# AgentMaker/PAPC

Measured on AMD Instinct MI355X. Metric: point-clouds/sec (fwd+bwd) PointNet++SSG B=32 N=4096, higher is better.
Workload: dtype f32

## Files before the change

include/papc_hip.h:

```cpp
#ifndef PAPC_HIP_H
#define PAPC_HIP_H

#include <stddef.h>
#include <stdint.h>

#ifdef __cplusplus
extern "C" {
#endif

#define PAPC_OK 0
#define PAPC_E_INVALID (-1)
#define PAPC_E_UNSUPPORTED (-2)
#define PAPC_E_LAUNCH (-3)

typedef void *papc_stream_t;

int papc_version(void);
#define PAPC_ABI_VERSION 8
int papc_abi_version(void);
int64_t papc_abi_sizeof(const char *struct_name);
const char *papc_last_error_string(void);


int papc_fps_f32(const float *xyz, int64_t sb, int64_t sn, int64_t sc, int B, int N, int npoint,
// ... 142 lines not shown
                        const papc_scatter_dst *scatter, const papc_bwd_red *next_red, papc_stream_t stream);

int papc_mlp_bwd_dw_f32(const papc_bwd_dy *dy, int a_mode, const float *x, int64_t ldx,
                        const papc_group_src *grp, const float *bn_scale, const float *bn_shift, int64_t M,
                        int Cin, int Cout, int rows_per_chunk, float *dw_partial, float *db_partial,
                        int64_t part_ld, papc_stream_t stream);

int papc_mlp_bwd_dw_chunk_hint(int64_t M, int Cin, int Cout, int a_mode, int dz_mode, int K);

int papc_reduce_partials_f32(const float *partial, int n_chunks, int64_t n, float *out, int accumulate,
                             papc_stream_t stream);
typedef struct papc_reduce_job {
    const float *partial;
    int32_t n_chunks;
    int32_t accumulate;
    int64_t ld, n1, n2;
    float *out1, *out2;
} papc_reduce_job;
int papc_reduce_partials_batch_f32(const papc_reduce_job *jobs, int count, papc_stream_t stream);
int papc_reduce_partials2_f32(const float *partial, int n_chunks, int64_t ld, int64_t n1, float *out1, int64_t n2,
                              float *out2, int accumulate, papc_stream_t stream);

#define PAPC_FOLD_MAX 24
typedef struct papc_fold_job {
    const float *partial;
    int32_t n_chunks;
    int32_t accumulate;
    int64_t ld;
    int32_t rows, cols;
    float *out; int64_t out_ld;
} papc_fold_job;
typedef struct papc_fold_list { papc_fold_job *jobs; int32_t capacity, count; } papc_fold_list;
int papc_fold_jobs_f32(const papc_fold_job *jobs, int count, papc_stream_t stream);

#define PAPC_SA_MAX_LAYERS 8
#define PAPC_SA_IN_GROUP 0
#define PAPC_SA_IN_ROWS 1
#define PAPC_SA_NO_LINGATHER 1u
#define PAPC_SA_NO_XYZ1 2u
#define PAPC_SA_NO_NOSTORE 4u
#define PAPC_SA_NO_GMAX 8u
#define PAPC_SA_NO_FUSED_RED 16u
#define PAPC_SA_NO_COMPACT 32u
#define PAPC_SA_NO_PLANES 64u
#define PAPC_SA_NO_PLANES_POINTWISE 128u
#define PAPC_SA_NO_XYZ_FUSE 256u
#define PAPC_SA_NO_PSEL 1024u
#define PAPC_SA_NO_GSIGN 2048u
#define PAPC_SA_NO_WSTATS 512u
typedef struct papc_sa_desc {
    int32_t B, N, S, K, D;
    int32_t n_layers;
    int32_t cin;
    int32_t cout[PAPC_SA_MAX_LAYERS];
    int32_t input;
    int32_t identity_rows;
    int32_t xyz_first, pool, eval_bn, cut_gather_grad;
    float eps, momentum;
    uint32_t disable;
    int32_t inference;
    int32_t want_input_grad;
} papc_sa_desc;
typedef struct papc_sa_layer {
    const float *w, *b, *gamma, *beta;
    float *running_mean, *running_var;
} papc_sa_layer;
typedef struct papc_compact_src {
    const int32_t *start, *rows, *cidx, *seg_grp;
    const float *wrow, *coef;
    int32_t G;
} papc_compact_src;
typedef struct papc_sa_io {
    const float *xyz; int64_t sb, sn, sc;
    const float *new_xyz;
    const float *feats;
    const int32_t *idx;
    const float *x_rows;
    const float *xc; const double *xc_gram;
    const papc_compact_src *compact;
    const float *consts3; int32_t consts3_ld;
    papc_sa_layer layer[PAPC_SA_MAX_LAYERS];
    float *out;
    void *saved, *scratch;
    const papc_point_lists *plists;
    const float *wfeat;
} papc_sa_io;
typedef struct papc_sa_plan {
    papc_sa_desc d;
    int32_t cin0;
    int32_t lin0, xyz1, gmax, nostore, compact, sparse_max, planes;
    int64_t saved_bytes, fwd_scratch_bytes, bwd_scratch_bytes;
    int64_t off_y[PAPC_SA_MAX_LAYERS], off_cst[PAPC_SA_MAX_LAYERS], off_argmax;
} papc_sa_plan;
typedef struct papc_sa_grads {
    const float *gout;
    float *dw[PAPC_SA_MAX_LAYERS], *db[PAPC_SA_MAX_LAYERS], *dgamma[PAPC_SA_MAX_LAYERS], *dbeta[PAPC_SA_MAX_LAYERS];
    int32_t acc_w[PAPC_SA_MAX_LAYERS], acc_gb[PAPC_SA_MAX_LAYERS];
    const float *wt[PAPC_SA_MAX_LAYERS];
    float *grad_feats, *grad_x;
    struct papc_fold_list *defer;
} papc_sa_grads;
int papc_sa_mlp_plan(const papc_sa_desc *desc, const papc_sa_io *io, papc_sa_plan *plan);
int papc_sa_mlp_fwd(const papc_sa_plan *plan, const papc_sa_io *io, papc_stream_t stream);
int papc_sa_mlp_bwd(const papc_sa_plan *plan, const papc_sa_io *io, const papc_sa_grads *grads, papc_stream_t stream);

typedef struct papc_pfn_desc {
    int32_t P, T, C;
    float vx, vy, x_offset, y_offset;
    float eps, momentum;
    int32_t training;
    int32_t zero_padded;
} papc_pfn_desc;
typedef struct papc_pfn_io {
    const float *features; const int32_t *num_voxels, *coors;
    const float *w, *gamma, *beta;
    float *running_mean, *running_var;
    float *out;
    void *saved, *scratch;
    uint32_t *tickets;
} papc_pfn_io;
int papc_pfn_workspace(const papc_pfn_desc *desc, int64_t *saved_bytes, int64_t *scratch_bytes);
int papc_pfn_fwd(const papc_pfn_desc *desc, const papc_pfn_io *io, papc_stream_t stream);
int papc_pfn_bwd(const papc_pfn_desc *desc, const papc_pfn_io *io, const float *gout, float *dw, float *dgamma, float *dbeta, int accumulate,
                 papc_stream_t stream);


int papc_pfn_decorate_f32(const float *features, const int32_t *num_voxels, const int32_t *coors, int P, int T,
                          float vx, float vy, float x_offset, float y_offset, int with_distance, float *out,
                          papc_stream_t stream);
int papc_pfn_decorate_nf_f32(const float *features, int F, const int32_t *num_voxels, const int32_t *coors, int P, int T,
                             float vx, float vy, float x_offset, float y_offset, int with_distance, float *out, papc_stream_t stream);
int papc_pfn_stats_f32(const float *features, const int32_t *num_voxels, const int32_t *coors, int P, int T,
                       float vx, float vy, float x_offset, float y_offset, const float *w, int C,
                       float *stats_partial, int *n_blocks_out, papc_stream_t stream);
int papc_pfn_apply_f32(const float *features, const int32_t *num_voxels, const int32_t *coors, int P, int T,
                       float vx, float vy, float x_offset, float y_offset, const float *w, int C,
// ... 195 lines not shown
int papc_mlp_gemm_rows_keys_f32(const float *x, int64_t ldx, const float *bn_scale, const float *bn_shift, const float *w, const float *bias,
                                int64_t M, int Cin, int Cout, float *y, float *stats_partial, const int32_t *rows_dev, const float *wrow,
                                const int32_t *seg_grp, const float *sign_src, unsigned long long *keys, papc_stream_t stream);
int papc_bn_relu_select_seg_f32(const unsigned long long *keys, const float *y, int C, const int32_t *start, const float *sign_src,
                                const float *scale, const float *shift, int G, float *out, int32_t *argmax, float *ysel, papc_stream_t stream);
int papc_lingather_fwd_f32(const float *P, const papc_group_src *grp, int B, const float *w, int ldw, int xcol0, const float *bias, int C,
                           float *y, float *stats_partial, papc_stream_t stream);
int papc_lingather_bwd_f32(const papc_bwd_dy *dy, const papc_group_src *grp, int B, int C, float *G, float *dwx_partial, papc_stream_t stream);
int papc_lingather_bwd_pp_ok(const papc_group_src *grp, int B, int C);
int papc_lingather_bwd_pp_f32(const papc_bwd_dy *dy, const papc_group_src *grp, int B, int C, const float *P, const float *w, int ldw, int xcol0,
                              const float *bias, float *G, float *dwx_partial, papc_stream_t stream);
int papc_lingather_list_parts(int64_t BN);
int papc_lingather_bwd_parts(const papc_group_src *grp, int B, int C);
int papc_lingather_bwd_lists_ok(const papc_group_src *grp, int C);
int papc_point_lists_f32(const papc_group_src *grp, int B, const int32_t *start, int32_t *prange, int32_t *prow, float *pmeta, float *pmom,
                         papc_stream_t stream);

int papc_mlp_bwd_dx_xyz_ok(int64_t M, int Cin, int Cout);
int papc_mlp_bwd_dx_xyz_f32(const papc_bwd_dy *dy, const float *wt, int64_t M, int Cin, int Cout, const float *xc, const float *wf,
                            float *partial, papc_stream_t stream);

int papc_bn_max_prep_f32(const float *gout, const float *ysel, const float *scale, const float *shift, const float *mean,
                         const float *invstd, const float *c1, const float *c2, const float *w, const float *bias, int64_t G, int Co,
                         int Ci, float *psel, float *wcat, float *hbias, float *e_out, float *q_out, papc_stream_t stream);
int papc_mlp_bwd_dx_max_f32(const float *psel, const int32_t *argmax, int K, const float *x, int64_t ldx, const float *bn_scale,
                            const float *bn_shift, const float *wcat, const float *hbias, int64_t M, int Cin, int Cout, float *dx,
                            const papc_bwd_red *next_red, papc_stream_t stream);

int papc_mlp_max_nostore_ok(int64_t M, int Cin, int Cout, int K);
int64_t papc_mlp_bwd_dw_max_ws_floats(int64_t M, int Cin, int Cout);
int papc_mlp_bwd_dw_max_f32(const float *psel, const int32_t *argmax, int K, const float *x, const float *bn_scale, const float *bn_shift,
                            const float *w, const float *e, const float *scale, const float *c1, int64_t M, int Cin, int Cout,
                            float *workspace, float *dw, int accumulate, papc_stream_t stream);

int papc_mlp_xyz_ok(int64_t M, int C1, int C2);
int papc_xyz_parts(int64_t M);
int papc_xyz_bwd_parts(int64_t M);
int papc_xyz_group_f32(const papc_group_src *grp, int B, float *xc, double *gram_partial, papc_stream_t stream);
int papc_xyz_gram_fold_f32(const double *gram_partial, int parts, double *gram, papc_stream_t stream);
int papc_xyz_l1_finalize_f32(const double *gram_partial, int parts, int64_t M, const float *w, int ldw, int xcol0, const float *bias,
                             const float *gamma, const float *beta, float eps, float momentum, int C, float *mean, float *invstd, float *scale,
                             float *shift, float *running_mean, float *running_var, float *wf, double *gram, papc_stream_t stream);
int papc_xyz_l1_bwd_f32(const float *dz, const float *xc, const float *wf, int64_t M, int C, float *partial, papc_stream_t stream);
int papc_xyz_l1_bwd_finalize_f32(const float *partial, int parts, int64_t M, int C, const double *gram, const float *w, int ldw, int xcol0,
                                 const float *bias, const float *mean, const float *invstd, const float *scale, float *dgamma, float *dbeta,
                                 float *dw, int accumulate, papc_stream_t stream);

size_t papc_pg_planes_bytes(int64_t R, int64_t K);

typedef struct papc_pg_wjob {
    const float *src;
    int64_t row_stride, col_stride;
    int R, K;
    void *planes;
} papc_pg_wjob;
int papc_pg_prep_weights_f32(const papc_pg_wjob *jobs, int count, papc_stream_t stream);

#define PAPC_PG_PLAIN 0
#define PAPC_PG_CONCAT 1
#define PAPC_PG_BNRELU 2
#define PAPC_PG_DY_DENSE 3
#define PAPC_PG_DY_MAX 4
typedef struct papc_pg_prep {
    int mode;
    int64_t M; int C;
    const float *x; int64_t ldx;
    const float *xyz; int64_t sb, sn, sc; const float *feats; int N, D, xyz_first;
    const float *dz;
    const float *gout, *ysel; const int32_t *argmax; int K;
    const float *stats; int parts;
    const float *gamma, *beta; float eps, momentum; float *running_mean, *running_var;
    float *mean, *invstd, *scale, *shift;
    const float *red; int red_parts;
    float *dgamma, *dbeta; int accumulate;
    void *planes, *planes_t;
} papc_pg_prep;
int papc_pg_prep_rows_f32(const papc_pg_prep *args, papc_stream_t stream);

#define PAPC_PG_STORE 0
// ... 86 lines not shown
```

papc_amd/_lib.py:

```python
import ctypes
import os

_HERE = os.path.dirname(os.path.abspath(__file__))
LIB_PATH = os.environ.get("PAPC_LIB") or os.path.join(_HERE, "libpapc_hip.so")

ABI_VERSION = 8

c_p = ctypes.c_void_p
c_i = ctypes.c_int
c_l = ctypes.c_int64
c_f = ctypes.c_float


class PapcError(RuntimeError):
    pass


class GroupSrc(ctypes.Structure):
    _fields_ = [("xyz", c_p), ("sb", c_l), ("sn", c_l), ("sc", c_l), ("new_xyz", c_p), ("feats", c_p),
                ("idx", c_p), ("N", c_i), ("S", c_i), ("K", c_i), ("D", c_i), ("xyz_first", c_i),
                ("cidx", c_p), ("seg_grp", c_p), ("rows_dev", c_p), ("wstat", c_p), ("plists", c_p)]


class PointLists(ctypes.Structure):
# ... 27 lines not shown

class ReduceJob(ctypes.Structure):
    _fields_ = [("partial", c_p), ("n_chunks", ctypes.c_int32), ("accumulate", ctypes.c_int32), ("ld", c_l), ("n1", c_l), ("n2", c_l),
                ("out1", c_p), ("out2", c_p)]


class ScatterDst(ctypes.Structure):
    _fields_ = [("grad_feats", c_p), ("idx", c_p), ("N", c_i), ("S", c_i), ("K", c_i), ("D", c_i), ("col0", c_i)]


SIGNATURES = {
    "papc_version": (c_i, []),
    "papc_abi_version": (c_i, []),
    "papc_abi_sizeof": (c_l, [ctypes.c_char_p]),
    "papc_last_error_string": (ctypes.c_char_p, []),
    "papc_fps_f32": (c_i, [c_p, c_l, c_l, c_l, c_i, c_i, c_i, c_p, c_f, c_p, c_p, c_p]),
    "papc_ball_query_f32": (c_i, [c_p, c_l, c_l, c_l, c_p, c_i, c_i, c_i, c_i, c_p, c_p, c_p, c_i, c_p]),
    "papc_square_distance_f32": (c_i, [c_p, c_p, c_i, c_i, c_i, c_p, c_p]),
    "papc_index_points_f32": (c_i, [c_p, c_p, c_i, c_i, c_i, c_i, c_i, c_p, c_p]),
    "papc_index_points_bwd_f32": (c_i, [c_p, c_p, c_i, c_i, c_i, c_i, c_i, c_p, c_p]),
    "papc_group_points_f32": (c_i, [c_p, c_l, c_l, c_l, c_p, c_p, c_p, c_i, c_i, c_i, c_i, c_i, c_i, c_p, c_p]),
    "papc_group_points_bwd_f32": (c_i, [c_p, c_p, c_i, c_i, c_i, c_i, c_i, c_i, c_p, c_p, c_p, c_p]),
    "papc_three_nn_f32": (c_i, [c_p, c_l, c_l, c_l, c_p, c_l, c_l, c_l, c_i, c_i, c_i, c_p, c_p, c_p, c_p]),
    "papc_three_interpolate_f32": (c_i, [c_p, c_p, c_p, c_i, c_i, c_i, c_i, c_p, c_p]),
    "papc_three_interpolate_bwd_f32": (c_i, [c_p, c_p, c_p, c_i, c_i, c_i, c_i, c_p, c_p]),
    "papc_three_interpolate_bwd_first3_f32": (c_i, [c_p, c_p, c_i, c_i, c_i, c_i, c_p, c_p]),
    "papc_mlp_gemm_parts": (c_i, [c_l]),
    "papc_mlp_gemm_gmax_ok": (c_i, [c_l, c_i, c_i]),
    "papc_mlp_gemm_f32": (c_i, [c_i, c_p, c_l, c_p, c_p, c_p, c_p, c_p, c_l, c_i, c_i, c_p, c_p, c_p, c_p]),
    "papc_mlp_gemm_rows_f32": (c_i, [c_i, c_p, c_l, c_p, c_p, c_p, c_p, c_p, c_l, c_i, c_i, c_p, c_p, c_p, c_p, c_p]),
    "papc_mlp_gemm_rows_w_f32": (c_i, [c_i, c_p, c_l, c_p, c_p, c_p, c_p, c_p, c_l, c_i, c_i, c_p, c_p, c_p, c_p, c_p, c_p]),
    "papc_sa_mlp_plan": (c_i, [c_p, c_p, c_p]),
    "papc_sa_mlp_fwd": (c_i, [c_p, c_p, c_p]),
    "papc_sa_mlp_bwd": (c_i, [c_p, c_p, c_p, c_p]),
    "papc_pfn_workspace": (c_i, [c_p, c_p, c_p]),
    "papc_pfn_fwd": (c_i, [c_p, c_p, c_p]),
    "papc_pfn_bwd": (c_i, [c_p, c_p, c_p, c_p, c_p, c_p, c_i, c_p]),
    "papc_compact_plan_f32": (c_i, [c_p, c_i, c_i, c_p, c_p, c_p, c_p, c_p, c_p, c_p, c_p]),
    "papc_compact_corr_parts": (c_i, []),
    "papc_mlp_compact_ok": (c_i, [c_l, c_i, c_i, c_p]),
    "papc_bn_stats_corr_f32": (c_i, [c_p, c_i, c_p, c_p, c_i, c_p, c_p]),
    "papc_bn_relu_max_seg_f32": (c_i, [c_p, c_i, c_p, c_p, c_p, c_i, c_p, c_p, c_p, c_p]),
    "papc_mlp_seg_epi_ok": (c_i, [c_l, c_i, c_i]),
    "papc_mlp_gemm_rows_keys_f32": (c_i, [c_p, c_l, c_p, c_p, c_p, c_p, c_l, c_i, c_i, c_p, c_p, c_p, c_p, c_p, c_p, c_p, c_p]),
    "papc_bn_relu_select_seg_f32": (c_i, [c_p, c_p, c_i, c_p, c_p, c_p, c_p, c_i, c_p, c_p, c_p, c_p]),
    "papc_bn_select_max_f32": (c_i, [c_p, c_p, c_p, c_p, c_p, c_p, c_l, c_i, c_p, c_p, c_p]),
    "papc_bn_finalize_f32": (c_i, [c_p, c_i, c_l, c_i, c_p, c_p, c_f, c_f, c_p, c_p, c_p, c_p, c_p, c_p, c_p]),
    "papc_bn_relu_max_f32": (c_i, [c_p, c_p, c_p, c_l, c_i, c_i, c_p, c_p, c_p]),
    "papc_bn_relu_f32": (c_i, [c_p, c_p, c_p, c_l, c_i, c_p, c_p]),
    "papc_bn_bwd_reduce_max_f32": (c_i, [c_p, c_p, c_i, c_p, c_p, c_p, c_p, c_l, c_i, c_i, c_p, c_p, c_p]),
    "papc_bn_bwd_reduce_f32": (c_i, [c_i, c_p, c_p, c_p, c_i, c_p, c_p, c_p, c_p, c_p, c_l, c_i, c_i, c_p, c_p]),
    "papc_bn_bwd_finalize_f32": (c_i, [c_p, c_i, c_l, c_i, c_p, c_p, c_p, c_p, c_i, c_p]),
    "papc_bn_eval_consts_f32": (c_i, [c_p, c_p, c_p, c_p, c_f, c_i, c_p, c_p, c_p, c_p, c_p]),
    "papc_group_max_bwd_f32": (c_i, [c_p, c_p, c_l, c_i, c_i, c_p, c_p]),
    "papc_mlp_bwd_dx_f32": (c_i, [c_p, c_p, c_l, c_i, c_i, c_p, c_p, c_p, c_p]),
    "papc_mlp_bwd_dw_f32": (c_i, [c_p, c_i, c_p, c_l, c_p, c_p, c_p, c_l, c_i, c_i, c_i, c_p, c_p, c_l, c_p]),
    "papc_reduce_partials2_f32": (c_i, [c_p, c_i, c_l, c_l, c_p, c_l, c_p, c_i, c_p]),
    "papc_reduce_partials_batch_f32": (c_i, [c_p, c_i, c_p]),
    "papc_fold_jobs_f32": (c_i, [c_p, c_i, c_p]),
    "papc_mlp_bwd_dw_chunk_hint": (c_i, [c_l, c_i, c_i, c_i, c_i, c_i]),
    "papc_reduce_partials_f32": (c_i, [c_p, c_i, c_l, c_p, c_i, c_p]),
    "papc_pfn_decorate_f32": (c_i, [c_p, c_p, c_p, c_i, c_i, c_f, c_f, c_f, c_f, c_i, c_p, c_p]),
    "papc_pfn_decorate_nf_f32": (c_i, [c_p, c_i, c_p, c_p, c_i, c_i, c_f, c_f, c_f, c_f, c_i, c_p, c_p]),
    "papc_pfn_stats_f32": (c_i, [c_p, c_p, c_p, c_i, c_i, c_f, c_f, c_f, c_f, c_p, c_i, c_p, c_p, c_p]),
    "papc_pfn_apply_f32": (c_i, [c_p, c_p, c_p, c_i, c_i, c_f, c_f, c_f, c_f, c_p, c_i, c_p, c_p, c_p, c_p, c_p]),
    "papc_pfn_num_blocks": (c_i, [c_i]),
# ... 42 lines not shown
    "papc_kdbn_fwd_f32": (c_i, [c_p, c_l, c_p, c_l, c_p, c_p, c_p, c_p, c_p, c_p, c_i, c_i, c_i, c_i, c_f, c_f, c_i, c_p, c_p, c_p, c_p, c_p, c_p, c_p,
                                ctypes.c_size_t, c_p]),
    "papc_kdbn_bwd_workspace": (ctypes.c_size_t, [c_i, c_i, c_i, c_i]),
    "papc_kdbn_bwd_f32": (c_i, [c_p, c_p, c_p, c_p, c_p, c_l, c_p, c_l, c_p, c_p, c_p, c_p, c_p, c_i, c_i, c_i, c_i, c_i, c_p, c_l, c_p, c_p, c_p, c_p, c_i,
                                c_p, ctypes.c_size_t, c_p]),
    "papc_voxconv_ok": (c_i, [c_i]),
    "papc_voxconv_parts": (c_i, [c_i, c_i]),
    "papc_voxconv1_fwd_f32": (c_i, [c_p, c_p, c_p, c_i, c_i, c_p, c_p, c_p]),
    "papc_voxconv2_prep_f32": (c_i, [c_p, c_p, c_p, c_p]),
    "papc_voxconv2_pool_fwd_f32": (c_i, [c_p, c_p, c_p, c_p, c_p, c_i, c_i, c_p, c_p, c_p]),
    "papc_voxconv2_bwd_dx_f32": (c_i, [c_p] * 8 + [c_i, c_i, c_p, c_p, c_p, c_p]),
    "papc_voxconv2_bwd_dw_workspace": (ctypes.c_size_t, [c_i, c_i]),
    "papc_voxconv2_bwd_dw_f32": (c_i, [c_p, c_p, c_p, c_p, c_p, c_i, c_i, c_p, c_p, c_i, c_p, ctypes.c_size_t, c_p]),
    "papc_voxconv1_bwd_dw_workspace": (ctypes.c_size_t, [c_i, c_i]),
    "papc_voxconv1_bwd_dw_f32": (c_i, [c_p] * 8 + [c_i, c_i, c_p, c_p, c_i, c_p, ctypes.c_size_t, c_p]),
    "papc_leaky_dropout_fwd_f32": (c_i, [c_p, c_l, c_f, c_f, c_p, c_i, c_i, c_p, c_p, c_p]),
    "papc_leaky_dropout_bwd_f32": (c_i, [c_p, c_p, c_p, c_l, c_f, c_f, c_p, c_p]),
    "papc_occupancy_grid_f32": (c_i, [c_p, c_i, c_i, c_i, c_p, c_p, c_p]),
    "papc_nms_workspace": (ctypes.c_size_t, [c_i]),
    "papc_nms_f32": (c_i, [c_p, c_i, c_f, c_p, c_p, c_p, ctypes.c_size_t, c_p]),
    "papc_lingather_parts": (c_i, [c_l]),
    "papc_lingather_fwd_f32": (c_i, [c_p, c_p, c_i, c_p, c_i, c_i, c_p, c_i, c_p, c_p, c_p]),
    "papc_lingather_bwd_f32": (c_i, [c_p, c_p, c_i, c_i, c_p, c_p, c_p]),
    "papc_lingather_bwd_pp_f32": (c_i, [c_p, c_p, c_i, c_i, c_p, c_p, c_i, c_i, c_p, c_p, c_p, c_p]),
    "papc_lingather_list_parts": (c_i, [c_l]),
    "papc_lingather_bwd_parts": (c_i, [c_p, c_i, c_i]),
    "papc_lingather_bwd_lists_ok": (c_i, [c_p, c_i]),
    "papc_point_lists_f32": (c_i, [c_p, c_i, c_p, c_p, c_p, c_p, c_p, c_p]),
    "papc_lingather_bwd_pp_ok": (c_i, [c_p, c_i, c_i]),
    "papc_bn_max_prep_f32": (c_i, [c_p] * 10 + [c_l, c_i, c_i] + [c_p] * 6),
    "papc_mlp_max_nostore_ok": (c_i, [c_l, c_i, c_i, c_i]),
    "papc_mlp_bwd_dw_max_ws_floats": (c_l, [c_l, c_i, c_i]),
    "papc_mlp_bwd_dw_max_f32": (c_i, [c_p, c_p, c_i, c_p, c_p, c_p, c_p, c_p, c_p, c_p, c_l, c_i, c_i, c_p, c_p, c_i, c_p]),
    "papc_mlp_bwd_dx_xyz_ok": (c_i, [c_l, c_i, c_i]),
    "papc_mlp_bwd_dx_xyz_f32": (c_i, [c_p, c_p, c_l, c_i, c_i, c_p, c_p, c_p, c_p]),
    "papc_mlp_bwd_dx_max_f32": (c_i, [c_p, c_p, c_i, c_p, c_l, c_p, c_p, c_p, c_p, c_l, c_i, c_i, c_p, c_p, c_p]),
    "papc_mlp_xyz_ok": (c_i, [c_l, c_i, c_i]),
    "papc_xyz_parts": (c_i, [c_l]),
    "papc_xyz_bwd_parts": (c_i, [c_l]),
    "papc_xyz_group_f32": (c_i, [c_p, c_i, c_p, c_p, c_p]),
    "papc_xyz_gram_fold_f32": (c_i, [c_p, c_i, c_p, c_p]),
    "papc_xyz_l1_finalize_f32": (c_i, [c_p, c_i, c_l, c_p, c_i, c_i, c_p, c_p, c_p, c_f, c_f, c_i] + [c_p] * 9),
    "papc_xyz_l1_bwd_f32": (c_i, [c_p, c_p, c_p, c_l, c_i, c_p, c_p]),
    "papc_xyz_l1_bwd_finalize_f32": (c_i, [c_p, c_i, c_l, c_i, c_p, c_p, c_i, c_i] + [c_p] * 7 + [c_i, c_p]),
    "papc_pg_planes_bytes": (ctypes.c_size_t, [c_l, c_l]),
    "papc_pg_prep_weights_f32": (c_i, [c_p, c_i, c_p]),
    "papc_pg_prep_rows_f32": (c_i, [c_p, c_p]),
    "papc_pg_gemm_f32": (c_i, [c_p, c_p]),
    "papc_pg_gemm_group_f32": (c_i, [c_p, c_i, c_p]),
    "papc_pg_final_f32": (c_i, [c_p, c_i, c_l, c_i, c_p, c_p, c_f, c_f] + [c_p] * 10 + [c_l, c_p, c_p, c_p]),
    "papc_pg_final_groups_f32": (c_i, [c_p, c_i, c_l, c_i, c_p, c_p, c_f, c_f] + [c_p] * 10 + [c_l, c_i, c_p, c_p, c_p, c_p]),
    "papc_pg_fold_f32": (c_i, [c_p, c_i, c_p]),
    "papc_transpose_batch_f32": (c_i, [c_p, c_p, c_p, c_p, c_i, c_p]),
    "papc_transpose_batch_ld_f32": (c_i, [c_p, c_p, c_p, c_p, c_p, c_p, c_i, c_p]),
    "papc_rotate_nms_f32": (c_i, [c_p, c_i, c_f, c_p, c_p, c_p, ctypes.c_size_t, c_p]),
    "papc_rotate_iou_f32": (c_i, [c_p, c_p, c_i, c_i, c_i, c_p, c_p]),
    "papc_rbbox_iou_f32": (c_i, [c_p, c_p, c_p, c_f, c_i, c_i, c_p, c_p]),
    "papc_riou_f32": (c_i, [c_p, c_p, c_f, c_i, c_i, c_p, c_p]),
    "papc_fill_f32": (c_i, [c_p, c_l, c_f, c_p]),
    "papc_copy_strided_batch_f32": (c_i, [c_p, c_i, c_p]),
    "papc_copy2d_f32": (c_i, [c_p, c_l, c_p, c_l, c_i, c_i, c_i, c_p]),
    "papc_reduce_partials_strided_f32": (c_i, [c_p, c_i, c_l, c_i, c_i, c_p, c_l, c_i, c_p]),
    "papc_scale_by_f32": (c_i, [c_p, c_p, c_l, c_p, c_p]),
    "papc_adam_step_f32": (c_i, [c_p, c_p, c_p, c_p, c_l, c_f, ctypes.c_double, ctypes.c_double, c_f, c_f, c_i, c_f, c_p]),
    "papc_adam_step_zero_f32": (c_i, [c_p, c_p, c_p, c_p, c_l, c_f, ctypes.c_double, ctypes.c_double, c_f, c_f, c_i, c_f, c_p]),
    "papc_adam_tick": (c_i, [c_p, c_p]),
    "papc_flag_set": (c_i, [c_p, ctypes.c_uint32, c_p, c_p]),
    "papc_flag_wait": (c_i, [c_p, c_l, c_p]),
    "papc_flag_wait_slot": (c_i, [c_p, c_i, c_l, c_p]),
    "papc_adam_step_dev_f32": (c_i, [c_p, c_p, c_p, c_p, c_l, c_f, ctypes.c_double, ctypes.c_double, c_f, c_f, c_p, c_f, c_i, c_p]),
    "papc_knob_set": (c_i, [ctypes.c_char_p, c_i]),
    "papc_knob_get": (c_i, [ctypes.c_char_p, ctypes.POINTER(c_i)]),
    "papc_prof_enable": (c_i, [ctypes.c_uint]),
    "papc_prof_reset": (c_i, []),
    "papc_prof_read": (c_i, [c_i, ctypes.POINTER(ctypes.c_double), ctypes.POINTER(c_l)]),
}

# ... 100 lines not shown
```

papc_amd/csrc/bn_ops.hip:

```cpp
#include "common.h"

namespace papc {

template <int V> struct Vec;
template <> struct Vec<4> {
    float4 v;
    __device__ static Vec load(const float *p) { Vec r; r.v = *reinterpret_cast<const float4 *>(p); return r; }
    __device__ void store(float *p) const { *reinterpret_cast<float4 *>(p) = v; }
    __device__ float &operator[](int i) { return (&v.x)[i]; }
    __device__ float operator[](int i) const { return (&v.x)[i]; }
};
template <> struct Vec<1> {
    float v;
    __device__ static Vec load(const float *p) { Vec r; r.v = *p; return r; }
    __device__ void store(float *p) const { *p = v; }
    __device__ float &operator[](int) { return v; }
    __device__ float operator[](int) const { return v; }
};

template <int D>
__device__ __forceinline__ void sum_partial_rows_d(const float *__restrict__ part, int n_tiles, int C, int c, int tl, double &s1, double &s2)
{
    for (int t0 = tl; t0 < n_tiles; t0 += 64 * D) {
        float a[D], b[D];
#pragma unroll
        for (int j = 0; j < D; ++j) {
            const int t = t0 + 64 * j;
            const int64_t o = (int64_t)(t < n_tiles ? t : t0) * 2 * C + c;
            a[j] = part[o];
            b[j] = part[o + C];
        }
#pragma unroll
        for (int j = 0; j < D; ++j) {
// ... 473 lines not shown
    const int n = blockIdx.x, tid = threadIdx.x;
    double hacc = 0.0;
    for (int c = tid; c < Co; c += 256) {
        const float s = scale[c];
        const float e = s * c2[c] * invstd[c];
        const float q = e * (mean[c] - (bias ? bias[c] : 0.f)) - s * c1[c];
        const float wv = w[(int64_t)c * Ci + n];
        ewn[c] = e * wv;
        hacc += (double)q * (double)wv;
        wcat[(int64_t)n * (Co + Ci) + c] = wv;
        if (n == 0) { e_out[c] = e; q_out[c] = q; }
    }
    red[tid] = hacc;
    __syncthreads();
    for (int st = 128; st > 0; st >>= 1) {
        if (tid < st) red[tid] += red[tid + st];
        __syncthreads();
    }
    if (tid == 0) hbias[n] = (float)red[0];
    for (int j = tid; j < Ci; j += 256) {
        double g = 0.0;
        for (int c = 0; c < Co; ++c) g += (double)ewn[c] * (double)w[(int64_t)c * Ci + j];
        wcat[(int64_t)n * (Co + Ci) + Co + j] = (float)(-g);
    }
}

struct TransposeBatch {
    const float *src[8];
    float *dst[8];
    int rows[8], cols[8];
    int ld[8], copy[8];
};

__global__ __launch_bounds__(256) void transpose_batch_kernel(TransposeBatch t)
{
    __shared__ float tile[32][33];
    const int m = blockIdx.y;
    const int rows = t.rows[m], cols = t.cols[m];
    const int tiles_c = (cols + 31) >> 5, tiles = ((rows + 31) >> 5) * tiles_c;
    const float *__restrict__ src = t.src[m];
    float *__restrict__ dst = t.dst[m];
    const int tx = threadIdx.x & 31, ty = threadIdx.x >> 5;
    for (int tl = blockIdx.x; tl < tiles; tl += gridDim.x) {
        const int r0 = (tl / tiles_c) * 32, c0 = (tl % tiles_c) * 32;
#pragma unroll
        for (int i = 0; i < 4; ++i) {
            const int r = r0 + ty + 8 * i, c = c0 + tx;
            const float v = (r < rows && c < cols) ? src[(int64_t)r * t.ld[m] + c] : 0.f;
            tile[ty + 8 * i][tx] = v;
            if (t.copy[m] && r < rows && c < cols) dst[(int64_t)r * cols + c] = v;
        }
        if (t.copy[m]) continue;
        __syncthreads();
#pragma unroll
        for (int i = 0; i < 4; ++i) {
            const int c = c0 + ty + 8 * i, r = r0 + tx;
            if (r < rows && c < cols) dst[(int64_t)c * rows + r] = tile[tx][ty + 8 * i];
        }
        __syncthreads();
    }
}

int bn_finalize_clear(const float *stats_partial, int n_tiles, int64_t M, int C, const float *gamma, const float *beta, float eps, float momentum,
                      float *mean, float *invstd, float *scale, float *shift, float *running_mean, float *running_var, void *clr, int64_t bytes,
                      hipStream_t st)
{
    PAPC_REQUIRE(stats_partial && mean && invstd && scale && shift && clr, PAPC_E_INVALID, "bn_finalize_clear: null pointer");
    PAPC_REQUIRE(n_tiles >= 1 && M >= 1 && C >= 1 && bytes >= 16 && bytes % 16 == 0 && aligned16(clr), PAPC_E_INVALID, "bn_finalize_clear: bad sizes");
    const int64_t n16 = bytes / 16, nclr = cdiv(n16, BN_CLEAR_PER_WG);
    PAPC_REQUIRE(nclr + C < (1ll << 31), PAPC_E_UNSUPPORTED, "bn_finalize_clear: %lld bytes", (long long)bytes);
    ProfScope prof(PAPC_K_MISC, st);
    hipLaunchKernelGGL(bn_finalize_clear_kernel, dim3((unsigned)(C + nclr)), dim3(64), 0, st, stats_partial, n_tiles, M, C, gamma, beta, eps, momentum,
                       mean, invstd, scale, shift, running_mean, running_var, reinterpret_cast<uint4 *>(clr), n16);
    return check_launch("bn_finalize_clear");
}

}


using namespace papc;

extern "C" {

int papc_bn_finalize_f32(const float *stats_partial, int n_tiles, int64_t M, int C, const float *gamma,
                         const float *beta, float eps, float momentum, float *mean, float *invstd,
                         float *scale, float *shift, float *running_mean, float *running_var,
                         papc_stream_t stream)
{
    PAPC_REQUIRE(stats_partial && mean && invstd && scale && shift, PAPC_E_INVALID, "papc_bn_finalize_f32: null pointer");
    PAPC_REQUIRE(n_tiles >= 1 && M >= 1 && C >= 1, PAPC_E_INVALID, "papc_bn_finalize_f32: bad sizes");
    hipStream_t st = as_stream(stream);
    ProfScope prof(PAPC_K_MISC, st);
    hipLaunchKernelGGL(bn_finalize_kernel, dim3((unsigned)C), dim3(64), 0, st, stats_partial, n_tiles, M, C, gamma,
// ... 151 lines not shown
    hipLaunchKernelGGL(copy_strided_batch_kernel, dim3((unsigned)std::min<int64_t>(tmax, 4096), (unsigned)count), dim3(256), 0, st, j);
    return check_launch("papc_copy_strided_batch_f32");
}

int papc_scale_by_f32(const float *x, const float *scalar, int64_t n, float *out, papc_stream_t stream)
{
    PAPC_REQUIRE(x && scalar && out && n >= 1, PAPC_E_INVALID, "papc_scale_by_f32: null pointer or n < 1");
    hipStream_t st = as_stream(stream);
    ProfScope prof(PAPC_K_MISC, st);
    hipLaunchKernelGGL(scale_by_kernel, dim3(ew_grid(n)), dim3(256), 0, st, x, scalar, n, out);
    return check_launch("papc_scale_by_f32");
}

int papc_bn_max_prep_f32(const float *gout, const float *ysel, const float *scale, const float *shift, const float *mean,
                         const float *invstd, const float *c1, const float *c2, const float *w, const float *bias, int64_t G, int Co,
                         int Ci, float *psel, float *wcat, float *hbias, float *e_out, float *q_out, papc_stream_t stream)
{
    PAPC_REQUIRE(scale && shift && mean && invstd && c1 && c2 && w && wcat && hbias && e_out && q_out && (!psel || (gout && ysel)), PAPC_E_INVALID,
                 "papc_bn_max_prep_f32: null pointer");
    PAPC_REQUIRE(G >= 1 && Co >= 1 && Ci >= 1 && Co <= 8192, PAPC_E_INVALID, "papc_bn_max_prep_f32: bad sizes");
    hipStream_t st = as_stream(stream);
    ProfScope prof(PAPC_K_BWD_REDUCE, st);
    if (psel) hipLaunchKernelGGL(bn_max_psel_kernel, dim3(ew_grid(G * Co)), dim3(256), 0, st, gout, ysel, scale, shift, G * Co, Co, psel);
    const size_t lds = (size_t)((Co + 1) & ~1) * sizeof(float) + 256 * sizeof(double);
    hipLaunchKernelGGL(bn_max_wcat_kernel, dim3((unsigned)Ci), dim3(256), lds, st, w, bias, scale, mean, invstd, c1, c2, Co, Ci, wcat, hbias, e_out, q_out);
    return check_launch("papc_bn_max_prep_f32");
}

int papc_transpose_batch_f32(const float *const *src, float *const *dst, const int *rows, const int *cols, int count, papc_stream_t stream)
{
    return papc_transpose_batch_ld_f32(src, nullptr, dst, rows, cols, nullptr, count, stream);
}

int papc_transpose_batch_ld_f32(const float *const *src, const int *src_ld, float *const *dst, const int *rows, const int *cols, const int *copy, int count,
                                papc_stream_t stream)
{
    PAPC_REQUIRE(src && dst && rows && cols, PAPC_E_INVALID, "papc_transpose_batch_f32: null pointer");
    PAPC_REQUIRE(count >= 1 && count <= 8, PAPC_E_INVALID, "papc_transpose_batch_f32: count=%d not in [1, 8]", count);
    TransposeBatch t{};
    int max_tiles = 1;
    for (int i = 0; i < count; ++i) {
        PAPC_REQUIRE(src[i] && dst[i] && rows[i] >= 1 && cols[i] >= 1, PAPC_E_INVALID, "papc_transpose_batch_f32: bad entry %d", i);
        t.src[i] = src[i]; t.dst[i] = dst[i]; t.rows[i] = rows[i]; t.cols[i] = cols[i];
        t.ld[i] = src_ld ? src_ld[i] : cols[i]; t.copy[i] = copy ? copy[i] : 0;
        PAPC_REQUIRE(t.ld[i] >= cols[i], PAPC_E_INVALID, "papc_transpose_batch_f32: entry %d: row stride shorter than a row", i);
        max_tiles = std::max(max_tiles, (int)(cdiv(rows[i], 32) * cdiv(cols[i], 32)));
    }
    hipStream_t st = as_stream(stream);
    ProfScope prof(PAPC_K_MISC, st);
    hipLaunchKernelGGL(transpose_batch_kernel, dim3((unsigned)std::min(max_tiles, 512), (unsigned)count), dim3(256), 0, st, t);
    return check_launch("papc_transpose_batch_f32");
}

static int adam_step(float *param, float *grad, float *exp_avg, float *exp_avg_sq, int64_t n, float lr, double beta1, double beta2, float eps,
                     float weight_decay, int step, float grad_scale, bool zero, papc_stream_t stream, const char *who)
{
    PAPC_REQUIRE(param && grad && exp_avg && exp_avg_sq, PAPC_E_INVALID, "%s: null pointer", who);
    PAPC_REQUIRE(n >= 1 && step >= 1, PAPC_E_INVALID, "%s: bad n/step", who);
    hipStream_t st = as_stream(stream);
    ProfScope prof(PAPC_K_MISC, st);
    const float bc1 = (float)(1.0 - pow(beta1, (double)step)), bc2 = (float)(1.0 - pow(beta2, (double)step));
    if (zero)
        hipLaunchKernelGGL(adam_kernel<true>, dim3(ew_grid(n)), dim3(256), 0, st, param, grad, exp_avg, exp_avg_sq, n, lr, (float)beta1, (float)beta2,
                           (float)(1.0 - beta1), (float)(1.0 - beta2), eps, weight_decay, bc1, bc2, grad_scale);
    else
        hipLaunchKernelGGL(adam_kernel<false>, dim3(ew_grid(n)), dim3(256), 0, st, param, grad, exp_avg, exp_avg_sq, n, lr, (float)beta1, (float)beta2,
                           (float)(1.0 - beta1), (float)(1.0 - beta2), eps, weight_decay, bc1, bc2, grad_scale);
    return check_launch(who);
}

int papc_adam_step_f32(float *param, const float *grad, float *exp_avg, float *exp_avg_sq, int64_t n,
                       float lr, double beta1, double beta2, float eps, float weight_decay, int step,
                       float grad_scale, papc_stream_t stream)
{
    return adam_step(param, const_cast<float *>(grad), exp_avg, exp_avg_sq, n, lr, beta1, beta2, eps, weight_decay, step, grad_scale, false, stream, "papc_adam_step_f32");
}

int papc_adam_tick(int64_t *step_dev, papc_stream_t stream)
{
    PAPC_REQUIRE(step_dev, PAPC_E_INVALID, "papc_adam_tick: null pointer");
    hipStream_t st = as_stream(stream);
    ProfScope prof(PAPC_K_MISC, st);
    hipLaunchKernelGGL(adam_tick_kernel, dim3(1), dim3(1), 0, st, step_dev);
    return check_launch("papc_adam_tick");
}
// ... 54 lines not shown
```

papc_amd/csrc/capi.hip:

```cpp
#include <stdarg.h>
#include <string.h>

#include <mutex>
#include <vector>

#include "common.h"

#define GEMM_PARTS_DEFAULT 768

namespace papc {

static thread_local char g_err[512] = "";

void set_error(const char *fmt, ...)
{
    va_list ap;
    va_start(ap, fmt);
    vsnprintf(g_err, sizeof(g_err), fmt, ap);
    va_end(ap);
}

int check_launch(const char *what)
{
    hipError_t e = hipGetLastError();
// ... 15 lines not shown
    {"PAPC_GEMM_WAVES", 0, 0, 8},
    {"PAPC_MAXCAT_WAVES", 8, 4, 8},
    {"PAPC_GEMM_WS", 0, 0, 3},
    {"PAPC_GEMM_OCC", 0, 0, 1},
    {"PAPC_GEMM_DBG", 0, 0, 1},
    {"PAPC_GEMM_KB", 0, 0, 2},
    {"PAPC_GEMM_MINWG", 192, 1, 4096},
    {"PAPC_GEMM_TL", 0, 0, 1},
    {"PAPC_FPS_THREADS", 0, 0, 1024},
    {"PAPC_FPS_THREADS_SMALL", 0, 0, 1024},
    {"PAPC_STREAM", 1, 0, 1},
    {"PAPC_STREAM_MINTILES", 2048, 1, 1 << 30},
    {"PAPC_STREAM_CK", 0, 0, 8},
    {"PAPC_STREAM_ASM", 1, 0, 1},
    {"PAPC_PFN_MFMA", 1, 0, 1},
    {"PAPC_DW_RS64", 1, 0, 1},
    {"PAPC_DW_ROWS", 1, 0, 1},
    {"PAPC_DW_ROWS_BLOCKS", 4, 1, 16},
    {"PAPC_DW_ROWSX", 1, 0, 1},
    {"PAPC_PG_DBG", 0, 0, 15},
    {"PAPC_PG_NB", 0, 0, 2},
    {"PAPC_PG_NS", 0, 0, 3},
    {"PAPC_STREAM_MAXCAT", 1, 0, 1},
    {"PAPC_MAX_NOSTORE", 1, 0, 1},
    {"PAPC_PFN_FUSED_TAILS", 1, 0, 1},
    {"PAPC_STREAM_NW12", 1, 0, 1},
    {"PAPC_LG_LISTS", 1, 0, 1},
    {"PAPC_FOLD_WAVES", 16, 8, 16},
    {"PAPC_LGL_VARIANT", 0, 0, 3},
    {"PAPC_LG_PP", 1, 0, 1},
    {"PAPC_PG_GROUP", 1, 0, 1},
    {"PAPC_PG_PIPE", 1, 0, 1},
    {"PAPC_SEG_EPI", 1, 0, 1},
};
static int g_knobs[KNOB_COUNT];
static int knob_parse(int id, const char *e)
{
    const KnobDef &d = g_knob_defs[id];
    if (!e || !*e) return d.def;
    const int v = atoi(e);
    return (v < d.lo || v > d.hi) ? d.def : v;
}
static const bool g_knobs_loaded = [] {
    for (int i = 0; i < KNOB_COUNT; ++i) g_knobs[i] = knob_parse(i, getenv(g_knob_defs[i].name));
    return true;
}();
int knob(int id) { return g_knobs[id]; }

struct ProfState {
    std::mutex mu;
    unsigned mask = 0;
    std::vector<std::pair<hipEvent_t, hipEvent_t>> pending[PAPC_K_COUNT];
    std::vector<hipEvent_t> pool;
    double total_ms[PAPC_K_COUNT] = {0};
    int64_t launches[PAPC_K_COUNT] = {0};
};
static ProfState g_prof;

static hipEvent_t prof_get_event()
{
    if (!g_prof.pool.empty()) {
        hipEvent_t e = g_prof.pool.back();
        g_prof.pool.pop_back();
        return e;
    }
    hipEvent_t e;
// ... 24 lines not shown
    for (auto &pr : g_prof.pending[k]) {
        float ms = 0.f;
        if (hipEventSynchronize(pr.second) == hipSuccess && hipEventElapsedTime(&ms, pr.first, pr.second) == hipSuccess) {
            g_prof.total_ms[k] += ms;
            g_prof.launches[k] += 1;
        }
        g_prof.pool.push_back(pr.first);
        g_prof.pool.push_back(pr.second);
    }
    g_prof.pending[k].clear();
}

}

extern "C" {

int papc_version(void) { return 600;  }

int papc_abi_version(void) { return PAPC_ABI_VERSION; }

int64_t papc_abi_sizeof(const char *struct_name)
{
    if (!struct_name) return -1;
#define PAPC_SIZEOF(T) if (strcmp(struct_name, #T) == 0) return (int64_t)sizeof(T);
    PAPC_SIZEOF(papc_group_src)
    PAPC_SIZEOF(papc_point_lists)
    PAPC_SIZEOF(papc_group_max)
    PAPC_SIZEOF(papc_bwd_dy)
    PAPC_SIZEOF(papc_scatter_dst)
    PAPC_SIZEOF(papc_bwd_red)
    PAPC_SIZEOF(papc_reduce_job)
    PAPC_SIZEOF(papc_fold_job)
    PAPC_SIZEOF(papc_fold_list)
    PAPC_SIZEOF(papc_sa_desc)
    PAPC_SIZEOF(papc_sa_layer)
    PAPC_SIZEOF(papc_compact_src)
    PAPC_SIZEOF(papc_sa_io)
    PAPC_SIZEOF(papc_sa_plan)
    PAPC_SIZEOF(papc_sa_grads)
    PAPC_SIZEOF(papc_pfn_desc)
    PAPC_SIZEOF(papc_pfn_io)
    PAPC_SIZEOF(papc_det_loss_desc)
    PAPC_SIZEOF(papc_det_loss_io)
    PAPC_SIZEOF(papc_det_post_desc)
    PAPC_SIZEOF(papc_det_post_io)
    PAPC_SIZEOF(papc_head_fc_layer)
    PAPC_SIZEOF(papc_head_bwd_job)
    PAPC_SIZEOF(papc_pg_wjob)
    PAPC_SIZEOF(papc_pg_prep)
    PAPC_SIZEOF(papc_pg_gemm)
    PAPC_SIZEOF(papc_pg_fold_job)
    PAPC_SIZEOF(papc_copy_job)
#undef PAPC_SIZEOF
    return -1;
}

const char *papc_last_error_string(void) { return papc::g_err; }

int papc_knob_set(const char *name, int value)
{
    PAPC_REQUIRE(name, PAPC_E_INVALID, "papc_knob_set: null name");
    for (int i = 0; i < papc::KNOB_COUNT; ++i)
        if (!strcmp(name, papc::g_knob_defs[i].name)) {
            PAPC_REQUIRE(value >= papc::g_knob_defs[i].lo && value <= papc::g_knob_defs[i].hi, PAPC_E_INVALID,
                         "papc_knob_set: %s = %d outside [%d, %d]", name, value, papc::g_knob_defs[i].lo, papc::g_knob_defs[i].hi);
            papc::g_knobs[i] = value;
// ... 45 lines not shown
```

papc_amd/csrc/common.h:

```cpp
#pragma once
#include <hip/hip_runtime.h>
#include <stdint.h>
#include <stdio.h>
#include <stdlib.h>
#include <string.h>
#include <algorithm>

#include "papc_hip.h"

namespace papc {

void set_error(const char *fmt, ...);
int check_launch(const char *what);

#define PAPC_REQUIRE(cond, code, ...)      \
    do {                                   \
        if (!(cond)) {                     \
            papc::set_error(__VA_ARGS__);  \
            return (code);                 \
        }                                  \
    } while (0)

enum Knob {
    KNOB_LG_PARTS, KNOB_DW_F32, KNOB_DW_DBG, KNOB_DW_XYZ, KNOB_PARTS, KNOB_GEMM_F32, KNOB_GEMM_WAVES, KNOB_MAXCAT_WAVES,
    KNOB_GEMM_WS, KNOB_GEMM_OCC, KNOB_GEMM_DBG, KNOB_GEMM_KB, KNOB_GEMM_MINWG, KNOB_GEMM_TL, KNOB_FPS_THREADS,
    KNOB_FPS_THREADS_SMALL, KNOB_STREAM, KNOB_STREAM_MINTILES, KNOB_STREAM_CK, KNOB_STREAM_ASM, KNOB_PFN_MFMA, KNOB_DW_RS64, KNOB_DW_ROWS, KNOB_DW_ROWS_BLOCKS, KNOB_DW_ROWSX, KNOB_PG_DBG, KNOB_PG_NB, KNOB_PG_NS, KNOB_STREAM_MAXCAT, KNOB_MAX_NOSTORE, KNOB_PFN_FUSED_TAILS, KNOB_STREAM_NW12, KNOB_LG_LISTS, KNOB_FOLD_WAVES, KNOB_LGL_VARIANT, KNOB_LG_PP, KNOB_PG_GROUP, KNOB_PG_PIPE, KNOB_SEG_EPI, KNOB_COUNT
};
int knob(int id);

struct ProfScope {
    int kernel;
    hipStream_t stream;
    bool on;
    hipEvent_t e0;
    ProfScope(int kernel, hipStream_t stream);
    ~ProfScope();
};

static inline hipStream_t as_stream(papc_stream_t s) { return reinterpret_cast<hipStream_t>(s); }

static inline int64_t cdiv(int64_t a, int64_t b) { return (a + b - 1) / b; }
static inline bool aligned16(const void *p) { return (reinterpret_cast<uintptr_t>(p) & 15) == 0; }

#define PAPC_DPP(v, ctrl, rmask) __builtin_amdgcn_update_dpp((int)(v), (int)(v), (ctrl), (rmask), 0xF, false)

__device__ __forceinline__ float wave_sum_f32_to_lane63(float v)
{
    float t;
    t = __int_as_float(PAPC_DPP(__float_as_int(v), 0xB1, 0xF));  v += t;
    t = __int_as_float(PAPC_DPP(__float_as_int(v), 0x4E, 0xF));  v += t;
    t = __int_as_float(PAPC_DPP(__float_as_int(v), 0x124, 0xF)); v += t;
    t = __int_as_float(PAPC_DPP(__float_as_int(v), 0x128, 0xF)); v += t;
    t = __int_as_float(__builtin_amdgcn_update_dpp(0, __float_as_int(v), 0x142, 0xA, 0xF, false)); v += t;
    t = __int_as_float(__builtin_amdgcn_update_dpp(0, __float_as_int(v), 0x143, 0xC, 0xF, false)); v += t;
    return v;
}

__device__ __forceinline__ float half_sum_f32(float v)
{
// ... 97 lines not shown
```

papc_amd/csrc/fold.h:

```cpp
#pragma once
#include "common.h"

namespace papc {

template <typename V> __device__ __forceinline__ V fold_zero();
template <> __device__ __forceinline__ float fold_zero<float>() { return 0.f; }
template <> __device__ __forceinline__ float4 fold_zero<float4>() { return make_float4(0.f, 0.f, 0.f, 0.f); }
__device__ __forceinline__ float fold_add(float s, float v) { return s + v; }
__device__ __forceinline__ float4 fold_add(float4 s, const float4 &v) { s.x += v.x; s.y += v.y; s.z += v.z; s.w += v.w; return s; }
__device__ __forceinline__ float fold_add_if(float s, float v, bool take) { return s + (take ? v : 0.f); }
__device__ __forceinline__ float4 fold_add_if(float4 s, const float4 &v, bool take) { return take ? fold_add(s, v) : s; }

template <int FW, int NLOAD, typename V>
__device__ __forceinline__ bool fold_lanes(const float *__restrict__ part, int64_t ld, int n_chunks, int64_t i, bool live, V (&red)[FW][64], V &total)
{
    const int el = threadIdx.x & 63, cl = threadIdx.x >> 6;
    V s = fold_zero<V>();
    if (live) {
        for (int t0 = cl; t0 < n_chunks; t0 += FW * NLOAD) {
            V v[NLOAD];
#pragma unroll
            for (int j = 0; j < NLOAD; ++j) {
                const int t = t0 + FW * j;
                v[j] = *reinterpret_cast<const V *>(part + (int64_t)(t < n_chunks ? t : t0) * ld + i);
            }
#pragma unroll
            for (int j = 0; j < NLOAD; ++j) s = fold_add_if(s, v[j], t0 + FW * j < n_chunks);
        }
    }
    red[cl][el] = s;
    __syncthreads();
    const bool top = cl == 0 && live;
    if (top) {
#pragma unroll
        for (int g = 1; g < FW; ++g) s = fold_add(s, red[g][el]);
    }
    total = s;
    return top;
}

enum FoldStart { FOLD_FROM_FIRST, FOLD_FROM_ZERO };

template <int NLOAD, FoldStart START, typename V>
__device__ __forceinline__ V fold_in_order(const float *__restrict__ part, int64_t ld, int n_chunks, int64_t i)
{
    V s = fold_zero<V>();
    for (int t0 = 0; t0 < n_chunks; t0 += NLOAD) {
        V v[NLOAD];
#pragma unroll
        for (int j = 0; j < NLOAD; ++j) v[j] = *reinterpret_cast<const V *>(part + (int64_t)(t0 + j < n_chunks ? t0 + j : t0) * ld + i);
#pragma unroll
        for (int j = 0; j < NLOAD; ++j)
            if (t0 + j < n_chunks) { if (START == FOLD_FROM_FIRST && t0 + j == 0) s = v[j]; else s = fold_add(s, v[j]); }
    }
    return s;
}

}
```

papc_amd/csrc/folds.hip:

```cpp
#include "fold.h"

namespace papc {

__device__ __forceinline__ void reduce_partials_body(float (&red)[16][64], const float *__restrict__ part, int n_chunks, int64_t n, int64_t ld,
                                                     float *__restrict__ out, int64_t n1, float *__restrict__ out2, int accumulate)
{
    const int64_t i = (int64_t)blockIdx.x * 64 + (threadIdx.x & 63);
    float s;
    if (fold_lanes<16, 8>(part, ld, n_chunks, i, i < n, red, s)) {
        float *o = i < n1 ? out + i : out2 + (i - n1);
        *o = accumulate ? *o + s : s;
    }
}

__global__ __launch_bounds__(1024) void reduce_partials_kernel(const float *__restrict__ part, int n_chunks, int64_t n,
                                                               int64_t ld, float *__restrict__ out, int64_t n1,
                                                               float *__restrict__ out2, int accumulate)
{
    __shared__ float red[16][64];
    reduce_partials_body(red, part, n_chunks, n, ld, out, n1, out2, accumulate);
}

struct ReduceBatch {
    const float *part[8]; float *out1[8], *out2[8];
    int64_t ld[8], n1[8], n[8];
    int n_chunks[8], accumulate[8];
};
__global__ __launch_bounds__(1024) void reduce_partials_batch_kernel(ReduceBatch b)
{
    __shared__ float red[16][64];
    const int job = blockIdx.y;
    if ((int64_t)blockIdx.x * 64 >= b.n[job]) return;
// ... 18 lines not shown
                                                                       float *__restrict__ out, int64_t out_ld, int accumulate)
{
    __shared__ float red[64][17];
    const int el = threadIdx.x & 15, sl = threadIdx.x >> 4;
    const int64_t n = (int64_t)rows * cols;
    const int64_t e = (int64_t)blockIdx.x * 16 + el;
    float s = 0.f;
    if (e < n) {
        for (int t0 = sl; t0 < n_chunks; t0 += 64 * 4) {
            float v[4];
#pragma unroll
            for (int j = 0; j < 4; ++j) v[j] = (t0 + 64 * j < n_chunks) ? part[(int64_t)(t0 + 64 * j) * ld + e] : 0.f;
#pragma unroll
            for (int j = 0; j < 4; ++j) s += v[j];
        }
    }
    red[sl][el] = s;
    __syncthreads();
    for (int h = 32; h >= 1; h >>= 1) {
        if (sl < h) red[sl][el] += red[sl + h][el];
        __syncthreads();
    }
    if (sl == 0 && e < n) {
        const int r = (int)(e / cols), c = (int)(e - (int64_t)r * cols);
        float *o = out + (int64_t)r * out_ld + c;
        *o = accumulate ? *o + red[0][el] : red[0][el];
    }
}

struct FoldBatch {
    const float *part[PAPC_FOLD_MAX]; float *out[PAPC_FOLD_MAX];
    int64_t ld[PAPC_FOLD_MAX], out_ld[PAPC_FOLD_MAX];
    int n_chunks[PAPC_FOLD_MAX], rows[PAPC_FOLD_MAX], cols[PAPC_FOLD_MAX], wg0[PAPC_FOLD_MAX + 1];
    unsigned acc_mask, wide_mask, vec_mask;
    int count;
};
template <int FW>
__global__ __launch_bounds__(64 * FW) void fold_jobs_kernel(FoldBatch b)
{
    __shared__ float red[FW][64];
    int job = 0;
    while (job + 1 < b.count && (int)blockIdx.x >= b.wg0[job + 1]) ++job;
    const int wg = (int)blockIdx.x - b.wg0[job];
    const float *__restrict__ part = b.part[job];
    float *__restrict__ out = b.out[job];
    const int64_t ld = b.ld[job], out_ld = b.out_ld[job];
    const int n_chunks = b.n_chunks[job], cols = b.cols[job];
    const int64_t n = (int64_t)b.rows[job] * cols;
    const bool acc = (b.acc_mask >> job) & 1u;
    if ((b.wide_mask >> job) & 1u) {
        const int64_t e = ((int64_t)wg * (64 * FW) + threadIdx.x) * 4;
        if (e >= n) return;
        float4 s = fold_in_order<8, FOLD_FROM_FIRST, float4>(part, ld, n_chunks, e);
        float4 *o = reinterpret_cast<float4 *>(out + e);
        if (acc) s = fold_add(s, *o);
        *o = s;
        return;
    }
    const int el = threadIdx.x & 63;
    if ((b.vec_mask >> job) & 1u) {
        __shared__ float4 red4[FW][64];
        const int64_t i4 = ((int64_t)wg * 64 + el) * 4;
        float4 s4;
        if (fold_lanes<FW, 8>(part, ld, n_chunks, i4, i4 < n, red4, s4)) {
            float4 *o = reinterpret_cast<float4 *>(out + i4);
            if (acc) s4 = fold_add(s4, *o);
            *o = s4;
        }
        return;
    }
    const int64_t i = (int64_t)wg * 64 + el;
    float s;
    if (fold_lanes<FW, 8>(part, ld, n_chunks, i, i < n, red, s)) {
        const int r = (int)(i / cols), c = (int)(i - (int64_t)r * cols);
        float *o = out + (int64_t)r * out_ld + c;
        *o = acc ? *o + s : s;
    }
}

}


using namespace papc;

static bool disjoint_column_blocks(const papc_fold_job &a, const papc_fold_job &b)
{
    if (a.rows < 2 || b.rows < 2 || a.out_ld != b.out_ld) return false;
    const bool a_first = (uintptr_t)a.out <= (uintptr_t)b.out;
    const papc_fold_job &p = a_first ? a : b, &q = a_first ? b : a;
    const uintptr_t bytes = (uintptr_t)q.out - (uintptr_t)p.out;
    if (bytes % sizeof(float)) return false;
    const int64_t c0 = (int64_t)(bytes / sizeof(float)) % p.out_ld;
    return c0 >= p.cols && c0 + q.cols <= p.out_ld;
}

extern "C" {

int papc_reduce_partials2_f32(const float *partial, int n_chunks, int64_t ld, int64_t n1, float *out1, int64_t n2,
                              float *out2, int accumulate, papc_stream_t stream)
{
    PAPC_REQUIRE(partial && out1 && (n2 == 0 || out2), PAPC_E_INVALID, "papc_reduce_partials2_f32: null pointer");
    PAPC_REQUIRE(n_chunks >= 1 && n1 >= 1 && n2 >= 0 && ld >= n1 + n2, PAPC_E_INVALID, "papc_reduce_partials2_f32: bad sizes");
    hipStream_t st = as_stream(stream);
    ProfScope prof(PAPC_K_MISC, st);
    const int64_t n = n1 + n2;
    const bool wide = n_chunks <= 64 && n >= 16384 && n1 % 4 == 0 && n2 % 4 == 0 && ld % 4 == 0 && aligned16(partial) && aligned16(out1) &&
                      (n2 == 0 || aligned16(out2));
    if (wide)
        hipLaunchKernelGGL(reduce_partials_wide_kernel, dim3((unsigned)cdiv(n, 256)), dim3(256), 0, st, partial, n_chunks, n, ld, out1, n1, out2, accumulate);
    else
        hipLaunchKernelGGL(reduce_partials_kernel, dim3((unsigned)cdiv(n, 64)), dim3(1024), 0, st, partial, n_chunks, n, ld, out1, n1, out2, accumulate);
    return check_launch("papc_reduce_partials2_f32");
}

int papc_reduce_partials_batch_f32(const papc_reduce_job *jobs, int count, papc_stream_t stream)
{
    PAPC_REQUIRE(jobs, PAPC_E_INVALID, "papc_reduce_partials_batch_f32: null jobs");
    PAPC_REQUIRE(count >= 1 && count <= 8, PAPC_E_INVALID, "papc_reduce_partials_batch_f32: count=%d not in [1, 8]", count);
    ReduceBatch b;
    memset(&b, 0, sizeof(b));
    int64_t nmax = 0;
    for (int i = 0; i < count; ++i) {
        const papc_reduce_job &j = jobs[i];
        PAPC_REQUIRE(j.partial && j.out1 && (j.n2 == 0 || j.out2), PAPC_E_INVALID, "papc_reduce_partials_batch_f32: null pointer in job %d", i);
        PAPC_REQUIRE(j.n_chunks >= 1 && j.n1 >= 1 && j.n2 >= 0 && j.ld >= j.n1 + j.n2, PAPC_E_INVALID, "papc_reduce_partials_batch_f32: bad sizes in job %d", i);
        b.part[i] = j.partial; b.out1[i] = j.out1; b.out2[i] = j.out2; b.ld[i] = j.ld; b.n1[i] = j.n1; b.n[i] = j.n1 + j.n2;
        b.n_chunks[i] = j.n_chunks; b.accumulate[i] = j.accumulate;
        nmax = std::max(nmax, j.n1 + j.n2);
    }
    hipStream_t st = as_stream(stream);
    ProfScope prof(PAPC_K_MISC, st);
    hipLaunchKernelGGL(reduce_partials_batch_kernel, dim3((unsigned)cdiv(nmax, 64), (unsigned)count), dim3(1024), 0, st, b);
    return check_launch("papc_reduce_partials_batch_f32");
}

int papc_fold_jobs_f32(const papc_fold_job *jobs, int count, papc_stream_t stream)
{
    PAPC_REQUIRE(jobs, PAPC_E_INVALID, "papc_fold_jobs_f32: null jobs");
    PAPC_REQUIRE(count >= 1, PAPC_E_INVALID, "papc_fold_jobs_f32: count=%d", count);
    hipStream_t st = as_stream(stream);
    const int FW = knob(KNOB_FOLD_WAVES) == 16 ? 16 : 8;
    for (int j0 = 0; j0 < count;) {
        FoldBatch b;
        memset(&b, 0, sizeof(b));
        int64_t wgs = 0;
        uintptr_t lo[PAPC_FOLD_MAX], hi[PAPC_FOLD_MAX];
        int nj = 0;
        for (; nj < PAPC_FOLD_MAX && j0 + nj < count; ++nj) {
            const int i = nj;
            const papc_fold_job &j = jobs[j0 + i];
            PAPC_REQUIRE(j.partial && j.out, PAPC_E_INVALID, "papc_fold_jobs_f32: null pointer in job %d", j0 + i);
            PAPC_REQUIRE(j.n_chunks >= 1 && j.rows >= 1 && j.cols >= 1 && j.ld >= (int64_t)j.rows * j.cols && j.out_ld >= j.cols, PAPC_E_INVALID,
                         "papc_fold_jobs_f32: bad sizes in job %d", j0 + i);
            lo[i] = (uintptr_t)j.out;
            hi[i] = lo[i] + sizeof(float) * (uintptr_t)((int64_t)(j.rows - 1) * j.out_ld + j.cols);
            bool overlaps = false;
            for (int k = 0; k < i && !overlaps; ++k)
                overlaps = lo[i] < hi[k] && lo[k] < hi[i] && !disjoint_column_blocks(jobs[j0 + k], j);
            if (overlaps) break;
            const int64_t n = (int64_t)j.rows * j.cols;
            const bool wide = j.n_chunks <= 16 && n >= 16384 && n % 4 == 0 && j.ld % 4 == 0 && (j.rows == 1 || j.out_ld == j.cols) && aligned16(j.partial) && aligned16(j.out);
            b.part[i] = j.partial; b.out[i] = j.out; b.ld[i] = j.ld; b.out_ld[i] = j.out_ld; b.n_chunks[i] = j.n_chunks; b.rows[i] = j.rows; b.cols[i] = j.cols;
            if (j.accumulate) b.acc_mask |= 1u << i;
            const bool vec = !wide && n >= 1024 && n % 4 == 0 && j.ld % 4 == 0 && (j.rows == 1 || j.out_ld == j.cols) && aligned16(j.partial) && aligned16(j.out);
            if (wide) b.wide_mask |= 1u << i;
            if (vec) b.vec_mask |= 1u << i;
            b.wg0[i] = (int)wgs;
            wgs += wide ? cdiv(n, 4 * 64 * FW) : (vec ? cdiv(n, 256) : cdiv(n, 64));
            PAPC_REQUIRE(wgs < (1ll << 30), PAPC_E_UNSUPPORTED, "papc_fold_jobs_f32: too many elements");
        }
        b.wg0[nj] = (int)wgs;
        b.count = nj;
        ProfScope prof(PAPC_K_BWD_DW, st);
        if (FW == 8) hipLaunchKernelGGL(fold_jobs_kernel<8>, dim3((unsigned)wgs), dim3(512), 0, st, b);
        else hipLaunchKernelGGL(fold_jobs_kernel<16>, dim3((unsigned)wgs), dim3(1024), 0, st, b);
        const int rc = check_launch("papc_fold_jobs_f32");
        if (rc != PAPC_OK) return rc;
        j0 += nj;
    }
    return PAPC_OK;
}

int papc_reduce_partials_f32(const float *partial, int n_chunks, int64_t n, float *out, int accumulate, papc_stream_t stream)
{
    PAPC_REQUIRE(partial && out, PAPC_E_INVALID, "papc_reduce_partials_f32: null pointer");
    PAPC_REQUIRE(n_chunks >= 1 && n >= 1, PAPC_E_INVALID, "papc_reduce_partials_f32: bad sizes");
    hipStream_t st = as_stream(stream);
    ProfScope prof(PAPC_K_MISC, st);
    hipLaunchKernelGGL(reduce_partials_kernel, dim3((unsigned)cdiv(n, 64)), dim3(1024), 0, st, partial, n_chunks, n, n, out, n, (float *)nullptr, accumulate);
    return check_launch("papc_reduce_partials_f32");
}

int papc_reduce_partials_strided_f32(const float *partial, int n_chunks, int64_t ld, int rows, int cols, float *out, int64_t out_ld,
                                     int accumulate, papc_stream_t stream)
{
    PAPC_REQUIRE(partial && out, PAPC_E_INVALID, "papc_reduce_partials_strided_f32: null pointer");
    PAPC_REQUIRE(n_chunks >= 1 && rows >= 1 && cols >= 1 && ld >= (int64_t)rows * cols && out_ld >= cols, PAPC_E_INVALID,
                 "papc_reduce_partials_strided_f32: bad sizes");
    hipStream_t st = as_stream(stream);
    ProfScope prof(PAPC_K_MISC, st);
    hipLaunchKernelGGL(reduce_partials_strided_kernel, dim3((unsigned)cdiv((int64_t)rows * cols, 16)), dim3(1024), 0, st, partial, n_chunks, ld,
                       rows, cols, out, out_ld, accumulate);
    return check_launch("papc_reduce_partials_strided_f32");
}

}
```

papc_amd/csrc/mlp_dw.hip:

```cpp
#include <type_traits>
#include "mlp_loaders.h"

namespace papc {

template <int I, int N, class F>
__device__ __forceinline__ void dw_sfor(F &&f)
{
    if constexpr (I < N) {
        f(std::integral_constant<int, I>{});
        dw_sfor<I + 1, N>(f);
    }
}

void fill_dy(DySrc &d, const papc_bwd_dy *s);
int check_dy(const papc_bwd_dy *dy, int64_t M, int C, bool *vec, const char *who);
int fill_asrc(ASrc &a, int a_mode, const float *x, int64_t ldx, const papc_group_src *grp, const float *sc,
              const float *sh, int Cin, const char *who);

struct DwArgs {
    ASrc x;
    ASrc dy;
    int64_t M; int Cin; int Cout; int rows_per_chunk;
    float *dw_partial;
    float *db_partial;
    int64_t part_ld;
    int xmap;
    int TOp, TIp;
    int RS;
    unsigned long long *dbg;
};

constexpr int DW_T = 128;
constexpr int DW_TI_WIDE = 160;
constexpr int DW_STAGE_FLOATS = 9216;
// ... 1047 lines not shown
            for (int a = 0; a < NT; ++a)
#pragma unroll
                for (int b = 0; b < NTI; ++b)
#pragma unroll
                    for (int r = 0; r < 16; ++r) slab[wave - half][(a * NTI + b) * 16 + r][lane] = acc[a][b][r];
        }
        __syncthreads();
        if (wave < half) {
#pragma unroll
            for (int a = 0; a < NT; ++a)
#pragma unroll
                for (int b = 0; b < NTI; ++b)
#pragma unroll
                    for (int r = 0; r < 16; ++r) acc[a][b][r] += slab[wave][(a * NTI + b) * 16 + r][lane];
        }
        __syncthreads();
    }
    if (wave == 0) {
#pragma unroll
        for (int a = 0; a < NT; ++a)
#pragma unroll
            for (int b = 0; b < NTI; ++b)
#pragma unroll
                for (int r = 0; r < 16; ++r) {
                    const int rr = (r & 3) + 8 * (r >> 2) + 4 * hi;
                    const int row = a < 2 ? o0 + 32 * a + rr : Cout + 32 * yb + rr;
                    out[(int64_t)row * CI + 32 * b + l31] = acc[a][b][r];
                }
    }
}

__global__ __launch_bounds__(64) void dw_max_fold_kernel(const float *__restrict__ partial, int n_chunks, int64_t part_ld, int n, double *__restrict__ out)
{
    const int l = threadIdx.x & 15, q = threadIdx.x >> 4;
    const int e = blockIdx.x * 16 + l;
    const int per = (n_chunks + 3) / 4, c0 = q * per, c1 = min(n_chunks, c0 + per);
    double s = 0.0;
    if (e < n) {
        int c = c0;
        for (; c + 8 <= c1; c += 8) {
            float v[8];
#pragma unroll
            for (int j = 0; j < 8; ++j) v[j] = partial[(int64_t)(c + j) * part_ld + e];
#pragma unroll
            for (int j = 0; j < 8; ++j) s += (double)v[j];
        }
        for (; c < c1; ++c) s += (double)partial[(int64_t)c * part_ld + e];
    }
    const double s1 = __shfl(s, l + 16), s2 = __shfl(s, l + 32), s3 = __shfl(s, l + 48);
    if (q == 0 && e < n) out[e] = ((s + s1) + s2) + s3;
}

__global__ __launch_bounds__(256) void dw_max_finalize_kernel(const double *__restrict__ fold, const float *__restrict__ w, const float *__restrict__ e,
                                                              const float *__restrict__ scale, const float *__restrict__ c1, double inv_m, int Cout,
                                                              float *__restrict__ dw, int accumulate)
{
    constexpr int CI = 64;
    __shared__ double gc[CI][CI];
    const int tid = threadIdx.x;
    const double *G = fold + (int64_t)Cout * CI, *S = G + CI * CI;
    for (int q = tid; q < CI * CI; q += 256) {
        const int j = q >> 6, i = q & 63;
        gc[j][i] = G[q] - S[j] * S[i] * inv_m;
    }
    __syncthreads();
    const int i = tid & 63, c = 4 * blockIdx.x + (tid >> 6);
    if (c >= Cout) return;
    double dot = 0.0;
    for (int j = 0; j < CI; ++j) dot += (double)w[(int64_t)c * CI + j] * gc[j][i];
    const double v = fold[(int64_t)c * CI + i] - (double)scale[c] * (double)c1[c] * S[i] - (double)e[c] * dot;
    float *o = dw + (int64_t)c * CI + i;
    *o = accumulate ? *o + (float)v : (float)v;
}

static void dw_dbg_report(const DwArgs &p, int xm, int dm)
{
    hipDeviceSynchronize();
    unsigned long long h[32];
    hipMemcpy(h, g_dw_dbg, sizeof(h), hipMemcpyDeviceToHost);
    const double n = (double)h[4];
    fprintf(stderr, "[dw dbg] x %d dy %d M %lld Cout %d Cin %d: slots %.0f | consumer cyc/slot: reads+mfma-issue %.0f barrier %.0f | producer grp0 per ACTIVE slot: wait %.0f finish %.0f issue %.0f ; barrier/slot %.0f\n",
            xm, dm, (long long)p.M, p.Cout, p.Cin, n, h[0] / n, h[1] / n, h[8] / n, h[9] / n, h[10] / n, h[11] / n);
}

static bool dw_rowsx_ragged(int Cin, int Cout)
{
    return (Cin == 128 && Cout == 196) || (Cin == 196 && Cout == 256) || (Cin == 96 && Cout == 128) || (Cin == 64 && Cout == 96);
}
static bool dw_rowsx_eligible(int Cin, int Cout, bool dense, int K)
{
    return knob(KNOB_DW_ROWSX) != 0 && ((Cin == 128 && Cout % 128 == 0) || dw_rowsx_ragged(Cin, Cout)) && !dw_f32_exact() && (dense || (K >= 16 && K % 16 == 0));
}
static bool dw_rows_eligible(int Cin, int Cout, bool dense, int K)
{
    return knob(KNOB_DW_ROWS) != 0 && Cin % 64 == 0 && Cout % 64 == 0 && (Cin / 64) * (Cout / 64) <= knob(KNOB_DW_ROWS_BLOCKS) && !dw_f32_exact() && (dense || (K >= 16 && K % 16 == 0));
}

template <int XMODE, int DYMODE, bool VEC>
static int launch_dw_v(const DwArgs &p_in, hipStream_t st)
{
    DwArgs p = p_in;
    const int dbg_on = knob(KNOB_DW_DBG);
    if (dbg_on) {
        if (!g_dw_dbg) hipMalloc(&g_dw_dbg, 32 * sizeof(unsigned long long));
        hipMemsetAsync(g_dw_dbg, 0, 32 * sizeof(unsigned long long), st);
// ... 147 lines not shown
        else hipLaunchKernelGGL(dw_xyz_kernel<1>, dim3((unsigned)cdiv(M, rows_per_chunk)), dim3(256), 0, st, p);
        return check_launch("papc_mlp_bwd_dw_f32");
    }
    switch (a_mode) {
    case A_PLAIN: return dense ? launch_dw<A_PLAIN, A_DY_DENSE>(p, vec, st) : launch_dw<A_PLAIN, A_DY_MAX>(p, vec, st);
    case A_BNRELU: return dense ? launch_dw<A_BNRELU, A_DY_DENSE>(p, vec, st) : launch_dw<A_BNRELU, A_DY_MAX>(p, vec, st);
    default: return dense ? launch_dw<A_GROUP, A_DY_DENSE>(p, vec, st) : launch_dw<A_GROUP, A_DY_MAX>(p, vec, st);
    }
}

static int dw_max_chunks()
{
    static int n = 0;
    if (!n) {
        hipDeviceProp_t prop;
        int dev = 0, ncu = 256;
        if (hipGetDevice(&dev) == hipSuccess && hipGetDeviceProperties(&prop, dev) == hipSuccess && prop.multiProcessorCount > 0) ncu = prop.multiProcessorCount;
        n = std::max(8, (ncu / 2) & ~7);
    }
    return n;
}

extern "C" int64_t papc_mlp_bwd_dw_max_ws_floats(int64_t M, int Cin, int Cout)
{
    (void)M;
    const int64_t n = (int64_t)(Cout + Cin) * Cin + Cin;
    return (int64_t)dw_max_chunks() * n + 2 * n + 2;
}

extern "C" int papc_mlp_bwd_dw_max_f32(const float *psel, const int32_t *argmax, int K, const float *x, const float *bn_scale, const float *bn_shift,
                                       const float *w, const float *e, const float *scale, const float *c1, int64_t M, int Cin, int Cout,
                                       float *workspace, float *dw, int accumulate, papc_stream_t stream)
{
    PAPC_REQUIRE(psel && argmax && x && bn_scale && bn_shift && w && e && scale && c1 && workspace && dw, PAPC_E_INVALID, "papc_mlp_bwd_dw_max_f32: null pointer");
    PAPC_REQUIRE(papc_mlp_max_nostore_ok(M, Cin, Cout, K), PAPC_E_UNSUPPORTED,
                 "papc_mlp_bwd_dw_max_f32: not built for M=%lld Cin=%d Cout=%d K=%d (see papc_mlp_max_nostore_ok)", (long long)M, Cin, Cout, K);
    PAPC_REQUIRE(aligned16(x) && aligned16(workspace), PAPC_E_INVALID, "papc_mlp_bwd_dw_max_f32: x / workspace must be 16-byte aligned");
    DwMaxArgs p;
    memset(&p, 0, sizeof(p));
    const int n = (Cout + Cin) * Cin + Cin;
    p.x = x; p.xsc = bn_scale; p.xsh = bn_shift; p.psel = psel; p.argmax = argmax; p.partial = workspace;
    p.M = M; p.part_ld = n; p.K = K; p.Cout = Cout; p.n_chunks = dw_max_chunks();
    p.rows_per_chunk = (int)(cdiv(cdiv(M, p.n_chunks), 64) * 64);
    double *fold = reinterpret_cast<double *>(workspace + (((int64_t)p.n_chunks * n + 1) & ~(int64_t)1));
    hipStream_t st = as_stream(stream);
    ProfScope prof(PAPC_K_BWD_DW, st);
    hipLaunchKernelGGL(dw_rows_max_kernel, dim3((unsigned)(2 * p.n_chunks)), dim3(512), 0, st, p);
    hipLaunchKernelGGL(dw_max_fold_kernel, dim3((unsigned)cdiv(n, 16)), dim3(64), 0, st, workspace, p.n_chunks, (int64_t)n, n, fold);
    hipLaunchKernelGGL(dw_max_finalize_kernel, dim3((unsigned)cdiv(Cout, 4)), dim3(256), 0, st, fold, w, e, scale, c1, 1.0 / (double)M, Cout, dw, accumulate);
    return check_launch("papc_mlp_bwd_dw_max_f32");
}
```

papc_amd/csrc/sa_mlp.hip:

```cpp
#include "common.h"

#define SA_CALL(expr)                 \
    do {                              \
        const int rc__ = (expr);      \
        if (rc__ != PAPC_OK) return rc__; \
    } while (0)

namespace papc {
int pfn_gram_stats(const float *features, const int32_t *num_voxels, const int32_t *coors, int P, int T, float vx, float vy, float x_offset, float y_offset, int zero_padded,
                   double *gram_partial, const float *w, int C, const float *gamma, const float *beta, float eps, float momentum, float *mean, float *invstd,
                   float *scale, float *shift, float *running_mean, float *running_var, double *gram, unsigned *ticket, hipStream_t st);
int pfn_gram_impl(const float *features, const int32_t *num_voxels, const int32_t *coors, int P, int T, float vx, float vy, float x_offset, float y_offset,
                  double *gram_partial, int zero_padded, papc_stream_t stream);
int pfn_apply_impl(const float *features, const int32_t *num_voxels, const int32_t *coors, int P, int T, float vx, float vy, float x_offset, float y_offset,
                   const float *w, int C, const float *scale, const float *shift, float *out, int32_t *argmax, int zero_padded, papc_stream_t stream);
int pfn_bwd_sparse_impl(const float *features, const int32_t *num_voxels, const int32_t *coors, int P, int T, float vx, float vy, float x_offset, float y_offset,
                        const float *w, int C, const float *gout, const int32_t *argmax, const float *mean, const float *invstd, const float *scale,
                        const float *shift, float *partial, int zero_padded, papc_stream_t stream);
int bn_finalize_clear(const float *stats_partial, int n_tiles, int64_t M, int C, const float *gamma, const float *beta, float eps, float momentum,
                      float *mean, float *invstd, float *scale, float *shift, float *running_mean, float *running_var, void *clr, int64_t bytes,
                      hipStream_t st);
int pfn_bwd_fold_finalize(const float *partial, int n_chunks, float *sums, int64_t M, const float *w, int C, const double *gram, const float *mean,
                          const float *invstd, const float *scale, float *dgamma, float *dbeta, float *dw, int flags, unsigned *ticket, hipStream_t st);

constexpr int A_PLAIN_ = PAPC_A_PLAIN, A_BNRELU_ = PAPC_A_BNRELU, A_GROUP_ = PAPC_A_GROUP, A_XYZ_ = PAPC_A_XYZ;

struct Carver {
    char *base;
    size_t off;
    template <class T>
    T *take(size_t n)
    {
        off = (off + 255) & ~(size_t)255;
// ... 441 lines not shown
            plan->off_cst[l] = l < L ? (int64_t)(reinterpret_cast<char *>(ps.cst[l]) - fake) : -1;
        }
        plan->off_argmax = ps.argmax ? (int64_t)(reinterpret_cast<char *>(ps.argmax) - fake) : -1;
        plan->saved_bytes = (int64_t)layout_planes_saved(*plan, nullptr, ps) + 256;
        plan->fwd_scratch_bytes = (int64_t)layout_planes_fwd(*plan, nullptr, pf) + 256;
        plan->bwd_scratch_bytes = (int64_t)layout_planes_bwd(*plan, nullptr, pb) + 256;
        return PAPC_OK;
    }
    plan->lin0 = !(d.disable & PAPC_SA_NO_LINGATHER) && !ev && !plain && has_idx && has_feats && L >= 2 && d.D % 4 == 0 && d.D >= 16 &&
                 d.cout[0] % 4 == 0 && d.cout[0] <= 256;
    plan->xyz1 = !(d.disable & PAPC_SA_NO_XYZ1) && !ev && !plain && has_idx && !has_feats && d.D == 0 && L >= 3 &&
                 papc_mlp_xyz_ok(M, d.cout[0], d.cout[1]);
    plan->compact = plan->lin0 && d.pool && !(d.disable & PAPC_SA_NO_COMPACT) && io && io->compact && papc_mlp_compact_ok(M, d.K, L, d.cout);
    const int cL = d.cout[L - 1], cLi = L > 1 ? d.cout[L - 2] : plan->cin0;
    plan->gmax = !plan->compact && d.pool && !(d.disable & PAPC_SA_NO_GMAX) && !ev && papc_mlp_gemm_gmax_ok(M, cL, d.K);
    plan->nostore = plan->gmax && !(d.disable & PAPC_SA_NO_NOSTORE) && L >= 2 && !(L == 2 && plan->xyz1) && papc_mlp_max_nostore_ok(M, cLi, cL, d.K);
    plan->sparse_max = plan->nostore;
    SavedPtrs s; FwdPtrs f; BwdPtrs b;
    {
        char *fake = reinterpret_cast<char *>((uintptr_t)1 << 40);
        layout_saved(*plan, fake, s);
        for (int l = 0; l < PAPC_SA_MAX_LAYERS; ++l) {
            plan->off_y[l] = (l < L && s.y[l]) ? (int64_t)(reinterpret_cast<char *>(s.y[l]) - fake) : -1;
            plan->off_cst[l] = (l < L && s.cst[l]) ? (int64_t)(reinterpret_cast<char *>(s.cst[l]) - fake) : -1;
        }
        plan->off_argmax = s.argmax ? (int64_t)(reinterpret_cast<char *>(s.argmax) - fake) : -1;
    }
    plan->saved_bytes = (int64_t)layout_saved(*plan, nullptr, s) + 256;
    plan->fwd_scratch_bytes = (int64_t)layout_fwd(*plan, nullptr, f) + 256;
    plan->bwd_scratch_bytes = (int64_t)layout_bwd(*plan, nullptr, b) + 256;
    return PAPC_OK;
}

int papc_sa_mlp_fwd(const papc_sa_plan *plan, const papc_sa_io *io, papc_stream_t st)
{
    PAPC_REQUIRE(plan && io && io->out && io->saved && io->scratch, PAPC_E_INVALID, "papc_sa_mlp_fwd: null pointer");
    const papc_sa_plan &p = *plan;
    const papc_sa_desc &d = p.d;
    const int L = d.n_layers;
    const int64_t M = rows_of(d), G = (int64_t)d.B * d.S;
    const bool plain = d.input == PAPC_SA_IN_ROWS, ev = d.eval_bn != 0;
    PAPC_REQUIRE(plain ? io->x_rows != nullptr : (io->xyz && io->new_xyz), PAPC_E_INVALID, "papc_sa_mlp_fwd: missing input");
    PAPC_REQUIRE(plain || d.identity_rows || io->idx, PAPC_E_INVALID, "papc_sa_mlp_fwd: grouped input without idx (set identity_rows for sample_and_group_all)");
    PAPC_REQUIRE(plain || d.D == 0 || io->feats, PAPC_E_INVALID, "papc_sa_mlp_fwd: D = %d but feats is NULL", d.D);
    PAPC_REQUIRE(!p.compact || io->compact, PAPC_E_INVALID, "papc_sa_mlp_fwd: the plan is compacted but io->compact is NULL");
    if (p.planes) {
        for (int l = 0; l < L; ++l) PAPC_REQUIRE(io->layer[l].w && io->layer[l].gamma && io->layer[l].beta, PAPC_E_INVALID, "papc_sa_mlp_fwd: layer %d lacks w / gamma / beta", l);
        return planes_fwd(p, *io, st);
    }
    SavedPtrs s; FwdPtrs f;
    layout_saved(p, io->saved, s);
    layout_fwd(p, io->scratch, f);
    const int parts = papc_mlp_gemm_parts(M);
    const bool wstats = p.compact && !(d.disable & PAPC_SA_NO_WSTATS);
    const int R_c = (p.compact && !wstats) ? papc_compact_corr_parts() : 0;
    papc_group_src grp;
    if (!plain) fill_grp(grp, d, *io, p.compact);
    if (!plain && wstats) grp.wstat = io->compact->wrow;
    int cmax = 0;
    for (int l = 0; l < L; ++l) cmax = std::max(cmax, d.cout[l]);
    const size_t stats_stride = (size_t)(std::max(parts, p.lin0 ? papc_lingather_parts(M) : 0) + R_c) * 2 * cmax;
    const bool seg_epi = seg_epi_widths(p) && !ev && knob(KNOB_SEG_EPI) && papc_mlp_seg_epi_ok(M, cin_of(p, L - 1), d.cout[L - 1]);

    const float *prev_y = nullptr, *prev_sc = nullptr, *prev_sh = nullptr;
    int cin = p.cin0;
    const float *xc = nullptr;
    papc_group_max gm;
    memset(&gm, 0, sizeof(gm));
    for (int l = 0; l < L; ++l) {
        const papc_sa_layer &ly = io->layer[l];
        PAPC_REQUIRE(ly.w && ly.gamma && ly.beta, PAPC_E_INVALID, "papc_sa_mlp_fwd: layer %d lacks w / gamma / beta", l);
        PAPC_REQUIRE(!ev || (ly.running_mean && ly.running_var), PAPC_E_INVALID, "papc_sa_mlp_fwd: eval_bn needs the running statistics");
        const int cout = d.cout[l];
        float *stats = ev ? nullptr : f.stats + (size_t)l * stats_stride;
        int parts_l = parts;
        const papc_group_max *gm_ref = nullptr;
        if (l == L - 1 && p.gmax) {
            gm.gmax = s.gbuf_f; gm.gmin = s.gbuf_f + G * cout; gm.amax = f.gbuf_i; gm.amin = f.gbuf_i + G * cout; gm.K = d.K;
            gm.sign_src = (d.disable & PAPC_SA_NO_GSIGN) ? nullptr : ly.gamma;
            gm_ref = &gm;
        }
        float *y = s.y[l];
        float *cst = s.cst[l];
        if (l == 0 && p.xyz1) {
            const double *gpart1;
            if (io->xc && io->xc_gram) { xc = io->xc; gpart1 = io->xc_gram; }
            else {
                SA_CALL(papc_xyz_group_f32(&grp, d.B, s.xc, f.gpart + 16, st));
                SA_CALL(papc_xyz_gram_fold_f32(f.gpart + 16, papc_xyz_parts(M), f.gpart, st));
                xc = s.xc; gpart1 = f.gpart;
            }
            SA_CALL(papc_xyz_l1_finalize_f32(gpart1, 1, M, ly.w, cin, 0, ly.b, ly.gamma, ly.beta, d.eps, d.momentum, cout, cst, cst + cout, cst + 2 * cout,
                                             cst + 3 * cout, ly.running_mean, ly.running_var, s.wf, s.gram, st));
            prev_y = nullptr; prev_sc = cst + 2 * cout; prev_sh = cst + 3 * cout;
            cin = cout;
            continue;
        }
        if (l == 1 && p.xyz1) {
            SA_CALL(papc_mlp_gemm_f32(A_XYZ_, xc, 4, nullptr, s.wf, nullptr, ly.w, ly.b, M, cin, cout, y, stats, gm_ref, st));
        } else if (l == 0 && plain) {
            SA_CALL(papc_mlp_gemm_f32(A_PLAIN_, io->x_rows, cin, nullptr, nullptr, nullptr, ly.w, ly.b, M, cin, cout, y, stats, gm_ref, st));
        } else if (l == 0 && p.lin0) {
            const int fcol0 = d.xyz_first ? 3 : 0;
            const float *wfeat = io->wfeat;
            if (!wfeat) {
                SA_CALL(papc_copy2d_f32(ly.w + fcol0, cin, f.wfeat, d.D, cout, d.D, 0, st));
                wfeat = f.wfeat;
            }
            const int64_t BN = (int64_t)d.B * d.N;
            SA_CALL(papc_mlp_gemm_f32(A_PLAIN_, io->feats, d.D, nullptr, nullptr, nullptr, wfeat, nullptr, BN, d.D, cout, s.P, nullptr, nullptr, st));
            parts_l = papc_lingather_parts(M);
            SA_CALL(papc_lingather_fwd_f32(s.P, &grp, d.B, ly.w, cin, d.xyz_first ? 0 : d.D, ly.b, cout, y, stats, st));
        } else if (l == 0) {
            SA_CALL(papc_mlp_gemm_f32(A_GROUP_, nullptr, 0, &grp, nullptr, nullptr, ly.w, ly.b, M, cin, cout, y, stats, gm_ref, st));
        } else if (p.compact && seg_epi && l == L - 1) {
            SA_CALL(papc_mlp_gemm_rows_keys_f32(prev_y, cin, prev_sc, prev_sh, ly.w, ly.b, M, cin, cout, y, stats, io->compact->rows,
                                                wstats ? io->compact->wrow : nullptr, io->compact->seg_grp, ly.gamma, f.keys, st));
        } else if (p.compact) {
            SA_CALL(papc_mlp_gemm_rows_w_f32(A_BNRELU_, prev_y, cin, nullptr, prev_sc, prev_sh, ly.w, ly.b, M, cin, cout, y, stats, nullptr, io->compact->rows,
                                             wstats ? io->compact->wrow : nullptr, st));
        } else {
            SA_CALL(papc_mlp_gemm_f32(A_BNRELU_, prev_y, cin, nullptr, prev_sc, prev_sh, ly.w, ly.b, M, cin, cout, y, stats, gm_ref, st));
        }
        if (p.compact && !wstats) {
            SA_CALL(papc_bn_stats_corr_f32(y, cout, io->compact->start, io->compact->coef, io->compact->G, stats + (size_t)parts_l * 2 * cout, st));
            parts_l += R_c;
// ... 65 lines not shown
        }
        if (n) SA_CALL(papc_transpose_batch_f32(srcs, dsts, rws, cls, n, st));
    }

    papc_reduce_job jobs[PAPC_SA_MAX_LAYERS];
    int n_jobs = 0;
    bool xyz_fused = false;
    bool dz0_masked = false;
    const float *dz = nullptr;
    const float *fused_red = nullptr;
    int flip = 0;
    for (int l = L - 1; l >= 0; --l) {
        const papc_sa_layer &ly = io->layer[l];
        const int cout = d.cout[l], cin = cin_of(p, l);
        const float *cst = s.cst[l];
        float *c12 = b.c12[l];
        const bool acc_w = gr->acc_w[l] != 0, acc_gb = gr->acc_gb[l] != 0;
        float *dgamma = gr->dgamma[l] ? gr->dgamma[l] : b.tmp_gb, *dbeta = gr->dbeta[l] ? gr->dbeta[l] : b.tmp_gb + cmaxc;
        const bool gb_tmp = ev && acc_gb && gr->db[l];
        float *fgamma = gb_tmp ? b.tmp_gb : dgamma, *fbeta = gb_tmp ? b.tmp_gb + cmaxc : dbeta;
        PAPC_REQUIRE(gr->dw[l], PAPC_E_INVALID, "papc_sa_mlp_bwd: dw[%d] is NULL", l);
        papc_bwd_dy dy;
        memset(&dy, 0, sizeof(dy));
        if (p.compact) { dy.wrow = io->compact->wrow; dy.seg_grp = io->compact->seg_grp; dy.rows_dev = io->compact->rows; }
        if (l == L - 1 && !d.pool) { dy.dz_mode = PAPC_DZ_DENSE; dy.dz = gr->gout; dy.K = 1; }
        else if (l == L - 1) { dy.dz_mode = PAPC_DZ_MAX; dy.gout = gr->gout; dy.argmax = s.argmax; dy.K = d.K; }
        else { dy.dz_mode = PAPC_DZ_DENSE; dy.dz = dz; dy.K = 1; }
        if (l == 0 && p.xyz1) {
            PAPC_REQUIRE(!gr->dgamma[l] || (gr->acc_gb[l] != 0) == (gr->acc_w[l] != 0), PAPC_E_UNSUPPORTED,
                         "papc_sa_mlp_bwd: the coordinates-only first layer takes ONE accumulate flag for dw / dgamma / dbeta");
            int nbp = papc_xyz_bwd_parts(M);
            if (xyz_fused) nbp = papc_mlp_gemm_parts(M);
            else SA_CALL(papc_xyz_l1_bwd_f32(dz, xc, s.wf, M, cout, b.bpart, st));
            SA_CALL(papc_xyz_l1_bwd_finalize_f32(b.bpart, nbp, M, cout, s.gram, ly.w, cin, 0, ly.b, cst, cst + cout, cst + 2 * cout, dgamma, dbeta, gr->dw[l],
                                                 acc_w ? 1 : 0, st));
            if (gr->db[l] && !acc_w) SA_CALL(papc_fill_f32(gr->db[l], cout, 0.f, st));
            break;
        }
        dy.y = s.y[l];
        dy.mean = cst; dy.invstd = cst + cout; dy.scale = cst + 2 * cout; dy.shift = cst + 3 * cout;
        dy.c1 = c12; dy.c2 = c12 + cout;
        const float *red;
        int red_parts;
        if (!fused_red) {
            red = b.red; red_parts = n_parts;
            if (p.sparse_max && l == L - 1)
                SA_CALL(papc_bn_bwd_reduce_max_f32(ysel, dy.gout, dy.K, dy.mean, dy.invstd, dy.scale, dy.shift, M, cout, n_parts, b.red, b.psel, st));
            else if (p.compact && l == L - 1 && dy.dz_mode == PAPC_DZ_MAX && ysel && b.psel && !(d.disable & PAPC_SA_NO_PSEL)) {
                SA_CALL(papc_bn_bwd_reduce_max_f32(ysel, dy.gout, dy.K, dy.mean, dy.invstd, dy.scale, dy.shift, M, cout, n_parts, b.red, b.psel, st));
                dy.psel = b.psel;
            } else
                SA_CALL(papc_bn_bwd_reduce_f32(dy.dz_mode, dy.dz_mode == PAPC_DZ_MAX ? ysel : dy.dz, dy.gout, dy.argmax, dy.K, dy.y, dy.mean, dy.invstd, dy.scale,
                                               dy.shift, M, cout, n_parts, b.red, st));
        } else { red = fused_red; red_parts = gemm_parts; }
        SA_CALL(papc_bn_bwd_finalize_f32(red, red_parts, M, cout, fgamma, fbeta, c12, c12 + cout, ((acc_gb && !gb_tmp) ? 1 : 0) | (ev ? 2 : 0), st));
        if (l == 0 && p.lin0) {
            const int64_t BN = (int64_t)d.B * d.N;
            const int parts_l = papc_lingather_bwd_parts(&grp, d.B, cout);
            if (!papc_lingather_bwd_lists_ok(&grp, cout)) SA_CALL(papc_fill_f32(b.Gs, BN * cout, 0.f, st));
            if (dz0_masked && papc_lingather_bwd_pp_ok(&grp, d.B, cout))
                SA_CALL(papc_lingather_bwd_pp_f32(&dy, &grp, d.B, cout, s.P, ly.w, cin, d.xyz_first ? 0 : d.D, ly.b, b.Gs, b.dwx_part, st));
            else
                SA_CALL(papc_lingather_bwd_f32(&dy, &grp, d.B, cout, b.Gs, b.dwx_part, st));
            const int fcol0 = d.xyz_first ? 3 : 0, xcol0 = d.xyz_first ? 0 : d.D;
            float *dw = gr->dw[l];
            const int acc = acc_w ? 1 : 0;
            if (!defer_fold(*gr, b.dwx_part, parts_l, (int64_t)cout * 3, cout, 3, dw + xcol0, cin, acc))
                SA_CALL(papc_reduce_partials_strided_f32(b.dwx_part, parts_l, (int64_t)cout * 3, cout, 3, dw + xcol0, cin, acc, st));
            papc_bwd_dy dyg;
            memset(&dyg, 0, sizeof(dyg));
            dyg.dz_mode = PAPC_DZ_DENSE; dyg.dz = b.Gs; dyg.K = 1; dyg.y = b.Gs;
            dyg.mean = zeros; dyg.invstd = ones; dyg.scale = ones; dyg.shift = big; dyg.c1 = zeros; dyg.c2 = zeros;
            const int rpc_g = dw_rows_per_chunk(BN, cout, d.D, 64);
            const int n_chunks_g = (int)((BN + rpc_g - 1) / rpc_g);
            const int64_t pld_g = (int64_t)cout * d.D + cout;
            SA_CALL(papc_mlp_bwd_dw_f32(&dyg, A_PLAIN_, io->feats, d.D, nullptr, nullptr, nullptr, BN, d.D, cout, rpc_g, b.part_g, b.part_g + (int64_t)cout * d.D, pld_g, st));
            if (!defer_fold(*gr, b.part_g, n_chunks_g, pld_g, cout, d.D, dw + fcol0, cin, acc))
                SA_CALL(papc_reduce_partials_strided_f32(b.part_g, n_chunks_g, pld_g, cout, d.D, dw + fcol0, cin, acc, st));
            if (gr->db[l] && !acc_w) SA_CALL(papc_fill_f32(gr->db[l], cout, 0.f, st));
            if (f_needs) {
                const float *wft;
                if (gr->wt[l]) wft = gr->wt[l] + (int64_t)fcol0 * cout;
                else {
                    SA_CALL(papc_copy2d_f32(ly.w + fcol0, cin, b.wft, cout, cout, d.D, 1, st));
                    wft = b.wft;
                }
                SA_CALL(papc_mlp_gemm_f32(A_PLAIN_, b.Gs, cout, nullptr, nullptr, nullptr, wft, nullptr, BN, cout, d.D, gr->grad_feats, nullptr, nullptr, st));
            }
            break;
        }
        if (p.sparse_max && l == L - 1) {
            SA_CALL(papc_bn_max_prep_f32(nullptr, nullptr, cst + 2 * cout, cst + 3 * cout, cst, cst + cout, c12, c12 + cout, ly.w, ly.b, G, cout, cin, nullptr,
                                         b.wcat, b.hb, b.eq, b.eq + cout, st));
        }
        const bool x1 = p.xyz1 && l == 1;
        if (p.nostore && l == L - 1) {
            const float *pc = s.cst[l - 1];
            SA_CALL(papc_mlp_bwd_dw_max_f32(b.psel, s.argmax, d.K, s.y[l - 1], pc + 2 * cin, pc + 3 * cin, ly.w, b.eq, cst + 2 * cout, c12, M, cin, cout, b.dwmax_ws,
                                            gr->dw[l], acc_w ? 1 : 0, st));
            if (gr->db[l] && !acc_w) SA_CALL(papc_fill_f32(gr->db[l], cout, 0.f, st));
        } else {
            const int am = l == 0 ? (plain ? A_PLAIN_ : A_GROUP_) : (x1 ? A_XYZ_ : A_BNRELU_);
            const int rpc = dw_chunk(p, l, am, dy.dz_mode);
            const int n_chunks = (int)((M + rpc - 1) / rpc);
            const int64_t pld = (int64_t)cout * cin + cout;
            float *dwp = b.part[l], *dbp = b.part[l] + (int64_t)cout * cin;
            if (l == 0 && plain) SA_CALL(papc_mlp_bwd_dw_f32(&dy, A_PLAIN_, io->x_rows, cin, nullptr, nullptr, nullptr, M, cin, cout, rpc, dwp, dbp, pld, st));
            else if (l == 0) SA_CALL(papc_mlp_bwd_dw_f32(&dy, A_GROUP_, nullptr, 0, &grp, nullptr, nullptr, M, cin, cout, rpc, dwp, dbp, pld, st));
            else if (x1) SA_CALL(papc_mlp_bwd_dw_f32(&dy, A_XYZ_, xc, 4, nullptr, s.wf, nullptr, M, cin, cout, rpc, dwp, dbp, pld, st));
            else {
                const float *pc = s.cst[l - 1];
                SA_CALL(papc_mlp_bwd_dw_f32(&dy, A_BNRELU_, s.y[l - 1], cin, nullptr, pc + 2 * cin, pc + 3 * cin, M, cin, cout, rpc, dwp, dbp, pld, st));
            }
            const bool want_db = gr->db[l] && !ev;
            if (defer_room(*gr, 2)) {
                defer_fold(*gr, b.part[l], n_chunks, pld, 1, cout * cin, gr->dw[l], (int64_t)cout * cin, acc_w ? 1 : 0);
                if (want_db) defer_fold(*gr, b.part[l] + (int64_t)cout * cin, n_chunks, pld, 1, cout, gr->db[l], cout, acc_w ? 1 : 0);
            } else {
                papc_reduce_job &j = jobs[n_jobs++];
                j.partial = b.part[l]; j.n_chunks = n_chunks; j.accumulate = acc_w ? 1 : 0; j.ld = pld; j.n1 = (int64_t)cout * cin; j.out1 = gr->dw[l];
                j.n2 = want_db ? cout : 0; j.out2 = want_db ? gr->db[l] : nullptr;
            }
            if (ev && gr->db[l]) {
                hipLaunchKernelGGL(mul_vec_kernel, dim3((unsigned)cdiv(cout, 256)), dim3(256), 0, as_stream(st), cst + 2 * cout, fbeta, cout, gr->db[l], acc_w ? 1 : 0);
                SA_CALL(check_launch("papc_sa_mlp_bwd (eval-mode bias gradient)"));
                if (gb_tmp) {
                    hipLaunchKernelGGL(add_vec2_kernel, dim3((unsigned)cdiv(cout, 256)), dim3(256), 0, as_stream(st), fgamma, fbeta, cout, gr->dgamma[l], gr->dbeta[l]);
                    SA_CALL(check_launch("papc_sa_mlp_bwd (eval-mode dgamma / dbeta accumulate)"));
                }
            }
        }
        fused_red = nullptr;
// ... 112 lines not shown
```

papc_amd/csrc/xyz1.hip:

```cpp
#include "mlp_loaders.h"

namespace papc {

constexpr int XYZ_T = 256;
constexpr int XYZ_MAX_PARTS = 512;

__global__ __launch_bounds__(XYZ_T) void xyz_group_kernel(GroupSrc g, int64_t M, float4 *__restrict__ xc, double *__restrict__ partial)
{
    __shared__ double red[XYZ_T / 64][10];
    double s[10];
#pragma unroll
    for (int i = 0; i < 10; ++i) s[i] = 0.0;
    const int64_t per = (M + gridDim.x - 1) / gridDim.x;
    const int64_t m0 = (int64_t)blockIdx.x * per, m1 = min(M, m0 + per);
    for (int64_t m = m0 + threadIdx.x; m < m1; m += XYZ_T) {
        const uint32_t grp = fdiv((uint32_t)m, g.divK);
        const uint32_t b = fdiv(grp, g.divS);
        int j = g.idx ? g.idx[m] : (int)(m - (int64_t)b * g.S * g.K);
        const bool ok = j >= 0 && j < g.N;
        j = ok ? j : 0;
        const float *pp = g.xyz + (int64_t)b * g.sb + (int64_t)j * g.sn;
        const float *qq = g.new_xyz + (int64_t)grp * 3;
        float x = pp[0] - qq[0], y = pp[g.sc] - qq[1], z = pp[2 * g.sc] - qq[2];
        if (!ok) { x = 0.f; y = 0.f; z = 0.f; }
        xc[m] = make_float4(x, y, z, 0.f);
        const double dx = x, dy = y, dz = z;
        s[0] += dx; s[1] += dy; s[2] += dz;
        s[3] += dx * dx; s[4] += dx * dy; s[5] += dx * dz; s[6] += dy * dy; s[7] += dy * dz; s[8] += dz * dz;
        s[9] += 1.0;
    }
    const int lane = threadIdx.x & 63, wave = threadIdx.x >> 6;
#pragma unroll
    for (int i = 0; i < 10; ++i) {
        double v = s[i];
#pragma unroll
        for (int o = 32; o >= 1; o >>= 1) v += __shfl_xor(v, o);
        if (lane == 0) red[wave][i] = v;
    }
    __syncthreads();
    if (threadIdx.x < 10) {
        double v = 0.0;
#pragma unroll
        for (int w = 0; w < XYZ_T / 64; ++w) v += red[w][threadIdx.x];
        partial[(int64_t)blockIdx.x * 16 + threadIdx.x] = v;
    }
}

__global__ __launch_bounds__(256) void xyz_gram_fold_kernel(const double *__restrict__ partial, int parts, double *__restrict__ gram)
{
    __shared__ double red[16][16];
    const int e = threadIdx.x & 15, sl = threadIdx.x >> 4;
    double s = 0.0;
    if (e < 10) for (int t = sl; t < parts; t += 16) s += partial[(int64_t)t * 16 + e];
    red[sl][e] = s;
    __syncthreads();
    if (threadIdx.x < 16) {
        double v = 0.0;
#pragma unroll
        for (int q = 0; q < 16; ++q) v += red[q][threadIdx.x];
        gram[threadIdx.x] = threadIdx.x < 10 ? v : 0.0;
    }
}

__global__ __launch_bounds__(256) void xyz_l1_finalize_kernel(const double *__restrict__ partial, int parts, double M, const float *__restrict__ w, int ldw,
                                                              int xcol0, const float *__restrict__ bias, const float *__restrict__ gamma,
                                                              const float *__restrict__ beta, float eps, float momentum, int C, float *mean,
                                                              float *invstd, float *scale, float *shift, float *rmean, float *rvar, float *wf,
                                                              double *gram)
{
    __shared__ double red[16][16];
    __shared__ double G[10];
    const int e = threadIdx.x & 15, sl = threadIdx.x >> 4;
    double s = 0.0;
    if (e < 10) for (int t = sl; t < parts; t += 16) s += partial[(int64_t)t * 16 + e];
    red[sl][e] = s;
    __syncthreads();
    if (threadIdx.x < 10) {
        double v = 0.0;
#pragma unroll
        for (int q = 0; q < 16; ++q) v += red[q][threadIdx.x];
        G[threadIdx.x] = v;
        gram[threadIdx.x] = v;
    }
    __syncthreads();
    for (int c = threadIdx.x; c < C; c += 256) {
        const double w0 = w[(int64_t)c * ldw + xcol0], w1 = w[(int64_t)c * ldw + xcol0 + 1], w2 = w[(int64_t)c * ldw + xcol0 + 2];
        const double b = bias ? (double)bias[c] : 0.0;
        const double mx = G[0] / M, my = G[1] / M, mz = G[2] / M;
        const double cxx = G[3] / M - mx * mx, cxy = G[4] / M - mx * my, cxz = G[5] / M - mx * mz;
        const double cyy = G[6] / M - my * my, cyz = G[7] / M - my * mz, czz = G[8] / M - mz * mz;
        const double mu = w0 * mx + w1 * my + w2 * mz + b;
        double var = w0 * (w0 * cxx + w1 * cxy + w2 * cxz) + w1 * (w0 * cxy + w1 * cyy + w2 * cyz) + w2 * (w0 * cxz + w1 * cyz + w2 * czz);
        if (var < 0.0) var = 0.0;
        const double is = 1.0 / sqrt(var + (double)eps);
        const double sc = (gamma ? (double)gamma[c] : 1.0) * is;
        const double sh = (beta ? (double)beta[c] : 0.0) - mu * sc;
        mean[c] = (float)mu; invstd[c] = (float)is; scale[c] = (float)sc; shift[c] = (float)sh;
        if (rmean) rmean[c] = momentum * rmean[c] + (1.f - momentum) * (float)mu;
        if (rvar) rvar[c] = momentum * rvar[c] + (1.f - momentum) * (float)var;
        wf[c * 4 + 0] = (float)(sc * w0); wf[c * 4 + 1] = (float)(sc * w1); wf[c * 4 + 2] = (float)(sc * w2);
        wf[c * 4 + 3] = (float)(sc * b + sh);
    }
}

__global__ __launch_bounds__(XYZ_T) void xyz_l1_bwd_kernel(const float *__restrict__ dz, const float4 *__restrict__ xc, const float *__restrict__ wf,
                                                           int64_t M, int C, int64_t rows_per_chunk, float *__restrict__ partial)
{
    __shared__ float red[XYZ_T * 16];
    const int tid = threadIdx.x;
    const int CQ = C >> 2;
    const int RSL = XYZ_T / CQ;
    const int cq = tid % CQ, slot = tid / CQ;
    const bool act = slot < RSL;
    const int c = cq * 4;
    float4 k[4];
#pragma unroll
    for (int i = 0; i < 4; ++i) k[i] = ld4(wf + (c + i) * 4);
    float a[4][4];
#pragma unroll
    for (int i = 0; i < 4; ++i) a[i][0] = a[i][1] = a[i][2] = a[i][3] = 0.f;
    const int64_t mbeg = (int64_t)blockIdx.x * rows_per_chunk, mend = min(M, mbeg + rows_per_chunk);
    constexpr int U = 4;
    if (act) {
        for (int64_t m0 = mbeg + slot; m0 < mend; m0 += (int64_t)U * RSL) {
            float4 vz[U], vx[U];
            bool ok[U];
#pragma unroll
            for (int u = 0; u < U; ++u) {
                const int64_t m = m0 + (int64_t)u * RSL;
                ok[u] = m < mend;
                const int64_t mc = ok[u] ? m : mbeg;
                vz[u] = ld4(dz + mc * C + c);
                vx[u] = xc[mc];
            }
#pragma unroll
            for (int u = 0; u < U; ++u) {
                if (!ok[u]) continue;
                const float g[4] = {vz[u].x, vz[u].y, vz[u].z, vz[u].w};
#pragma unroll
                for (int i = 0; i < 4; ++i) {
                    const float z = fmaf(k[i].z, vx[u].z, fmaf(k[i].y, vx[u].y, fmaf(k[i].x, vx[u].x, k[i].w)));
                    const float p = z > 0.f ? g[i] : 0.f;
                    a[i][0] = fmaf(p, vx[u].x, a[i][0]); a[i][1] = fmaf(p, vx[u].y, a[i][1]); a[i][2] = fmaf(p, vx[u].z, a[i][2]);
                    a[i][3] += p;
                }
            }
        }
    }
#pragma unroll
    for (int i = 0; i < 4; ++i)
#pragma unroll
        for (int j = 0; j < 4; ++j) red[tid * 16 + i * 4 + j] = act ? a[i][j] : 0.f;
    __syncthreads();
    float *out = partial + (int64_t)blockIdx.x * C * 4;
    for (int t = tid; t < C * 4; t += XYZ_T) {
        const int ch = t >> 2, j = t & 3;
        const int q = ch >> 2, i = ch & 3;
        float sacc = 0.f;
        for (int sl = 0; sl < RSL; ++sl) sacc += red[(sl * CQ + q) * 16 + i * 4 + j];
        out[t] = sacc;
    }
}

__global__ __launch_bounds__(1024) void xyz_l1_bwd_finalize_kernel(const float *__restrict__ partial, int parts, double M, int C, const double *__restrict__ gram,
                                                                   const float *__restrict__ w, int ldw, int xcol0, const float *__restrict__ bias,
                                                                   const float *__restrict__ mean, const float *__restrict__ invstd,
                                                                   const float *__restrict__ scale, float *dgamma, float *dbeta, float *dw, int accumulate)
{
    __shared__ double red[64][17], red2[8][17];
    const int e = threadIdx.x & 15, sl = threadIdx.x >> 4;
    const int e0 = blockIdx.x * 16;
    const int c = blockIdx.x * 4 + threadIdx.x;
    const bool fin = threadIdx.x < 4 && c < C;
    const int cc = fin ? c : 0;
    const double w0 = w[(int64_t)cc * ldw + xcol0], w1 = w[(int64_t)cc * ldw + xcol0 + 1], w2 = w[(int64_t)cc * ldw + xcol0 + 2];
    const double b = bias ? (double)bias[cc] : 0.0;
    const double mu = mean[cc], is = invstd[cc], sc = scale[cc];
    double gq[9];
#pragma unroll
    for (int i = 0; i < 9; ++i) gq[i] = gram[i];
    double s = 0.0;
    if (e0 + e < C * 4) {
        for (int t0 = sl; t0 < parts; t0 += 64 * 12) {
            float v[12];
#pragma unroll
            for (int q = 0; q < 12; ++q) v[q] = (t0 + 64 * q < parts) ? partial[(int64_t)(t0 + 64 * q) * C * 4 + e0 + e] : 0.f;
#pragma unroll
            for (int q = 0; q < 12; ++q) s += (double)v[q];
        }
    }
    red[sl][e] = s;
    __syncthreads();
    if (sl < 8) {
        double t = 0.0;
#pragma unroll
        for (int q = 0; q < 8; ++q) t += red[sl * 8 + q][e];
        red2[sl][e] = t;
    }
    __syncthreads();
    if (sl == 0) {
        double t = 0.0;
#pragma unroll
        for (int q = 0; q < 8; ++q) t += red2[q][e];
        red[0][e] = t;
    }
    __syncthreads();
    if (fin) {
        const double T0 = red[0][threadIdx.x * 4 + 0], T1 = red[0][threadIdx.x * 4 + 1], T2 = red[0][threadIdx.x * 4 + 2], S = red[0][threadIdx.x * 4 + 3];
        const double dg = is * (w0 * T0 + w1 * T1 + w2 * T2 + (b - mu) * S);
        dbeta[c] = accumulate ? dbeta[c] + (float)S : (float)S;
        dgamma[c] = accumulate ? dgamma[c] + (float)dg : (float)dg;
        const double c1 = S / M, c2 = dg / M;
        const double Sx[3] = {gq[0], gq[1], gq[2]};
        const double Sxx[3][3] = {{gq[3], gq[4], gq[5]}, {gq[4], gq[6], gq[7]}, {gq[5], gq[7], gq[8]}};
        const double T[3] = {T0, T1, T2};
#pragma unroll
        for (int k = 0; k < 3; ++k) {
            const double yx = w0 * Sxx[0][k] + w1 * Sxx[1][k] + w2 * Sxx[2][k] + (b - mu) * Sx[k];
            const float gk_ = (float)(sc * (T[k] - c1 * Sx[k] - c2 * is * yx));
            float *o = dw + (int64_t)c * ldw + xcol0 + k;
            *o = accumulate ? *o + gk_ : gk_;
        }
    }
}

}

using namespace papc;

extern "C" {

int papc_xyz_parts(int64_t M) { return M >= 1 ? (int)std::min<int64_t>(cdiv(M, 1024), XYZ_MAX_PARTS) : 0; }
int papc_xyz_bwd_parts(int64_t M) { return M >= 1 ? (int)cdiv(M, 1024) : 0; }

int papc_xyz_group_f32(const papc_group_src *grp, int B, float *xc, double *gram_partial, papc_stream_t stream)
{
    PAPC_REQUIRE(grp && grp->xyz && grp->new_xyz && xc && gram_partial, PAPC_E_INVALID, "papc_xyz_group_f32: null pointer");
    PAPC_REQUIRE(B >= 1 && grp->N >= 1 && grp->S >= 1 && grp->K >= 1, PAPC_E_INVALID, "papc_xyz_group_f32: bad sizes");
    PAPC_REQUIRE(aligned16(xc), PAPC_E_INVALID, "papc_xyz_group_f32: xc must be 16-byte aligned");
    const int64_t M = (int64_t)B * grp->S * grp->K;
    PAPC_REQUIRE(M < (1ll << 31), PAPC_E_UNSUPPORTED, "papc_xyz_group_f32: M=%lld >= 2^31 rows", (long long)M);
    GroupSrc g;
    memset(&g, 0, sizeof(g));
    g.xyz = grp->xyz; g.sb = grp->sb; g.sn = grp->sn; g.sc = grp->sc; g.new_xyz = grp->new_xyz; g.idx = grp->idx;
    g.N = grp->N; g.S = grp->S; g.K = grp->K; g.D = 0; g.xyz_first = 1;
    g.divK = make_fastdiv((uint32_t)grp->K); g.divS = make_fastdiv((uint32_t)grp->S);
    hipStream_t st = as_stream(stream);
    ProfScope prof(PAPC_K_GROUP, st);
    hipLaunchKernelGGL(xyz_group_kernel, dim3((unsigned)papc_xyz_parts(M)), dim3(XYZ_T), 0, st, g, M, reinterpret_cast<float4 *>(xc), gram_partial);
    return check_launch("papc_xyz_group_f32");
}

int papc_xyz_gram_fold_f32(const double *gram_partial, int parts, double *gram, papc_stream_t stream)
{
    PAPC_REQUIRE(gram_partial && gram && parts >= 1, PAPC_E_INVALID, "papc_xyz_gram_fold_f32: bad arguments");
    hipStream_t st = as_stream(stream);
    ProfScope prof(PAPC_K_GROUP, st);
    hipLaunchKernelGGL(xyz_gram_fold_kernel, dim3(1), dim3(256), 0, st, gram_partial, parts, gram);
    return check_launch("papc_xyz_gram_fold_f32");
}

int papc_xyz_l1_finalize_f32(const double *gram_partial, int parts, int64_t M, const float *w, int ldw, int xcol0, const float *bias,
                             const float *gamma, const float *beta, float eps, float momentum, int C, float *mean, float *invstd, float *scale,
                             float *shift, float *running_mean, float *running_var, float *wf, double *gram, papc_stream_t stream)
{
    PAPC_REQUIRE(gram_partial && w && mean && invstd && scale && shift && wf && gram, PAPC_E_INVALID, "papc_xyz_l1_finalize_f32: null pointer");
    PAPC_REQUIRE(parts >= 1 && M >= 1 && C >= 1 && ldw >= xcol0 + 3 && xcol0 >= 0, PAPC_E_INVALID, "papc_xyz_l1_finalize_f32: bad sizes");
    hipStream_t st = as_stream(stream);
    ProfScope prof(PAPC_K_MISC, st);
    hipLaunchKernelGGL(xyz_l1_finalize_kernel, dim3(1), dim3(256), 0, st, gram_partial, parts, (double)M, w, ldw, xcol0, bias, gamma, beta, eps,
                       momentum, C, mean, invstd, scale, shift, running_mean, running_var, wf, gram);
    return check_launch("papc_xyz_l1_finalize_f32");
}

int papc_xyz_l1_bwd_f32(const float *dz, const float *xc, const float *wf, int64_t M, int C, float *partial, papc_stream_t stream)
{
    PAPC_REQUIRE(dz && xc && wf && partial, PAPC_E_INVALID, "papc_xyz_l1_bwd_f32: null pointer");
    PAPC_REQUIRE(M >= 1 && C >= 4 && C <= 256 && C % 4 == 0, PAPC_E_UNSUPPORTED, "papc_xyz_l1_bwd_f32: C=%d must be a multiple of 4 in [4, 256]", C);
    PAPC_REQUIRE(aligned16(dz) && aligned16(xc) && aligned16(wf), PAPC_E_INVALID, "papc_xyz_l1_bwd_f32: 16-byte alignment");
    hipStream_t st = as_stream(stream);
    ProfScope prof(PAPC_K_BWD_DW, st);
    hipLaunchKernelGGL(xyz_l1_bwd_kernel, dim3((unsigned)papc_xyz_bwd_parts(M)), dim3(XYZ_T), 0, st, dz, reinterpret_cast<const float4 *>(xc), wf, M, C,
                       (int64_t)1024, partial);
    return check_launch("papc_xyz_l1_bwd_f32");
}

int papc_xyz_l1_bwd_finalize_f32(const float *partial, int parts, int64_t M, int C, const double *gram, const float *w, int ldw, int xcol0,
                                 const float *bias, const float *mean, const float *invstd, const float *scale, float *dgamma, float *dbeta,
                                 float *dw, int accumulate, papc_stream_t stream)
{
    PAPC_REQUIRE(partial && gram && w && mean && invstd && scale && dgamma && dbeta && dw, PAPC_E_INVALID, "papc_xyz_l1_bwd_finalize_f32: null pointer");
    PAPC_REQUIRE(parts >= 1 && M >= 1 && C >= 1 && C <= 256 && ldw >= xcol0 + 3 && xcol0 >= 0, PAPC_E_INVALID, "papc_xyz_l1_bwd_finalize_f32: bad sizes");
    hipStream_t st = as_stream(stream);
    ProfScope prof(PAPC_K_BWD_DW, st);
    hipLaunchKernelGGL(xyz_l1_bwd_finalize_kernel, dim3((unsigned)cdiv(C, 4)), dim3(1024), 0, st, partial, parts, (double)M, C, gram, w, ldw, xcol0, bias, mean, invstd,
                       scale, dgamma, dbeta, dw, accumulate);
    return check_launch("papc_xyz_l1_bwd_finalize_f32");
}

}
```

papc_amd/folds.py:

```python
import ctypes
import os
import threading

import torch

from . import _lib

ENABLED = os.environ.get("PAPC_DEFER_FOLDS", "1") != "0"
CAPACITY = 96


class FoldJob(ctypes.Structure):
    _fields_ = [("partial", ctypes.c_void_p), ("n_chunks", ctypes.c_int32), ("accumulate", ctypes.c_int32), ("ld", ctypes.c_int64),
                ("rows", ctypes.c_int32), ("cols", ctypes.c_int32), ("out", ctypes.c_void_p), ("out_ld", ctypes.c_int64)]


class FoldList(ctypes.Structure):
    _fields_ = [("jobs", ctypes.POINTER(FoldJob)), ("capacity", ctypes.c_int32), ("count", ctypes.c_int32)]


class _Pending:

    def __init__(self, task_id):
        self.task_id = task_id
        self.jobs = (FoldJob * CAPACITY)()
        self.lst = FoldList(ctypes.cast(self.jobs, ctypes.POINTER(FoldJob)), CAPACITY, 0)
        self.keep = []
        self.stream = _cur_stream()
        self.owner = threading.get_ident()
        self.done = False

    def flush(self):
        with _lock:
            _live.pop(self.task_id, None)
            for k in [k for k, q in _live.items() if q.owner == self.owner and k > self.task_id]:
                _live.pop(k).drop()
        if self.done:
            return
        try:
            if self.lst.count:
                _launch(self)
        finally:
            self.drop()

    def drop(self):
        self.done = True
        self.lst.count = 0
# ... 51 lines not shown
```

papc_amd/mlp.py:

```python
import ctypes

import torch

from . import _lib
from ._lib import BwdDy, BwdRed, GroupMax, GroupSrc, ReduceJob, ScatterDst, check, cst_ptrs, ptr, stream_ptr
from .nodeparts import DwPartials, LayerSlots, bn_bwd_sums, identity_bn, launch_batched
from .nodeparts import grad_targets_of, _dw_rows_per_chunk

A_PLAIN, A_BNRELU, A_GROUP, A_XYZ = 0, 1, 2, 6
DZ_DENSE, DZ_MAX = 0, 1


class StackSpec:

    def __init__(self, B, N, S, K, D, xyz_first, eps=1e-5, momentum=0.9, cut_gather_grad=False, pool=True, eval_bn=False):
        self.B, self.N, self.S, self.K, self.D = B, N, S, K, D
        self.pool = bool(pool)
        self.eval_bn = bool(eval_bn)
        self.xyz_first = bool(xyz_first)
        self.eps, self.momentum = float(eps), float(momentum)
        self.cut_gather_grad = cut_gather_grad
        self.M = B * S * K
        self.grad_targets = None
        self.wt_table = None
        self.xyz_pre = None
        self.compact = None
        self.plists = None


def _group_src(spec, xyz, new_xyz, feats, idx):
    g = GroupSrc()
    g.xyz = xyz.data_ptr()
    g.sb, g.sn, g.sc = xyz.stride(0), xyz.stride(1), xyz.stride(2)
    g.new_xyz = new_xyz.data_ptr()
    g.feats = ptr(feats)
    g.idx = ptr(idx)
    g.N, g.S, g.K, g.D = spec.N, spec.S, spec.K, spec.D
    g.xyz_first = int(spec.xyz_first)
    return g


import os
_FUSE_RED = os.environ.get("PAPC_NO_RED") != "1"
_FUSE_GMAX = os.environ.get("PAPC_NO_GMAX") != "1"
_LIN_GATHER = os.environ.get("PAPC_LIN_GATHER", "1") == "1"
_NOSTORE = os.environ.get("PAPC_NOSTORE", "1") == "1"
_SPARSE_MAX = os.environ.get("PAPC_SPARSE_MAX", "0") == "1"
_PY_ORCH = os.environ.get("PAPC_PY_ORCH", "0") == "1"
_XYZ1 = os.environ.get("PAPC_XYZ1", "1") == "1"
_XYZ_FUSE = os.environ.get("PAPC_XYZ_FUSE", "1") == "1"




def precompute_wt(weights, feat_blocks=()):
    lib = _lib.load()
    st = stream_ptr()
    table = {}
    ok = lambda w: w.is_cuda and w.is_contiguous() and w.dtype == torch.float32
    jobs = []
    for w in weights:
        if ok(w):
            cout = w.shape[0]
            cin = w.numel() // cout
            t = torch.empty(cin, cout, device=w.device, dtype=torch.float32)
            table[w.data_ptr()] = t
            jobs.append((w.data_ptr(), cin, t, cout, cin, 0))
    for w, xyz_first in feat_blocks:
        cout = w.shape[0]
        cin = w.numel() // cout
        if ok(w) and cin > 3:
            t = torch.empty(cout, cin - 3, device=w.device, dtype=torch.float32)
            table[("f", w.data_ptr())] = (t, bool(xyz_first))
            jobs.append((w.data_ptr() + (12 if xyz_first else 0), cin, t, cout, cin - 3, 1))
    for g0 in range(0, len(jobs), 8):
        grp = jobs[g0:g0 + 8]
        n = len(grp)
        srcs, dsts = (ctypes.c_void_p * n)(), (ctypes.c_void_p * n)()
        lds, rws, cls, cps = (ctypes.c_int * n)(), (ctypes.c_int * n)(), (ctypes.c_int * n)(), (ctypes.c_int * n)()
        for i, (src, ld, t, rows, cols, cp) in enumerate(grp):
            srcs[i], lds[i], dsts[i], rws[i], cls[i], cps[i] = src, ld, t.data_ptr(), rows, cols, cp
        check(lib.papc_transpose_batch_ld_f32(srcs, lds, dsts, rws, cls, cps, n, st), "papc_transpose_batch_ld_f32")
    return table


def xyz_first_layer_ok(M, c1, c2, n_layers):
    return bool(_XYZ1 and n_layers >= 3 and _lib.load().papc_mlp_xyz_ok(M, c1, c2))


def xyz_pregroup(xyz, new_xyz, idx, out=None):
    lib = _lib.load()
    B, N = xyz.shape[0], xyz.shape[1]
    S, K = idx.shape[1], idx.shape[2]
    M = B * S * K
    dev = xyz.device
    if out is None:
        out = (torch.empty(M, 4, device=dev, dtype=torch.float32), torch.empty(1, 16, device=dev, dtype=torch.float64))
    gpart = torch.empty(lib.papc_xyz_parts(M), 16, device=dev, dtype=torch.float64)
    g = GroupSrc()
    g.xyz = xyz.data_ptr()
    g.sb, g.sn, g.sc = xyz.stride(0), xyz.stride(1), xyz.stride(2)
    g.new_xyz, g.feats, g.idx = new_xyz.data_ptr(), 0, idx.data_ptr()
    g.N, g.S, g.K, g.D, g.xyz_first = N, S, K, 0, 1
    check(lib.papc_xyz_group_f32(ctypes.byref(g), B, ptr(out[0]), ptr(gpart), stream_ptr()), "papc_xyz_group_f32")
    check(lib.papc_xyz_gram_fold_f32(ptr(gpart), gpart.shape[0], ptr(out[1]), stream_ptr()), "papc_xyz_gram_fold_f32")
    return out


class SharedMLPMax(torch.autograd.Function):

    @staticmethod
    def forward(ctx, spec, bn_buffers, xyz, new_xyz, feats, idx, x_rows, *params):
        lib = _lib.load()
        st = stream_ptr()
        dev = params[0].device
# ... 342 lines not shown
```

papc_amd/models.py:

```python
import torch
import torch.nn as nn
import torch.nn.functional as F

from .layers import (PointNetFeaturePropagation, PointNetSetAbstraction, PointNetSetAbstractionMsg, _bn_buffers,
                     _stack_params)
from . import _lib
from . import head as _head
from .copyops import cat_copy
from .mlp import StackSpec, shared_mlp_max
from .plan import new_xyz

import os
_FUSED_HEAD = os.environ.get("PAPC_NO_FUSED_HEAD") != "1"


def _starts(start_idx, n):
    if start_idx is None:
        return [None] * n
    assert len(start_idx) == n, "start_idx must hold one [B] tensor per FPS level"
    return list(start_idx)


def _bn1d(bn, y):
    if not (bn.training and bn.track_running_stats and y.shape[0] > 1):
# ... 49 lines not shown
        self.bn2 = nn.BatchNorm1d(256)
        self.drop2 = nn.Dropout(0.4)
        self.fc3 = nn.Linear(256, num_classes)

    def plan_sampling(self, inputs, start_idx=None, out=None, stage=None):
        xyz = torch.as_tensor(inputs)
        if self.normal_channel:
            xyz = xyz[:, :3, :]
        s = _starts(start_idx, 2)
        with torch.no_grad():
            o = out if out is not None else (None, None)
            if stage == "fps1":
                return self.sa1.sample_fps(xyz, s[0], out=new_xyz(o[0]))
            p1 = self.sa1.sample(xyz, s[0], out=o[0], new_xyz=new_xyz(o[0]) if stage == "rest" else None)
            p2 = self.sa2.sample(new_xyz(p1).transpose(1, 2), s[1], out=o[1])
        return p1, p2

    def forward(self, inputs, start_idx=None, plan=None, after_sa2=None, tap=None, after_sa3=None, labels=None, after_sa1=None):
        xyz = torch.as_tensor(inputs)
        B = xyz.shape[0]
        if self.normal_channel:
            norm, xyz = xyz[:, 3:, :], xyz[:, :3, :]
        else:
            norm = None
        s = _starts(start_idx, 2)
        pl = plan if plan is not None else (None, None)
        wt = None
        if torch.is_grad_enabled() and xyz.is_cuda:
            from . import smallm
            from .mlp import precompute_wt
            ws = [c.weight for c in list(self.sa1.mlp_convs)[1:]] + [c.weight for c in self.sa2.mlp_convs]
            if not (smallm.takes_group_all(B, self.sa2.npoint, [c.weight.shape[0] for c in self.sa3.mlp_convs])):
                ws += [c.weight for c in self.sa3.mlp_convs]
            wt = precompute_wt(ws, feat_blocks=[(self.sa2.mlp_convs[0].weight, True)])
        l1_xyz, l1_points = self.sa1(xyz, norm, s[0], sampled=pl[0], wt_table=wt)
        if after_sa1 is not None:
            after_sa1()
        l2_xyz, l2_points = self.sa2(l1_xyz, l1_points, s[1], sampled=pl[1], wt_table=wt)
        if after_sa2 is not None:
            after_sa2()
        if tap is not None:
            tap["l2_points"] = l2_points
        l3_xyz, l3_points = self.sa3(l2_xyz, l2_points, wt_table=wt)
        if after_sa3 is not None:
            after_sa3()
        x = l3_points.reshape(B, 1024)
        return self._head(x, labels)


class PointNet2_MSG_Clas(nn.Module, _ClasHead):
    def __init__(self, name_scope='PointNet2_MSG_Clas_', num_classes=16, normal_channel=False, reference_quirks=False):
        super().__init__()
        in_channel = 3 if normal_channel else 0
        self.normal_channel = normal_channel
        q = dict(reference_quirks=reference_quirks)
        self.sa1 = PointNetSetAbstractionMsg(512, [0.1, 0.2, 0.4], [16, 32, 128], in_channel,
                                             [[32, 32, 64], [64, 64, 128], [64, 96, 128]], **q)
        self.sa2 = PointNetSetAbstractionMsg(128, [0.2, 0.4, 0.8], [32, 64, 128], 320,
                                             [[64, 64, 128], [128, 128, 256], [128, 128, 256]], **q)
        self.sa3 = PointNetSetAbstraction(None, None, None, 640 + 3, [256, 512, 1024], True, **q)
        self.fc1 = nn.Linear(1024, 512)
        self.bn1 = nn.BatchNorm1d(512)
        self.drop1 = nn.Dropout(0.4)
        self.fc2 = nn.Linear(512, 256)
        self.bn2 = nn.BatchNorm1d(256)
        self.drop2 = nn.Dropout(0.5)
        self.fc3 = nn.Linear(256, num_classes)

# ... 592 lines not shown
```

papc_amd/stack.py:

```python
import ctypes
import os

import torch

from . import _lib
from ._lib import check, ptr, stream_ptr
from .nodeparts import LayerSlots

MAXL = 8
c_p, c_i, c_l, c_f = ctypes.c_void_p, ctypes.c_int32, ctypes.c_int64, ctypes.c_float
NO_LINGATHER, NO_XYZ1, NO_NOSTORE, NO_GMAX, NO_FUSED_RED, NO_COMPACT, NO_PLANES, NO_PLANES_POINTWISE, NO_XYZ_FUSE, NO_WSTATS, NO_PSEL, NO_GSIGN = 1, 2, 4, 8, 16, 32, 64, 128, 256, 512, 1024, 2048


class SaDesc(ctypes.Structure):
    _fields_ = [("B", c_i), ("N", c_i), ("S", c_i), ("K", c_i), ("D", c_i), ("n_layers", c_i), ("cin", c_i), ("cout", c_i * MAXL),
                ("input", c_i), ("identity_rows", c_i), ("xyz_first", c_i), ("pool", c_i), ("eval_bn", c_i), ("cut_gather_grad", c_i),
                ("eps", c_f), ("momentum", c_f), ("disable", ctypes.c_uint32), ("inference", c_i), ("want_input_grad", c_i)]


class SaLayer(ctypes.Structure):
    _fields_ = [("w", c_p), ("b", c_p), ("gamma", c_p), ("beta", c_p), ("running_mean", c_p), ("running_var", c_p)]


class CompactSrc(ctypes.Structure):
    _fields_ = [("start", c_p), ("rows", c_p), ("cidx", c_p), ("seg_grp", c_p), ("wrow", c_p), ("coef", c_p), ("G", c_i)]


class SaIo(ctypes.Structure):
    _fields_ = [("xyz", c_p), ("sb", c_l), ("sn", c_l), ("sc", c_l), ("new_xyz", c_p), ("feats", c_p), ("idx", c_p), ("x_rows", c_p),
                ("xc", c_p), ("xc_gram", c_p), ("compact", ctypes.POINTER(CompactSrc)), ("consts3", c_p), ("consts3_ld", c_i),
                ("layer", SaLayer * MAXL), ("out", c_p), ("saved", c_p), ("scratch", c_p), ("plists", c_p), ("wfeat", c_p)]


class SaPlan(ctypes.Structure):
    _fields_ = [("d", SaDesc), ("cin0", c_i), ("lin0", c_i), ("xyz1", c_i), ("gmax", c_i), ("nostore", c_i), ("compact", c_i), ("sparse_max", c_i),
                ("planes", c_i), ("saved_bytes", c_l), ("fwd_scratch_bytes", c_l), ("bwd_scratch_bytes", c_l), ("off_y", c_l * MAXL), ("off_cst", c_l * MAXL),
                ("off_argmax", c_l)]


class SaGrads(ctypes.Structure):
    _fields_ = [("gout", c_p), ("dw", c_p * MAXL), ("db", c_p * MAXL), ("dgamma", c_p * MAXL), ("dbeta", c_p * MAXL), ("acc_w", c_i * MAXL),
                ("acc_gb", c_i * MAXL), ("wt", c_p * MAXL), ("grad_feats", c_p), ("grad_x", c_p), ("defer", c_p)]

# ... 78 lines not shown
        lib = _lib.load()
        dev = params[0].device
        L = len(params) // 4
        assert 1 <= L <= MAXL
        plain = x_rows is not None
        d = SaDesc()
        d.B, d.N, d.S, d.K, d.D, d.n_layers = spec.B, spec.N, spec.S, spec.K, spec.D, L
        d.cin = x_rows.shape[1] if plain else spec.D + 3
        for l in range(L):
            d.cout[l] = params[4 * l].shape[0]
        d.input = 1 if plain else 0
        d.identity_rows = int((not plain) and idx is None)
        d.xyz_first, d.pool, d.eval_bn, d.cut_gather_grad = int(spec.xyz_first), int(spec.pool), int(spec.eval_bn), int(bool(spec.cut_gather_grad))
        d.eps, d.momentum = spec.eps, spec.momentum
        d.disable = _disable_bits()
        if feats is not None and not feats.is_contiguous():
            d.disable |= NO_LINGATHER | NO_PLANES
        if plain and not x_rows.is_contiguous():
            d.disable |= NO_PLANES
        d.inference = int(not any(ctx.needs_input_grad))
        d.want_input_grad = int((plain and x_rows.requires_grad) or ((not plain) and feats is not None and feats.requires_grad and not spec.cut_gather_grad))
        keep = []
        io = SaIo()
        _fill_io(io, spec, xyz, new_xyz, feats, idx, x_rows, params, bn_buffers, keep)
        plan = SaPlan()
        check(lib.papc_sa_mlp_plan(ctypes.byref(d), ctypes.byref(io), ctypes.byref(plan)), "papc_sa_mlp_plan")
        M = spec.M
        G = spec.B * spec.S
        cL = params[4 * (L - 1)].shape[0]
        out = torch.empty(G if spec.pool else M, cL, device=dev, dtype=torch.float32)
        saved = torch.empty(plan.saved_bytes, device=dev, dtype=torch.uint8)
        scratch = torch.empty(plan.fwd_scratch_bytes, device=dev, dtype=torch.uint8)
        io.out, io.saved, io.scratch = out.data_ptr(), saved.data_ptr(), scratch.data_ptr()
        check(lib.papc_sa_mlp_fwd(ctypes.byref(plan), ctypes.byref(io), stream_ptr()), "papc_sa_mlp_fwd")
        ctx.spec, ctx.L, ctx.plan, ctx.saved = spec, L, plan, saved
        LAST_PLANS[(int(M), tuple(int(d.cout[l]) for l in range(L)))] = dict(
            lin0=bool(plan.lin0), xyz1=bool(plan.xyz1), gmax=bool(plan.gmax), nostore=bool(plan.nostore), compact=bool(plan.compact), planes=bool(plan.planes),
            xyz_fuse=bool(plan.xyz1) and not (d.disable & NO_XYZ_FUSE))
        ctx.compact = spec.compact if plan.compact else None
        ctx.nostore, ctx.xyz1, ctx.lin0, ctx.planes = bool(plan.nostore), bool(plan.xyz1), bool(plan.lin0), bool(plan.planes)
        ctx.bn_buffers = bn_buffers
        ctx.wt_table = spec.wt_table
        ctx.feats_needs_grad = feats is not None and feats.requires_grad and not spec.cut_gather_grad
        ctx.x_needs_grad = plain and x_rows.requires_grad
        ctx.save_for_backward(xyz, new_xyz, feats, idx, x_rows, *params)
        return out

    @staticmethod
    def views(ctx):
        plan, saved, spec, L = ctx.plan, ctx.saved, ctx.spec, ctx.L
        M, G = spec.M, spec.B * spec.S
        def view(off, n, dt):
            return None if off < 0 else saved[off: off + 4 * n].view(dt)
        cs = [plan.d.cout[l] for l in range(L)]
        am = view(plan.off_argmax, G * cs[-1], torch.int32)
        ys = [None if plan.off_y[l] < 0 else view(plan.off_y[l], M * cs[l], torch.float32).view(M, cs[l]) for l in range(L)]
        cst = [view(plan.off_cst[l], 4 * cs[l], torch.float32).view(4, cs[l]) for l in range(L)]
        return (None if am is None else am.view(G, cs[-1])), ys, cst

    @staticmethod
    def backward(ctx, gout):
        lib = _lib.load()
        spec, L, plan = ctx.spec, ctx.L, ctx.plan
        tens = ctx.saved_tensors
        xyz, new_xyz, feats, idx, x_rows = tens[:5]
        params = tens[5:]
# ... 38 lines not shown
```

Before: 22300.

## Fold small finalize kernels into transpose and fold-job launches

Defers the weight-transpose prep so it runs in the same launch as the SA1 xyz layer-1 BN finalize, with an extra grid row executing the finalize body. It also adds deferred variants of the dw-max and xyz-l1 backward finalize that push a finalize record into the fold job list instead of launching separate single-block kernels. The aim is to cut kernel launch count and per-launch overhead of tiny serial kernels. It adds complexity through mixed job encodings in the fold list and new knobs.

New measurement: 22550, median of 6. 1.01x the previous value.

```diff
diff --git a/include/papc_hip.h b/include/papc_hip.h
--- a/include/papc_hip.h
+++ b/include/papc_hip.h
@@ -198,6 +198,20 @@
 } papc_fold_job;
 typedef struct papc_fold_list { papc_fold_job *jobs; int32_t capacity, count; } papc_fold_list;
 int papc_fold_jobs_f32(const papc_fold_job *jobs, int count, papc_stream_t stream);
+#define PAPC_FOLD_F64Q (-1)
+#define PAPC_FOLD_FIN (-2)
+#define PAPC_FIN_DW_MAX 1
+#define PAPC_FIN_XYZ_BWD 2
+typedef struct papc_fold_fin {
+    int32_t kind, accumulate;
+    int32_t C, parts, ldw, xcol0;
+    double M, inv_m;
+    const void *src;
+    const double *gram;
+    const float *w, *bias, *mean, *invstd, *scale, *e, *c1;
+    float *dgamma, *dbeta, *dw;
+} papc_fold_fin;
+#define PAPC_FOLD_FIN_SLOTS ((int)((sizeof(papc_fold_fin) + sizeof(papc_fold_job) - 1) / sizeof(papc_fold_job)))
 
 #define PAPC_SA_MAX_LAYERS 8
 #define PAPC_SA_IN_GROUP 0
@@ -213,6 +227,7 @@
 #define PAPC_SA_NO_XYZ_FUSE 256u
 #define PAPC_SA_NO_PSEL 1024u
 #define PAPC_SA_NO_GSIGN 2048u
+#define PAPC_SA_L1_DONE 4096u
 #define PAPC_SA_NO_WSTATS 512u
 typedef struct papc_sa_desc {
     int32_t B, N, S, K, D;
@@ -268,6 +283,8 @@
 } papc_sa_grads;
 int papc_sa_mlp_plan(const papc_sa_desc *desc, const papc_sa_io *io, papc_sa_plan *plan);
 int papc_sa_mlp_fwd(const papc_sa_plan *plan, const papc_sa_io *io, papc_stream_t stream);
+int papc_sa_mlp_xyz1_prep(const papc_sa_plan *plan, const papc_sa_io *io, const float *const *src, const int *src_ld, float *const *dst,
+                          const int *rows, const int *cols, const int *copy, int count, papc_stream_t stream);
 int papc_sa_mlp_bwd(const papc_sa_plan *plan, const papc_sa_io *io, const papc_sa_grads *grads, papc_stream_t stream);
 
 typedef struct papc_pfn_desc {
@@ -529,6 +546,9 @@
 int papc_mlp_bwd_dw_max_f32(const float *psel, const int32_t *argmax, int K, const float *x, const float *bn_scale, const float *bn_shift,
                             const float *w, const float *e, const float *scale, const float *c1, int64_t M, int Cin, int Cout,
                             float *workspace, float *dw, int accumulate, papc_stream_t stream);
+int papc_mlp_bwd_dw_max_defer_f32(const float *psel, const int32_t *argmax, int K, const float *x, const float *bn_scale, const float *bn_shift,
+                                  const float *w, const float *e, const float *scale, const float *c1, int64_t M, int Cin, int Cout,
+                                  float *workspace, float *dw, int accumulate, papc_fold_list *defer, papc_stream_t stream);
 
 int papc_mlp_xyz_ok(int64_t M, int C1, int C2);
 int papc_xyz_parts(int64_t M);
@@ -542,6 +562,9 @@
 int papc_xyz_l1_bwd_finalize_f32(const float *partial, int parts, int64_t M, int C, const double *gram, const float *w, int ldw, int xcol0,
                                  const float *bias, const float *mean, const float *invstd, const float *scale, float *dgamma, float *dbeta,
                                  float *dw, int accumulate, papc_stream_t stream);
+int papc_xyz_l1_bwd_finalize_defer_f32(const float *partial, int parts, int64_t M, int C, const double *gram, const float *w, int ldw, int xcol0,
+                                       const float *bias, const float *mean, const float *invstd, const float *scale, float *dgamma, float *dbeta,
+                                       float *dw, int accumulate, papc_fold_list *defer, papc_stream_t stream);
 
 size_t papc_pg_planes_bytes(int64_t R, int64_t K);
 
diff --git a/papc_amd/_lib.py b/papc_amd/_lib.py
--- a/papc_amd/_lib.py
+++ b/papc_amd/_lib.py
@@ -83,6 +83,7 @@
     "papc_mlp_gemm_rows_w_f32": (c_i, [c_i, c_p, c_l, c_p, c_p, c_p, c_p, c_p, c_l, c_i, c_i, c_p, c_p, c_p, c_p, c_p, c_p]),
     "papc_sa_mlp_plan": (c_i, [c_p, c_p, c_p]),
     "papc_sa_mlp_fwd": (c_i, [c_p, c_p, c_p]),
+    "papc_sa_mlp_xyz1_prep": (c_i, [c_p, c_p, c_p, c_p, c_p, c_p, c_p, c_p, c_i, c_p]),
     "papc_sa_mlp_bwd": (c_i, [c_p, c_p, c_p, c_p]),
     "papc_pfn_workspace": (c_i, [c_p, c_p, c_p]),
     "papc_pfn_fwd": (c_i, [c_p, c_p, c_p]),
@@ -191,6 +192,7 @@
     "papc_mlp_max_nostore_ok": (c_i, [c_l, c_i, c_i, c_i]),
     "papc_mlp_bwd_dw_max_ws_floats": (c_l, [c_l, c_i, c_i]),
     "papc_mlp_bwd_dw_max_f32": (c_i, [c_p, c_p, c_i, c_p, c_p, c_p, c_p, c_p, c_p, c_p, c_l, c_i, c_i, c_p, c_p, c_i, c_p]),
+    "papc_mlp_bwd_dw_max_defer_f32": (c_i, [c_p, c_p, c_i, c_p, c_p, c_p, c_p, c_p, c_p, c_p, c_l, c_i, c_i, c_p, c_p, c_i, c_p, c_p]),
     "papc_mlp_bwd_dx_xyz_ok": (c_i, [c_l, c_i, c_i]),
     "papc_mlp_bwd_dx_xyz_f32": (c_i, [c_p, c_p, c_l, c_i, c_i, c_p, c_p, c_p, c_p]),
     "papc_mlp_bwd_dx_max_f32": (c_i, [c_p, c_p, c_i, c_p, c_l, c_p, c_p, c_p, c_p, c_l, c_i, c_i, c_p, c_p, c_p]),
@@ -202,6 +204,7 @@
     "papc_xyz_l1_finalize_f32": (c_i, [c_p, c_i, c_l, c_p, c_i, c_i, c_p, c_p, c_p, c_f, c_f, c_i] + [c_p] * 9),
     "papc_xyz_l1_bwd_f32": (c_i, [c_p, c_p, c_p, c_l, c_i, c_p, c_p]),
     "papc_xyz_l1_bwd_finalize_f32": (c_i, [c_p, c_i, c_l, c_i, c_p, c_p, c_i, c_i] + [c_p] * 7 + [c_i, c_p]),
+    "papc_xyz_l1_bwd_finalize_defer_f32": (c_i, [c_p, c_i, c_l, c_i, c_p, c_p, c_i, c_i] + [c_p] * 7 + [c_i, c_p, c_p]),
     "papc_pg_planes_bytes": (ctypes.c_size_t, [c_l, c_l]),
     "papc_pg_prep_weights_f32": (c_i, [c_p, c_i, c_p]),
     "papc_pg_prep_rows_f32": (c_i, [c_p, c_p]),
diff --git a/papc_amd/csrc/bn_ops.hip b/papc_amd/csrc/bn_ops.hip
--- a/papc_amd/csrc/bn_ops.hip
+++ b/papc_amd/csrc/bn_ops.hip
@@ -1,4 +1,5 @@
 #include "common.h"
+#include "finalize.h"
 
 namespace papc {
 
@@ -538,9 +539,8 @@
     int ld[8], copy[8];
 };
 
-__global__ __launch_bounds__(256) void transpose_batch_kernel(TransposeBatch t)
-{
-    __shared__ float tile[32][33];
+__device__ __forceinline__ void transpose_batch_body(float (&tile)[32][33], const TransposeBatch &t)
+{
     const int m = blockIdx.y;
     const int rows = t.rows[m], cols = t.cols[m];
     const int tiles_c = (cols + 31) >> 5, tiles = ((rows + 31) >> 5) * tiles_c;
@@ -565,6 +565,20 @@
         }
         __syncthreads();
     }
+}
+
+__global__ __launch_bounds__(256) void transpose_batch_kernel(TransposeBatch t)
+{
+    __shared__ float tile[32][33];
+    transpose_batch_body(tile, t);
+}
+
+__global__ __launch_bounds__(256) void transpose_batch_l1_kernel(TransposeBatch t, int count, XyzL1Fin a)
+{
+    __shared__ float tile[32][33];
+    __shared__ double lds[XYZ_L1_FIN_LDS];
+    if ((int)blockIdx.y < count) transpose_batch_body(tile, t);
+    else if (blockIdx.x == 0) xyz_l1_finalize_body(lds, a);
 }
 
 int bn_finalize_clear(const float *stats_partial, int n_tiles, int64_t M, int C, const float *gamma, const float *beta, float eps, float momentum,
@@ -782,25 +796,51 @@
     return papc_transpose_batch_ld_f32(src, nullptr, dst, rows, cols, nullptr, count, stream);
 }
 
-int papc_transpose_batch_ld_f32(const float *const *src, const int *src_ld, float *const *dst, const int *rows, const int *cols, const int *copy, int count,
-                                papc_stream_t stream)
-{
-    PAPC_REQUIRE(src && dst && rows && cols, PAPC_E_INVALID, "papc_transpose_batch_f32: null pointer");
-    PAPC_REQUIRE(count >= 1 && count <= 8, PAPC_E_INVALID, "papc_transpose_batch_f32: count=%d not in [1, 8]", count);
-    TransposeBatch t{};
-    int max_tiles = 1;
+static int fill_transposes(TransposeBatch &t, int *max_tiles, const float *const *src, const int *src_ld, float *const *dst, const int *rows, const int *cols,
+                           const int *copy, int count)
+{
+    *max_tiles = 1;
     for (int i = 0; i < count; ++i) {
         PAPC_REQUIRE(src[i] && dst[i] && rows[i] >= 1 && cols[i] >= 1, PAPC_E_INVALID, "papc_transpose_batch_f32: bad entry %d", i);
         t.src[i] = src[i]; t.dst[i] = dst[i]; t.rows[i] = rows[i]; t.cols[i] = cols[i];
         t.ld[i] = src_ld ? src_ld[i] : cols[i]; t.copy[i] = copy ? copy[i] : 0;
         PAPC_REQUIRE(t.ld[i] >= cols[i], PAPC_E_INVALID, "papc_transpose_batch_f32: entry %d: row stride shorter than a row", i);
-        max_tiles = std::max(max_tiles, (int)(cdiv(rows[i], 32) * cdiv(cols[i], 32)));
-    }
+        *max_tiles = std::max(*max_tiles, (int)(cdiv(rows[i], 32) * cdiv(cols[i], 32)));
+    }
+    return PAPC_OK;
+}
+
+int papc_transpose_batch_ld_f32(const float *const *src, const int *src_ld, float *const *dst, const int *rows, const int *cols, const int *copy, int count,
+                                papc_stream_t stream)
+{
+    PAPC_REQUIRE(src && dst && rows && cols, PAPC_E_INVALID, "papc_transpose_batch_f32: null pointer");
+    PAPC_REQUIRE(count >= 1 && count <= 8, PAPC_E_INVALID, "papc_transpose_batch_f32: count=%d not in [1, 8]", count);
+    TransposeBatch t{};
+    int max_tiles = 1;
+    const int rc = fill_transposes(t, &max_tiles, src, src_ld, dst, rows, cols, copy, count);
+    if (rc != PAPC_OK) return rc;
     hipStream_t st = as_stream(stream);
     ProfScope prof(PAPC_K_MISC, st);
     hipLaunchKernelGGL(transpose_batch_kernel, dim3((unsigned)std::min(max_tiles, 512), (unsigned)count), dim3(256), 0, st, t);
     return check_launch("papc_transpose_batch_f32");
 }
+
+}
+
+int papc::transpose_batch_l1(const float *const *src, const int *src_ld, float *const *dst, const int *rows, const int *cols, const int *copy, int count,
+                             const XyzL1Fin &a, hipStream_t st)
+{
+    PAPC_REQUIRE(count >= 0 && count <= 8 && (count == 0 || (src && dst && rows && cols)), PAPC_E_INVALID, "transpose_batch_l1: bad arguments");
+    TransposeBatch t{};
+    int max_tiles = 1;
+    const int rc = fill_transposes(t, &max_tiles, src, src_ld, dst, rows, cols, copy, count);
+    if (rc != PAPC_OK) return rc;
+    ProfScope prof(PAPC_K_MISC, st);
+    hipLaunchKernelGGL(transpose_batch_l1_kernel, dim3((unsigned)std::min(max_tiles, 512), (unsigned)count + 1), dim3(256), 0, st, t, count, a);
+    return check_launch("papc_sa_mlp_xyz1_prep");
+}
+
+extern "C" {
 
 static int adam_step(float *param, float *grad, float *exp_avg, float *exp_avg_sq, int64_t n, float lr, double beta1, double beta2, float eps,
                      float weight_decay, int step, float grad_scale, bool zero, papc_stream_t stream, const char *who)
diff --git a/papc_amd/csrc/capi.hip b/papc_amd/csrc/capi.hip
--- a/papc_amd/csrc/capi.hip
+++ b/papc_amd/csrc/capi.hip
@@ -71,6 +71,8 @@
     {"PAPC_PG_GROUP", 1, 0, 1},
     {"PAPC_PG_PIPE", 1, 0, 1},
     {"PAPC_SEG_EPI", 1, 0, 1},
+    {"PAPC_FOLD_FIN", 1, 0, 1},
+    {"PAPC_XYZ1_RIDE", 1, 0, 1},
 };
 static int g_knobs[KNOB_COUNT];
 static int knob_parse(int id, const char *e)
@@ -161,6 +163,7 @@
     PAPC_SIZEOF(papc_reduce_job)
     PAPC_SIZEOF(papc_fold_job)
     PAPC_SIZEOF(papc_fold_list)
+    PAPC_SIZEOF(papc_fold_fin)
     PAPC_SIZEOF(papc_sa_desc)
     PAPC_SIZEOF(papc_sa_layer)
     PAPC_SIZEOF(papc_compact_src)
diff --git a/papc_amd/csrc/common.h b/papc_amd/csrc/common.h
--- a/papc_amd/csrc/common.h
+++ b/papc_amd/csrc/common.h
@@ -24,7 +24,7 @@
 enum Knob {
     KNOB_LG_PARTS, KNOB_DW_F32, KNOB_DW_DBG, KNOB_DW_XYZ, KNOB_PARTS, KNOB_GEMM_F32, KNOB_GEMM_WAVES, KNOB_MAXCAT_WAVES,
     KNOB_GEMM_WS, KNOB_GEMM_OCC, KNOB_GEMM_DBG, KNOB_GEMM_KB, KNOB_GEMM_MINWG, KNOB_GEMM_TL, KNOB_FPS_THREADS,
-    KNOB_FPS_THREADS_SMALL, KNOB_STREAM, KNOB_STREAM_MINTILES, KNOB_STREAM_CK, KNOB_STREAM_ASM, KNOB_PFN_MFMA, KNOB_DW_RS64, KNOB_DW_ROWS, KNOB_DW_ROWS_BLOCKS, KNOB_DW_ROWSX, KNOB_PG_DBG, KNOB_PG_NB, KNOB_PG_NS, KNOB_STREAM_MAXCAT, KNOB_MAX_NOSTORE, KNOB_PFN_FUSED_TAILS, KNOB_STREAM_NW12, KNOB_LG_LISTS, KNOB_FOLD_WAVES, KNOB_LGL_VARIANT, KNOB_LG_PP, KNOB_PG_GROUP, KNOB_PG_PIPE, KNOB_SEG_EPI, KNOB_COUNT
+    KNOB_FPS_THREADS_SMALL, KNOB_STREAM, KNOB_STREAM_MINTILES, KNOB_STREAM_CK, KNOB_STREAM_ASM, KNOB_PFN_MFMA, KNOB_DW_RS64, KNOB_DW_ROWS, KNOB_DW_ROWS_BLOCKS, KNOB_DW_ROWSX, KNOB_PG_DBG, KNOB_PG_NB, KNOB_PG_NS, KNOB_STREAM_MAXCAT, KNOB_MAX_NOSTORE, KNOB_PFN_FUSED_TAILS, KNOB_STREAM_NW12, KNOB_LG_LISTS, KNOB_FOLD_WAVES, KNOB_LGL_VARIANT, KNOB_LG_PP, KNOB_PG_GROUP, KNOB_PG_PIPE, KNOB_SEG_EPI, KNOB_FOLD_FIN, KNOB_XYZ1_RIDE, KNOB_COUNT
 };
 int knob(int id);
 
diff --git a/papc_amd/csrc/finalize.h b/papc_amd/csrc/finalize.h
--- /dev/null
+++ b/papc_amd/csrc/finalize.h
@@ -0,0 +1,143 @@
+#pragma once
+#include "common.h"
+
+namespace papc {
+
+constexpr int DWMAX_CI = 64;
+constexpr int DWMAX_FIN_LDS = DWMAX_CI * DWMAX_CI;
+constexpr int XYZ_BWD_FIN_LDS = 64 * 17 + 8 * 17;
+
+__device__ __forceinline__ void dw_max_finalize_body(double *__restrict__ gc, int wg, int nt, const double *__restrict__ fold, const float *__restrict__ w,
+                                                     const float *__restrict__ e, const float *__restrict__ scale, const float *__restrict__ c1, double inv_m,
+                                                     int Cout, float *__restrict__ dw, int accumulate)
+{
+    constexpr int CI = DWMAX_CI;
+    const int tid = threadIdx.x;
+    const double *G = fold + (int64_t)Cout * CI, *S = G + CI * CI;
+    for (int q = tid; q < CI * CI; q += nt) {
+        const int j = q >> 6, i = q & 63;
+        gc[j * CI + i] = G[q] - S[j] * S[i] * inv_m;
+    }
+    __syncthreads();
+    const int i = tid & 63, c = 4 * wg + (tid >> 6);
+    if (tid >= 256 || c >= Cout) return;
+    double dot = 0.0;
+    for (int j = 0; j < CI; ++j) dot += (double)w[(int64_t)c * CI + j] * gc[j * CI + i];
+    const double v = fold[(int64_t)c * CI + i] - (double)scale[c] * (double)c1[c] * S[i] - (double)e[c] * dot;
+    float *o = dw + (int64_t)c * CI + i;
+    *o = accumulate ? *o + (float)v : (float)v;
+}
+
+struct XyzL1Fin {
+    const double *partial; int parts; double M;
+    const float *w; int ldw, xcol0;
+    const float *bias, *gamma, *beta;
+    float eps, momentum; int C;
+    float *mean, *invstd, *scale, *shift, *rmean, *rvar, *wf;
+    double *gram;
+};
+constexpr int XYZ_L1_FIN_LDS = 16 * 16 + 10;
+int transpose_batch_l1(const float *const *src, const int *src_ld, float *const *dst, const int *rows, const int *cols, const int *copy, int count,
+                       const XyzL1Fin &a, hipStream_t st);
+__device__ __forceinline__ void xyz_l1_finalize_body(double *__restrict__ lds, const XyzL1Fin &a)
+{
+    double(*red)[16] = reinterpret_cast<double(*)[16]>(lds);
+    double *G = lds + 16 * 16;
+    const double M = a.M;
+    const int e = threadIdx.x & 15, sl = threadIdx.x >> 4;
+    double s = 0.0;
+    if (e < 10) for (int t = sl; t < a.parts; t += 16) s += a.partial[(int64_t)t * 16 + e];
+    red[sl][e] = s;
+    __syncthreads();
+    if (threadIdx.x < 10) {
+        double v = 0.0;
+#pragma unroll
+        for (int q = 0; q < 16; ++q) v += red[q][threadIdx.x];
+        G[threadIdx.x] = v;
+        a.gram[threadIdx.x] = v;
+    }
+    __syncthreads();
+    for (int c = threadIdx.x; c < a.C; c += 256) {
+        const double w0 = a.w[(int64_t)c * a.ldw + a.xcol0], w1 = a.w[(int64_t)c * a.ldw + a.xcol0 + 1], w2 = a.w[(int64_t)c * a.ldw + a.xcol0 + 2];
+        const double b = a.bias ? (double)a.bias[c] : 0.0;
+        const double mx = G[0] / M, my = G[1] / M, mz = G[2] / M;
+        const double cxx = G[3] / M - mx * mx, cxy = G[4] / M - mx * my, cxz = G[5] / M - mx * mz;
+        const double cyy = G[6] / M - my * my, cyz = G[7] / M - my * mz, czz = G[8] / M - mz * mz;
+        const double mu = w0 * mx + w1 * my + w2 * mz + b;
+        double var = w0 * (w0 * cxx + w1 * cxy + w2 * cxz) + w1 * (w0 * cxy + w1 * cyy + w2 * cyz) + w2 * (w0 * cxz + w1 * cyz + w2 * czz);
+        if (var < 0.0) var = 0.0;
+        const double is = 1.0 / sqrt(var + (double)a.eps);
+        const double sc = (a.gamma ? (double)a.gamma[c] : 1.0) * is;
+        const double sh = (a.beta ? (double)a.beta[c] : 0.0) - mu * sc;
+        a.mean[c] = (float)mu; a.invstd[c] = (float)is; a.scale[c] = (float)sc; a.shift[c] = (float)sh;
+        if (a.rmean) a.rmean[c] = a.momentum * a.rmean[c] + (1.f - a.momentum) * (float)mu;
+        if (a.rvar) a.rvar[c] = a.momentum * a.rvar[c] + (1.f - a.momentum) * (float)var;
+        a.wf[c * 4 + 0] = (float)(sc * w0); a.wf[c * 4 + 1] = (float)(sc * w1); a.wf[c * 4 + 2] = (float)(sc * w2);
+        a.wf[c * 4 + 3] = (float)(sc * b + sh);
+    }
+}
+
+__device__ __forceinline__ void xyz_l1_bwd_finalize_body(double *__restrict__ lds, int wg, const float *__restrict__ partial, int parts, double M, int C,
+                                                         const double *__restrict__ gram, const float *__restrict__ w, int ldw, int xcol0,
+                                                         const float *__restrict__ bias, const float *__restrict__ mean, const float *__restrict__ invstd,
+                                                         const float *__restrict__ scale, float *dgamma, float *dbeta, float *dw, int accumulate)
+{
+    double(*red)[17] = reinterpret_cast<double(*)[17]>(lds);
+    double(*red2)[17] = reinterpret_cast<double(*)[17]>(lds + 64 * 17);
+    const int e = threadIdx.x & 15, sl = threadIdx.x >> 4;
+    const int e0 = wg * 16;
+    const int c = wg * 4 + threadIdx.x;
+    const bool fin = threadIdx.x < 4 && c < C;
+    const int cc = fin ? c : 0;
+    const double w0 = w[(int64_t)cc * ldw + xcol0], w1 = w[(int64_t)cc * ldw + xcol0 + 1], w2 = w[(int64_t)cc * ldw + xcol0 + 2];
+    const double b = bias ? (double)bias[cc] : 0.0;
+    const double mu = mean[cc], is = invstd[cc], sc = scale[cc];
+    double gq[9];
+#pragma unroll
+    for (int i = 0; i < 9; ++i) gq[i] = gram[i];
+    double s = 0.0;
+    if (e0 + e < C * 4) {
+        for (int t0 = sl; t0 < parts; t0 += 64 * 12) {
+            float v[12];
+#pragma unroll
+            for (int q = 0; q < 12; ++q) v[q] = (t0 + 64 * q < parts) ? partial[(int64_t)(t0 + 64 * q) * C * 4 + e0 + e] : 0.f;
+#pragma unroll
+            for (int q = 0; q < 12; ++q) s += (double)v[q];
+        }
+    }
+    red[sl][e] = s;
+    __syncthreads();
+    if (sl < 8) {
+        double t = 0.0;
+#pragma unroll
+        for (int q = 0; q < 8; ++q) t += red[sl * 8 + q][e];
+        red2[sl][e] = t;
+    }
+    __syncthreads();
+    if (sl == 0) {
+        double t = 0.0;
+#pragma unroll
+        for (int q = 0; q < 8; ++q) t += red2[q][e];
+        red[0][e] = t;
+    }
+    __syncthreads();
+    if (fin) {
+        const double T0 = red[0][threadIdx.x * 4 + 0], T1 = red[0][threadIdx.x * 4 + 1], T2 = red[0][threadIdx.x * 4 + 2], S = red[0][threadIdx.x * 4 + 3];
+        const double dg = is * (w0 * T0 + w1 * T1 + w2 * T2 + (b - mu) * S);
+        dbeta[c] = accumulate ? dbeta[c] + (float)S : (float)S;
+        dgamma[c] = accumulate ? dgamma[c] + (float)dg : (float)dg;
+        const double c1 = S / M, c2 = dg / M;
+        const double Sx[3] = {gq[0], gq[1], gq[2]};
+        const double Sxx[3][3] = {{gq[3], gq[4], gq[5]}, {gq[4], gq[6], gq[7]}, {gq[5], gq[7], gq[8]}};
+        const double T[3] = {T0, T1, T2};
+#pragma unroll
+        for (int k = 0; k < 3; ++k) {
+            const double yx = w0 * Sxx[0][k] + w1 * Sxx[1][k] + w2 * Sxx[2][k] + (b - mu) * Sx[k];
+            const float gk_ = (float)(sc * (T[k] - c1 * Sx[k] - c2 * is * yx));
+            float *o = dw + (int64_t)c * ldw + xcol0 + k;
+            *o = accumulate ? *o + gk_ : gk_;
+        }
+    }
+}
+
+}
diff --git a/papc_amd/csrc/fold.h b/papc_amd/csrc/fold.h
--- a/papc_amd/csrc/fold.h
+++ b/papc_amd/csrc/fold.h
@@ -2,6 +2,22 @@
 #include "common.h"
 
 namespace papc {
+
+static inline bool fold_list_room(const papc_fold_list *fl, int slots) { return fl && fl->jobs && fl->count + slots <= fl->capacity; }
+static inline void fold_list_push_f64q(papc_fold_list *fl, const float *partial, int n_chunks, int64_t ld, int n, double *out)
+{
+    papc_fold_job &j = fl->jobs[fl->count++];
+    memset(&j, 0, sizeof(j));
+    j.partial = partial; j.n_chunks = n_chunks; j.ld = ld; j.rows = PAPC_FOLD_F64Q; j.cols = n; j.out = reinterpret_cast<float *>(out); j.out_ld = n;
+}
+static inline void fold_list_push_fin(papc_fold_list *fl, const papc_fold_fin &f)
+{
+    papc_fold_job &j = fl->jobs[fl->count];
+    memset(&j, 0, sizeof(j) * (1 + PAPC_FOLD_FIN_SLOTS));
+    j.rows = PAPC_FOLD_FIN; j.n_chunks = PAPC_FOLD_FIN_SLOTS; j.cols = f.kind;
+    memcpy(&fl->jobs[fl->count + 1], &f, sizeof(f));
+    fl->count += 1 + PAPC_FOLD_FIN_SLOTS;
+}
 
 template <typename V> __device__ __forceinline__ V fold_zero();
 template <> __device__ __forceinline__ float fold_zero<float>() { return 0.f; }
@@ -56,4 +72,25 @@
     return s;
 }
 
+__device__ __forceinline__ bool fold_quarters_f64(const float *__restrict__ part, int64_t ld, int n_chunks, int64_t e, bool live, double &total)
+{
+    const int l = threadIdx.x & 15, q = (threadIdx.x & 63) >> 4;
+    const int per = (n_chunks + 3) / 4, c0 = q * per, c1 = min(n_chunks, c0 + per);
+    double s = 0.0;
+    if (live) {
+        int c = c0;
+        for (; c + 8 <= c1; c += 8) {
+            float v[8];
+#pragma unroll
+            for (int j = 0; j < 8; ++j) v[j] = part[(int64_t)(c + j) * ld + e];
+#pragma unroll
+            for (int j = 0; j < 8; ++j) s += (double)v[j];
+        }
+        for (; c < c1; ++c) s += (double)part[(int64_t)c * ld + e];
+    }
+    const double s1 = __shfl(s, l + 16), s2 = __shfl(s, l + 32), s3 = __shfl(s, l + 48);
+    total = ((s + s1) + s2) + s3;
+    return q == 0 && live;
 }
+
+}
diff --git a/papc_amd/csrc/folds.hip b/papc_amd/csrc/folds.hip
--- a/papc_amd/csrc/folds.hip
+++ b/papc_amd/csrc/folds.hip
@@ -1,3 +1,6 @@
+#include <vector>
+
+#include "finalize.h"
 #include "fold.h"
 
 namespace papc {
@@ -82,7 +85,7 @@
     const float *part[PAPC_FOLD_MAX]; float *out[PAPC_FOLD_MAX];
     int64_t ld[PAPC_FOLD_MAX], out_ld[PAPC_FOLD_MAX];
     int n_chunks[PAPC_FOLD_MAX], rows[PAPC_FOLD_MAX], cols[PAPC_FOLD_MAX], wg0[PAPC_FOLD_MAX + 1];
-    unsigned acc_mask, wide_mask, vec_mask;
+    unsigned acc_mask, wide_mask, vec_mask, f64_mask;
     int count;
 };
 template <int FW>
@@ -98,6 +101,12 @@
     const int n_chunks = b.n_chunks[job], cols = b.cols[job];
     const int64_t n = (int64_t)b.rows[job] * cols;
     const bool acc = (b.acc_mask >> job) & 1u;
+    if ((b.f64_mask >> job) & 1u) {
+        const int64_t e = ((int64_t)wg * FW + (threadIdx.x >> 6)) * 16 + (threadIdx.x & 15);
+        double t;
+        if (fold_quarters_f64(part, ld, n_chunks, e, e < n, t)) reinterpret_cast<double *>(out)[e] = t;
+        return;
+    }
     if ((b.wide_mask >> job) & 1u) {
         const int64_t e = ((int64_t)wg * (64 * FW) + threadIdx.x) * 4;
         if (e >= n) return;
@@ -128,10 +137,52 @@
     }
 }
 
+constexpr int FIN_MAX = 4;
+struct FinBatch { papc_fold_fin f[FIN_MAX]; int wg0[FIN_MAX + 1], count; };
+__global__ __launch_bounds__(1024) void fold_fin_kernel(FinBatch b)
+{
+    __shared__ double lds[DWMAX_FIN_LDS > XYZ_BWD_FIN_LDS ? DWMAX_FIN_LDS : XYZ_BWD_FIN_LDS];
+    int r = 0;
+    while (r + 1 < b.count && (int)blockIdx.x >= b.wg0[r + 1]) ++r;
+    const int wg = (int)blockIdx.x - b.wg0[r];
+    const papc_fold_fin &f = b.f[r];
+    if (f.kind == PAPC_FIN_DW_MAX)
+        dw_max_finalize_body(lds, wg, 1024, static_cast<const double *>(f.src), f.w, f.e, f.scale, f.c1, f.inv_m, f.C, f.dw, f.accumulate);
+    else
+        xyz_l1_bwd_finalize_body(lds, wg, static_cast<const float *>(f.src), f.parts, f.M, f.C, f.gram, f.w, f.ldw, f.xcol0, f.bias, f.mean, f.invstd,
+                                 f.scale, f.dgamma, f.dbeta, f.dw, f.accumulate);
+}
+
 }
 
 
 using namespace papc;
+
+static int launch_fins(const papc_fold_fin *fins, int count, hipStream_t st)
+{
+    for (int r0 = 0; r0 < count;) {
+        FinBatch b;
+        memset(&b, 0, sizeof(b));
+        int n = 0, wgs = 0;
+        for (; n < FIN_MAX && r0 + n < count; ++n) {
+            const papc_fold_fin &f = fins[r0 + n];
+            bool shared = false;
+            for (int k = 0; k < n && !shared; ++k) shared = b.f[k].dw == f.dw || (f.dgamma && b.f[k].dgamma == f.dgamma) || (f.dbeta && b.f[k].dbeta == f.dbeta);
+            if (shared) break;
+            b.f[n] = f;
+            b.wg0[n] = wgs;
+            wgs += (int)cdiv(f.C, 4);
+        }
+        b.wg0[n] = wgs;
+        b.count = n;
+        ProfScope prof(PAPC_K_BWD_DW, st);
+        hipLaunchKernelGGL(fold_fin_kernel, dim3((unsigned)wgs), dim3(1024), 0, st, b);
+        const int rc = check_launch("papc_fold_jobs_f32 (finalizes)");
+        if (rc != PAPC_OK) return rc;
+        r0 += n;
+    }
+    return PAPC_OK;
+}
 
 static bool disjoint_column_blocks(const papc_fold_job &a, const papc_fold_job &b)
 {
@@ -184,11 +235,25 @@
     return check_launch("papc_reduce_partials_batch_f32");
 }
 
-int papc_fold_jobs_f32(const papc_fold_job *jobs, int count, papc_stream_t stream)
-{
-    PAPC_REQUIRE(jobs, PAPC_E_INVALID, "papc_fold_jobs_f32: null jobs");
-    PAPC_REQUIRE(count >= 1, PAPC_E_INVALID, "papc_fold_jobs_f32: count=%d", count);
-    hipStream_t st = as_stream(stream);
+int papc_fold_jobs_f32(const papc_fold_job *list, int list_count, papc_stream_t stream)
+{
+    PAPC_REQUIRE(list, PAPC_E_INVALID, "papc_fold_jobs_f32: null jobs");
+    PAPC_REQUIRE(list_count >= 1, PAPC_E_INVALID, "papc_fold_jobs_f32: count=%d", list_count);
+    hipStream_t st = as_stream(stream);
+    std::vector<papc_fold_job> folds;
+    std::vector<papc_fold_fin> fins;
+    for (int i = 0; i < list_count; ++i) {
+        if (list[i].rows != PAPC_FOLD_FIN) { folds.push_back(list[i]); continue; }
+        PAPC_REQUIRE(list[i].n_chunks == PAPC_FOLD_FIN_SLOTS && i + PAPC_FOLD_FIN_SLOTS < list_count, PAPC_E_INVALID, "papc_fold_jobs_f32: truncated finalize record at job %d", i);
+        papc_fold_fin f;
+        memcpy(&f, &list[i + 1], sizeof(f));
+        PAPC_REQUIRE((f.kind == PAPC_FIN_DW_MAX || f.kind == PAPC_FIN_XYZ_BWD) && f.kind == list[i].cols && f.C >= 1 && f.src && f.dw, PAPC_E_INVALID,
+                     "papc_fold_jobs_f32: bad finalize record at job %d", i);
+        fins.push_back(f);
+        i += PAPC_FOLD_FIN_SLOTS;
+    }
+    const papc_fold_job *jobs = folds.data();
+    const int count = (int)folds.size();
     const int FW = knob(KNOB_FOLD_WAVES) == 16 ? 16 : 8;
     for (int j0 = 0; j0 < count;) {
         FoldBatch b;
@@ -198,25 +263,29 @@
         int nj = 0;
         for (; nj < PAPC_FOLD_MAX && j0 + nj < count; ++nj) {
             const int i = nj;
-            const papc_fold_job &j = jobs[j0 + i];
+            papc_fold_job j = jobs[j0 + i];
+            const bool f64 = j.rows == PAPC_FOLD_F64Q;
+            if (f64) j.rows = 1;
             PAPC_REQUIRE(j.partial && j.out, PAPC_E_INVALID, "papc_fold_jobs_f32: null pointer in job %d", j0 + i);
             PAPC_REQUIRE(j.n_chunks >= 1 && j.rows >= 1 && j.cols >= 1 && j.ld >= (int64_t)j.rows * j.cols && j.out_ld >= j.cols, PAPC_E_INVALID,
                          "papc_fold_jobs_f32: bad sizes in job %d", j0 + i);
+            PAPC_REQUIRE(!f64 || (!j.accumulate && ((uintptr_t)j.out & 7) == 0), PAPC_E_INVALID, "papc_fold_jobs_f32: bad float64 job %d", j0 + i);
             lo[i] = (uintptr_t)j.out;
-            hi[i] = lo[i] + sizeof(float) * (uintptr_t)((int64_t)(j.rows - 1) * j.out_ld + j.cols);
+            hi[i] = lo[i] + (f64 ? sizeof(double) : sizeof(float)) * (uintptr_t)((int64_t)(j.rows - 1) * j.out_ld + j.cols);
             bool overlaps = false;
             for (int k = 0; k < i && !overlaps; ++k)
                 overlaps = lo[i] < hi[k] && lo[k] < hi[i] && !disjoint_column_blocks(jobs[j0 + k], j);
             if (overlaps) break;
             const int64_t n = (int64_t)j.rows * j.cols;
-            const bool wide = j.n_chunks <= 16 && n >= 16384 && n % 4 == 0 && j.ld % 4 == 0 && (j.rows == 1 || j.out_ld == j.cols) && aligned16(j.partial) && aligned16(j.out);
+            const bool wide = !f64 && j.n_chunks <= 16 && n >= 16384 && n % 4 == 0 && j.ld % 4 == 0 && (j.rows == 1 || j.out_ld == j.cols) && aligned16(j.partial) && aligned16(j.out);
             b.part[i] = j.partial; b.out[i] = j.out; b.ld[i] = j.ld; b.out_ld[i] = j.out_ld; b.n_chunks[i] = j.n_chunks; b.rows[i] = j.rows; b.cols[i] = j.cols;
             if (j.accumulate) b.acc_mask |= 1u << i;
-            const bool vec = !wide && n >= 1024 && n % 4 == 0 && j.ld % 4 == 0 && (j.rows == 1 || j.out_ld == j.cols) && aligned16(j.partial) && aligned16(j.out);
+            const bool vec = !f64 && !wide && n >= 1024 && n % 4 == 0 && j.ld % 4 == 0 && (j.rows == 1 || j.out_ld == j.cols) && aligned16(j.partial) && aligned16(j.out);
             if (wide) b.wide_mask |= 1u << i;
             if (vec) b.vec_mask |= 1u << i;
+            if (f64) b.f64_mask |= 1u << i;
             b.wg0[i] = (int)wgs;
-            wgs += wide ? cdiv(n, 4 * 64 * FW) : (vec ? cdiv(n, 256) : cdiv(n, 64));
+            wgs += f64 ? cdiv(n, 16 * FW) : wide ? cdiv(n, 4 * 64 * FW) : (vec ? cdiv(n, 256) : cdiv(n, 64));
             PAPC_REQUIRE(wgs < (1ll << 30), PAPC_E_UNSUPPORTED, "papc_fold_jobs_f32: too many elements");
         }
         b.wg0[nj] = (int)wgs;
@@ -228,7 +297,7 @@
         if (rc != PAPC_OK) return rc;
         j0 += nj;
     }
-    return PAPC_OK;
+    return fins.empty() ? PAPC_OK : launch_fins(fins.data(), (int)fins.size(), st);
 }
 
 int papc_reduce_partials_f32(const float *partial, int n_chunks, int64_t n, float *out, int accumulate, papc_stream_t stream)
diff --git a/papc_amd/csrc/mlp_dw.hip b/papc_amd/csrc/mlp_dw.hip
--- a/papc_amd/csrc/mlp_dw.hip
+++ b/papc_amd/csrc/mlp_dw.hip
@@ -1,5 +1,7 @@
 #include <type_traits>
 #include "mlp_loaders.h"
+#include "finalize.h"
+#include "fold.h"
 
 namespace papc {
 
@@ -1113,45 +1115,17 @@
 
 __global__ __launch_bounds__(64) void dw_max_fold_kernel(const float *__restrict__ partial, int n_chunks, int64_t part_ld, int n, double *__restrict__ out)
 {
-    const int l = threadIdx.x & 15, q = threadIdx.x >> 4;
-    const int e = blockIdx.x * 16 + l;
-    const int per = (n_chunks + 3) / 4, c0 = q * per, c1 = min(n_chunks, c0 + per);
-    double s = 0.0;
-    if (e < n) {
-        int c = c0;
-        for (; c + 8 <= c1; c += 8) {
-            float v[8];
-#pragma unroll
-            for (int j = 0; j < 8; ++j) v[j] = partial[(int64_t)(c + j) * part_ld + e];
-#pragma unroll
-            for (int j = 0; j < 8; ++j) s += (double)v[j];
-        }
-        for (; c < c1; ++c) s += (double)partial[(int64_t)c * part_ld + e];
-    }
-    const double s1 = __shfl(s, l + 16), s2 = __shfl(s, l + 32), s3 = __shfl(s, l + 48);
-    if (q == 0 && e < n) out[e] = ((s + s1) + s2) + s3;
+    const int e = blockIdx.x * 16 + (threadIdx.x & 15);
+    double t;
+    if (fold_quarters_f64(partial, part_ld, n_chunks, e, e < n, t)) out[e] = t;
 }
 
 __global__ __launch_bounds__(256) void dw_max_finalize_kernel(const double *__restrict__ fold, const float *__restrict__ w, const float *__restrict__ e,
                                                               const float *__restrict__ scale, const float *__restrict__ c1, double inv_m, int Cout,
                                                               float *__restrict__ dw, int accumulate)
 {
-    constexpr int CI = 64;
-    __shared__ double gc[CI][CI];
-    const int tid = threadIdx.x;
-    const double *G = fold + (int64_t)Cout * CI, *S = G + CI * CI;
-    for (int q = tid; q < CI * CI; q += 256) {
-        const int j = q >> 6, i = q & 63;
-        gc[j][i] = G[q] - S[j] * S[i] * inv_m;
-    }
-    __syncthreads();
-    const int i = tid & 63, c = 4 * blockIdx.x + (tid >> 6);
-    if (c >= Cout) return;
-    double dot = 0.0;
-    for (int j = 0; j < CI; ++j) dot += (double)w[(int64_t)c * CI + j] * gc[j][i];
-    const double v = fold[(int64_t)c * CI + i] - (double)scale[c] * (double)c1[c] * S[i] - (double)e[c] * dot;
-    float *o = dw + (int64_t)c * CI + i;
-    *o = accumulate ? *o + (float)v : (float)v;
+    __shared__ double gc[DWMAX_FIN_LDS];
+    dw_max_finalize_body(gc, blockIdx.x, 256, fold, w, e, scale, c1, inv_m, Cout, dw, accumulate);
 }
 
 static void dw_dbg_report(const DwArgs &p, int xm, int dm)
@@ -1365,6 +1339,13 @@
                                        const float *w, const float *e, const float *scale, const float *c1, int64_t M, int Cin, int Cout,
                                        float *workspace, float *dw, int accumulate, papc_stream_t stream)
 {
+    return papc_mlp_bwd_dw_max_defer_f32(psel, argmax, K, x, bn_scale, bn_shift, w, e, scale, c1, M, Cin, Cout, workspace, dw, accumulate, nullptr, stream);
+}
+
+extern "C" int papc_mlp_bwd_dw_max_defer_f32(const float *psel, const int32_t *argmax, int K, const float *x, const float *bn_scale, const float *bn_shift,
+                                             const float *w, const float *e, const float *scale, const float *c1, int64_t M, int Cin, int Cout,
+                                             float *workspace, float *dw, int accumulate, papc_fold_list *defer, papc_stream_t stream)
+{
     PAPC_REQUIRE(psel && argmax && x && bn_scale && bn_shift && w && e && scale && c1 && workspace && dw, PAPC_E_INVALID, "papc_mlp_bwd_dw_max_f32: null pointer");
     PAPC_REQUIRE(papc_mlp_max_nostore_ok(M, Cin, Cout, K), PAPC_E_UNSUPPORTED,
                  "papc_mlp_bwd_dw_max_f32: not built for M=%lld Cin=%d Cout=%d K=%d (see papc_mlp_max_nostore_ok)", (long long)M, Cin, Cout, K);
@@ -1379,6 +1360,15 @@
     hipStream_t st = as_stream(stream);
     ProfScope prof(PAPC_K_BWD_DW, st);
     hipLaunchKernelGGL(dw_rows_max_kernel, dim3((unsigned)(2 * p.n_chunks)), dim3(512), 0, st, p);
+    if (knob(KNOB_FOLD_FIN) && fold_list_room(defer, 2 + PAPC_FOLD_FIN_SLOTS)) {
+        fold_list_push_f64q(defer, workspace, p.n_chunks, (int64_t)n, n, fold);
+        papc_fold_fin f;
+        memset(&f, 0, sizeof(f));
+        f.kind = PAPC_FIN_DW_MAX; f.accumulate = accumulate; f.C = Cout; f.inv_m = 1.0 / (double)M;
+        f.src = fold; f.w = w; f.e = e; f.scale = scale; f.c1 = c1; f.dw = dw;
+        fold_list_push_fin(defer, f);
+        return check_launch("papc_mlp_bwd_dw_max_f32");
+    }
     hipLaunchKernelGGL(dw_max_fold_kernel, dim3((unsigned)cdiv(n, 16)), dim3(64), 0, st, workspace, p.n_chunks, (int64_t)n, n, fold);
     hipLaunchKernelGGL(dw_max_finalize_kernel, dim3((unsigned)cdiv(Cout, 4)), dim3(256), 0, st, fold, w, e, scale, c1, 1.0 / (double)M, Cout, dw, accumulate);
     return check_launch("papc_mlp_bwd_dw_max_f32");
diff --git a/papc_amd/csrc/sa_mlp.hip b/papc_amd/csrc/sa_mlp.hip
--- a/papc_amd/csrc/sa_mlp.hip
+++ b/papc_amd/csrc/sa_mlp.hip
@@ -1,4 +1,5 @@
 #include "common.h"
+#include "finalize.h"
 
 #define SA_CALL(expr)                 \
     do {                              \
@@ -506,6 +507,33 @@
     return PAPC_OK;
 }
 
+int papc_sa_mlp_xyz1_prep(const papc_sa_plan *plan, const papc_sa_io *io, const float *const *src, const int *src_ld, float *const *dst, const int *rows,
+                          const int *cols, const int *copy, int count, papc_stream_t st)
+{
+    PAPC_REQUIRE(plan && io && io->saved, PAPC_E_INVALID, "papc_sa_mlp_xyz1_prep: null pointer");
+    const papc_sa_plan &p = *plan;
+    const papc_sa_desc &d = p.d;
+    PAPC_REQUIRE(p.xyz1 && !p.planes && io->xc && io->xc_gram, PAPC_E_UNSUPPORTED,
+                 "papc_sa_mlp_xyz1_prep: needs a plan with the coordinates-only first layer and the pregrouped coordinates (xc, xc_gram)");
+    PAPC_REQUIRE(count >= 0 && count <= 8, PAPC_E_INVALID, "papc_sa_mlp_xyz1_prep: count=%d not in [0, 8]", count);
+    const papc_sa_layer &ly = io->layer[0];
+    PAPC_REQUIRE(ly.w && ly.gamma && ly.beta, PAPC_E_INVALID, "papc_sa_mlp_xyz1_prep: layer 0 lacks w / gamma / beta");
+    SavedPtrs s;
+    layout_saved(p, io->saved, s);
+    const int cout = d.cout[0];
+    float *cst = s.cst[0];
+    if (!knob(KNOB_XYZ1_RIDE)) {
+        if (count) SA_CALL(papc_transpose_batch_ld_f32(src, src_ld, dst, rows, cols, copy, count, st));
+        return papc_xyz_l1_finalize_f32(io->xc_gram, 1, rows_of(d), ly.w, p.cin0, 0, ly.b, ly.gamma, ly.beta, d.eps, d.momentum, cout, cst, cst + cout,
+                                        cst + 2 * cout, cst + 3 * cout, ly.running_mean, ly.running_var, s.wf, s.gram, st);
+    }
+    XyzL1Fin a;
+    a.partial = io->xc_gram; a.parts = 1; a.M = (double)rows_of(d); a.w = ly.w; a.ldw = p.cin0; a.xcol0 = 0; a.bias = ly.b; a.gamma = ly.gamma; a.beta = ly.beta;
+    a.eps = d.eps; a.momentum = d.momentum; a.C = cout; a.mean = cst; a.invstd = cst + cout; a.scale = cst + 2 * cout; a.shift = cst + 3 * cout;
+    a.rmean = ly.running_mean; a.rvar = ly.running_var; a.wf = s.wf; a.gram = s.gram;
+    return transpose_batch_l1(src, src_ld, dst, rows, cols, copy, count, a, as_stream(st));
+}
+
 int papc_sa_mlp_fwd(const papc_sa_plan *plan, const papc_sa_io *io, papc_stream_t st)
 {
     PAPC_REQUIRE(plan && io && io->out && io->saved && io->scratch, PAPC_E_INVALID, "papc_sa_mlp_fwd: null pointer");
@@ -525,6 +553,8 @@
     SavedPtrs s; FwdPtrs f;
     layout_saved(p, io->saved, s);
     layout_fwd(p, io->scratch, f);
+    PAPC_REQUIRE(!(d.disable & PAPC_SA_L1_DONE) || (p.xyz1 && io->xc && io->xc_gram), PAPC_E_INVALID,
+                 "papc_sa_mlp_fwd: PAPC_SA_L1_DONE without the path papc_sa_mlp_xyz1_prep serves");
     const int parts = papc_mlp_gemm_parts(M);
     const bool wstats = p.compact && !(d.disable & PAPC_SA_NO_WSTATS);
     const int R_c = (p.compact && !wstats) ? papc_compact_corr_parts() : 0;
@@ -564,8 +594,9 @@
                 SA_CALL(papc_xyz_gram_fold_f32(f.gpart + 16, papc_xyz_parts(M), f.gpart, st));
                 xc = s.xc; gpart1 = f.gpart;
             }
-            SA_CALL(papc_xyz_l1_finalize_f32(gpart1, 1, M, ly.w, cin, 0, ly.b, ly.gamma, ly.beta, d.eps, d.momentum, cout, cst, cst + cout, cst + 2 * cout,
-                                             cst + 3 * cout, ly.running_mean, ly.running_var, s.wf, s.gram, st));
+            if (!(d.disable & PAPC_SA_L1_DONE))
+                SA_CALL(papc_xyz_l1_finalize_f32(gpart1, 1, M, ly.w, cin, 0, ly.b, ly.gamma, ly.beta, d.eps, d.momentum, cout, cst, cst + cout, cst + 2 * cout,
+                                                 cst + 3 * cout, ly.running_mean, ly.running_var, s.wf, s.gram, st));
             prev_y = nullptr; prev_sc = cst + 2 * cout; prev_sh = cst + 3 * cout;
             cin = cout;
             continue;
@@ -697,8 +728,8 @@
             int nbp = papc_xyz_bwd_parts(M);
             if (xyz_fused) nbp = papc_mlp_gemm_parts(M);
             else SA_CALL(papc_xyz_l1_bwd_f32(dz, xc, s.wf, M, cout, b.bpart, st));
-            SA_CALL(papc_xyz_l1_bwd_finalize_f32(b.bpart, nbp, M, cout, s.gram, ly.w, cin, 0, ly.b, cst, cst + cout, cst + 2 * cout, dgamma, dbeta, gr->dw[l],
-                                                 acc_w ? 1 : 0, st));
+            SA_CALL(papc_xyz_l1_bwd_finalize_defer_f32(b.bpart, nbp, M, cout, s.gram, ly.w, cin, 0, ly.b, cst, cst + cout, cst + 2 * cout, dgamma, dbeta, gr->dw[l],
+                                                       acc_w ? 1 : 0, gr->defer, st));
             if (gr->db[l] && !acc_w) SA_CALL(papc_fill_f32(gr->db[l], cout, 0.f, st));
             break;
         }
@@ -761,8 +792,8 @@
         const bool x1 = p.xyz1 && l == 1;
         if (p.nostore && l == L - 1) {
             const float *pc = s.cst[l - 1];
-            SA_CALL(papc_mlp_bwd_dw_max_f32(b.psel, s.argmax, d.K, s.y[l - 1], pc + 2 * cin, pc + 3 * cin, ly.w, b.eq, cst + 2 * cout, c12, M, cin, cout, b.dwmax_ws,
-                                            gr->dw[l], acc_w ? 1 : 0, st));
+            SA_CALL(papc_mlp_bwd_dw_max_defer_f32(b.psel, s.argmax, d.K, s.y[l - 1], pc + 2 * cin, pc + 3 * cin, ly.w, b.eq, cst + 2 * cout, c12, M, cin, cout, b.dwmax_ws,
+                                                  gr->dw[l], acc_w ? 1 : 0, gr->defer, st));
             if (gr->db[l] && !acc_w) SA_CALL(papc_fill_f32(gr->db[l], cout, 0.f, st));
         } else {
             const int am = l == 0 ? (plain ? A_PLAIN_ : A_GROUP_) : (x1 ? A_XYZ_ : A_BNRELU_);
diff --git a/papc_amd/csrc/xyz1.hip b/papc_amd/csrc/xyz1.hip
--- a/papc_amd/csrc/xyz1.hip
+++ b/papc_amd/csrc/xyz1.hip
@@ -1,4 +1,6 @@
 #include "mlp_loaders.h"
+#include "finalize.h"
+#include "fold.h"
 
 namespace papc {
 
@@ -62,45 +64,10 @@
     }
 }
 
-__global__ __launch_bounds__(256) void xyz_l1_finalize_kernel(const double *__restrict__ partial, int parts, double M, const float *__restrict__ w, int ldw,
-                                                              int xcol0, const float *__restrict__ bias, const float *__restrict__ gamma,
-                                                              const float *__restrict__ beta, float eps, float momentum, int C, float *mean,
-                                                              float *invstd, float *scale, float *shift, float *rmean, float *rvar, float *wf,
-                                                              double *gram)
-{
-    __shared__ double red[16][16];
-    __shared__ double G[10];
-    const int e = threadIdx.x & 15, sl = threadIdx.x >> 4;
-    double s = 0.0;
-    if (e < 10) for (int t = sl; t < parts; t += 16) s += partial[(int64_t)t * 16 + e];
-    red[sl][e] = s;
-    __syncthreads();
-    if (threadIdx.x < 10) {
-        double v = 0.0;
-#pragma unroll
-        for (int q = 0; q < 16; ++q) v += red[q][threadIdx.x];
-        G[threadIdx.x] = v;
-        gram[threadIdx.x] = v;
-    }
-    __syncthreads();
-    for (int c = threadIdx.x; c < C; c += 256) {
-        const double w0 = w[(int64_t)c * ldw + xcol0], w1 = w[(int64_t)c * ldw + xcol0 + 1], w2 = w[(int64_t)c * ldw + xcol0 + 2];
-        const double b = bias ? (double)bias[c] : 0.0;
-        const double mx = G[0] / M, my = G[1] / M, mz = G[2] / M;
-        const double cxx = G[3] / M - mx * mx, cxy = G[4] / M - mx * my, cxz = G[5] / M - mx * mz;
-        const double cyy = G[6] / M - my * my, cyz = G[7] / M - my * mz, czz = G[8] / M - mz * mz;
-        const double mu = w0 * mx + w1 * my + w2 * mz + b;
-        double var = w0 * (w0 * cxx + w1 * cxy + w2 * cxz) + w1 * (w0 * cxy + w1 * cyy + w2 * cyz) + w2 * (w0 * cxz + w1 * cyz + w2 * czz);
-        if (var < 0.0) var = 0.0;
-        const double is = 1.0 / sqrt(var + (double)eps);
-        const double sc = (gamma ? (double)gamma[c] : 1.0) * is;
-        const double sh = (beta ? (double)beta[c] : 0.0) - mu * sc;
-        mean[c] = (float)mu; invstd[c] = (float)is; scale[c] = (float)sc; shift[c] = (float)sh;
-        if (rmean) rmean[c] = momentum * rmean[c] + (1.f - momentum) * (float)mu;
-        if (rvar) rvar[c] = momentum * rvar[c] + (1.f - momentum) * (float)var;
-        wf[c * 4 + 0] = (float)(sc * w0); wf[c * 4 + 1] = (float)(sc * w1); wf[c * 4 + 2] = (float)(sc * w2);
-        wf[c * 4 + 3] = (float)(sc * b + sh);
-    }
+__global__ __launch_bounds__(256) void xyz_l1_finalize_kernel(XyzL1Fin a)
+{
+    __shared__ double lds[XYZ_L1_FIN_LDS];
+    xyz_l1_finalize_body(lds, a);
 }
 
 __global__ __launch_bounds__(XYZ_T) void xyz_l1_bwd_kernel(const float *__restrict__ dz, const float4 *__restrict__ xc, const float *__restrict__ wf,
@@ -167,61 +134,8 @@
                                                                    const float *__restrict__ mean, const float *__restrict__ invstd,
                                                                    const float *__restrict__ scale, float *dgamma, float *dbeta, float *dw, int accumulate)
 {
-    __shared__ double red[64][17], red2[8][17];
-    const int e = threadIdx.x & 15, sl = threadIdx.x >> 4;
-    const int e0 = blockIdx.x * 16;
-    const int c = blockIdx.x * 4 + threadIdx.x;
-    const bool fin = threadIdx.x < 4 && c < C;
-    const int cc = fin ? c : 0;
-    const double w0 = w[(int64_t)cc * ldw + xcol0], w1 = w[(int64_t)cc * ldw + xcol0 + 1], w2 = w[(int64_t)cc * ldw + xcol0 + 2];
-    const double b = bias ? (double)bias[cc] : 0.0;
-    const double mu = mean[cc], is = invstd[cc], sc = scale[cc];
-    double gq[9];
-#pragma unroll
-    for (int i = 0; i < 9; ++i) gq[i] = gram[i];
-    double s = 0.0;
-    if (e0 + e < C * 4) {
-        for (int t0 = sl; t0 < parts; t0 += 64 * 12) {
-            float v[12];
-#pragma unroll
-            for (int q = 0; q < 12; ++q) v[q] = (t0 + 64 * q < parts) ? partial[(int64_t)(t0 + 64 * q) * C * 4 + e0 + e] : 0.f;
-#pragma unroll
-            for (int q = 0; q < 12; ++q) s += (double)v[q];
-        }
-    }
-    red[sl][e] = s;
-    __syncthreads();
-    if (sl < 8) {
-        double t = 0.0;
-#pragma unroll
-        for (int q = 0; q < 8; ++q) t += red[sl * 8 + q][e];
-        red2[sl][e] = t;
-    }
-    __syncthreads();
-    if (sl == 0) {
-        double t = 0.0;
-#pragma unroll
-        for (int q = 0; q < 8; ++q) t += red2[q][e];
-        red[0][e] = t;
-    }
-    __syncthreads();
-    if (fin) {
-        const double T0 = red[0][threadIdx.x * 4 + 0], T1 = red[0][threadIdx.x * 4 + 1], T2 = red[0][threadIdx.x * 4 + 2], S = red[0][threadIdx.x * 4 + 3];
-        const double dg = is * (w0 * T0 + w1 * T1 + w2 * T2 + (b - mu) * S);
-        dbeta[c] = accumulate ? dbeta[c] + (float)S : (float)S;
-        dgamma[c] = accumulate ? dgamma[c] + (float)dg : (float)dg;
-        const double c1 = S / M, c2 = dg / M;
-        const double Sx[3] = {gq[0], gq[1], gq[2]};
-        const double Sxx[3][3] = {{gq[3], gq[4], gq[5]}, {gq[4], gq[6], gq[7]}, {gq[5], gq[7], gq[8]}};
-        const double T[3] = {T0, T1, T2};
-#pragma unroll
-        for (int k = 0; k < 3; ++k) {
-            const double yx = w0 * Sxx[0][k] + w1 * Sxx[1][k] + w2 * Sxx[2][k] + (b - mu) * Sx[k];
-            const float gk_ = (float)(sc * (T[k] - c1 * Sx[k] - c2 * is * yx));
-            float *o = dw + (int64_t)c * ldw + xcol0 + k;
-            *o = accumulate ? *o + gk_ : gk_;
-        }
-    }
+    __shared__ double lds[XYZ_BWD_FIN_LDS];
+    xyz_l1_bwd_finalize_body(lds, blockIdx.x, partial, parts, M, C, gram, w, ldw, xcol0, bias, mean, invstd, scale, dgamma, dbeta, dw, accumulate);
 }
 
 }
@@ -268,8 +182,11 @@
     PAPC_REQUIRE(parts >= 1 && M >= 1 && C >= 1 && ldw >= xcol0 + 3 && xcol0 >= 0, PAPC_E_INVALID, "papc_xyz_l1_finalize_f32: bad sizes");
     hipStream_t st = as_stream(stream);
     ProfScope prof(PAPC_K_MISC, st);
-    hipLaunchKernelGGL(xyz_l1_finalize_kernel, dim3(1), dim3(256), 0, st, gram_partial, parts, (double)M, w, ldw, xcol0, bias, gamma, beta, eps,
-                       momentum, C, mean, invstd, scale, shift, running_mean, running_var, wf, gram);
+    XyzL1Fin a;
+    a.partial = gram_partial; a.parts = parts; a.M = (double)M; a.w = w; a.ldw = ldw; a.xcol0 = xcol0; a.bias = bias; a.gamma = gamma; a.beta = beta;
+    a.eps = eps; a.momentum = momentum; a.C = C; a.mean = mean; a.invstd = invstd; a.scale = scale; a.shift = shift; a.rmean = running_mean;
+    a.rvar = running_var; a.wf = wf; a.gram = gram;
+    hipLaunchKernelGGL(xyz_l1_finalize_kernel, dim3(1), dim3(256), 0, st, a);
     return check_launch("papc_xyz_l1_finalize_f32");
 }
 
@@ -298,4 +215,21 @@
     return check_launch("papc_xyz_l1_bwd_finalize_f32");
 }
 
-}
+int papc_xyz_l1_bwd_finalize_defer_f32(const float *partial, int parts, int64_t M, int C, const double *gram, const float *w, int ldw, int xcol0,
+                                       const float *bias, const float *mean, const float *invstd, const float *scale, float *dgamma, float *dbeta,
+                                       float *dw, int accumulate, papc_fold_list *defer, papc_stream_t stream)
+{
+    if (!knob(KNOB_FOLD_FIN) || !fold_list_room(defer, 1 + PAPC_FOLD_FIN_SLOTS))
+        return papc_xyz_l1_bwd_finalize_f32(partial, parts, M, C, gram, w, ldw, xcol0, bias, mean, invstd, scale, dgamma, dbeta, dw, accumulate, stream);
+    PAPC_REQUIRE(partial && gram && w && mean && invstd && scale && dgamma && dbeta && dw, PAPC_E_INVALID, "papc_xyz_l1_bwd_finalize_f32: null pointer");
+    PAPC_REQUIRE(parts >= 1 && M >= 1 && C >= 1 && C <= 256 && ldw >= xcol0 + 3 && xcol0 >= 0, PAPC_E_INVALID, "papc_xyz_l1_bwd_finalize_f32: bad sizes");
+    papc_fold_fin f;
+    memset(&f, 0, sizeof(f));
+    f.kind = PAPC_FIN_XYZ_BWD; f.accumulate = accumulate; f.C = C; f.parts = parts; f.ldw = ldw; f.xcol0 = xcol0; f.M = (double)M;
+    f.src = partial; f.gram = gram; f.w = w; f.bias = bias; f.mean = mean; f.invstd = invstd; f.scale = scale;
+    f.dgamma = dgamma; f.dbeta = dbeta; f.dw = dw;
+    fold_list_push_fin(defer, f);
+    return PAPC_OK;
+}
+
+}
diff --git a/papc_amd/folds.py b/papc_amd/folds.py
--- a/papc_amd/folds.py
+++ b/papc_amd/folds.py
@@ -13,6 +13,16 @@
 class FoldJob(ctypes.Structure):
     _fields_ = [("partial", ctypes.c_void_p), ("n_chunks", ctypes.c_int32), ("accumulate", ctypes.c_int32), ("ld", ctypes.c_int64),
                 ("rows", ctypes.c_int32), ("cols", ctypes.c_int32), ("out", ctypes.c_void_p), ("out_ld", ctypes.c_int64)]
+
+
+class FoldFin(ctypes.Structure):
+    _fields_ = ([("kind", ctypes.c_int32), ("accumulate", ctypes.c_int32), ("C", ctypes.c_int32), ("parts", ctypes.c_int32), ("ldw", ctypes.c_int32),
+                 ("xcol0", ctypes.c_int32), ("M", ctypes.c_double), ("inv_m", ctypes.c_double)]
+                + [(n, ctypes.c_void_p) for n in ("src", "gram", "w", "bias", "mean", "invstd", "scale", "e", "c1", "dgamma", "dbeta", "dw")])
+
+
+FOLD_F64Q, FOLD_FIN = -1, -2
+FOLD_FIN_SLOTS = -(-ctypes.sizeof(FoldFin) // ctypes.sizeof(FoldJob))
 
 
 class FoldList(ctypes.Structure):
diff --git a/papc_amd/mlp.py b/papc_amd/mlp.py
--- a/papc_amd/mlp.py
+++ b/papc_amd/mlp.py
@@ -53,10 +53,23 @@
 
 
 
-def precompute_wt(weights, feat_blocks=()):
-    lib = _lib.load()
-    st = stream_ptr()
-    table = {}
+class WtTable(dict):
+    pending = ()
+
+    def flush(self, l1=None):
+        groups, self.pending = self.pending, ()
+        lib = _lib.load()
+        st = stream_ptr()
+        for i, (srcs, lds, dsts, rws, cls, cps, n) in enumerate(groups):
+            if l1 is not None and i == len(groups) - 1:
+                check(lib.papc_sa_mlp_xyz1_prep(ctypes.byref(l1[0]), ctypes.byref(l1[1]), srcs, lds, dsts, rws, cls, cps, n, st), "papc_sa_mlp_xyz1_prep")
+            else:
+                check(lib.papc_transpose_batch_ld_f32(srcs, lds, dsts, rws, cls, cps, n, st), "papc_transpose_batch_ld_f32")
+        return l1 is not None and bool(groups)
+
+
+def precompute_wt(weights, feat_blocks=(), lazy=False):
+    table = WtTable()
     ok = lambda w: w.is_cuda and w.is_contiguous() and w.dtype == torch.float32
     jobs = []
     for w in weights:
@@ -73,6 +86,7 @@
             t = torch.empty(cout, cin - 3, device=w.device, dtype=torch.float32)
             table[("f", w.data_ptr())] = (t, bool(xyz_first))
             jobs.append((w.data_ptr() + (12 if xyz_first else 0), cin, t, cout, cin - 3, 1))
+    groups = []
     for g0 in range(0, len(jobs), 8):
         grp = jobs[g0:g0 + 8]
         n = len(grp)
@@ -80,7 +94,10 @@
         lds, rws, cls, cps = (ctypes.c_int * n)(), (ctypes.c_int * n)(), (ctypes.c_int * n)(), (ctypes.c_int * n)()
         for i, (src, ld, t, rows, cols, cp) in enumerate(grp):
             srcs[i], lds[i], dsts[i], rws[i], cls[i], cps[i] = src, ld, t.data_ptr(), rows, cols, cp
-        check(lib.papc_transpose_batch_ld_f32(srcs, lds, dsts, rws, cls, cps, n, st), "papc_transpose_batch_ld_f32")
+        groups.append((srcs, lds, dsts, rws, cls, cps, n))
+    table.pending = tuple(groups)
+    if not lazy:
+        table.flush()
     return table
 
 
diff --git a/papc_amd/models.py b/papc_amd/models.py
--- a/papc_amd/models.py
+++ b/papc_amd/models.py
@@ -105,8 +105,10 @@
             ws = [c.weight for c in list(self.sa1.mlp_convs)[1:]] + [c.weight for c in self.sa2.mlp_convs]
             if not (smallm.takes_group_all(B, self.sa2.npoint, [c.weight.shape[0] for c in self.sa3.mlp_convs])):
                 ws += [c.weight for c in self.sa3.mlp_convs]
-            wt = precompute_wt(ws, feat_blocks=[(self.sa2.mlp_convs[0].weight, True)])
+            wt = precompute_wt(ws, feat_blocks=[(self.sa2.mlp_convs[0].weight, True)], lazy=True)
         l1_xyz, l1_points = self.sa1(xyz, norm, s[0], sampled=pl[0], wt_table=wt)
+        if wt is not None:
+            wt.flush()
         if after_sa1 is not None:
             after_sa1()
         l2_xyz, l2_points = self.sa2(l1_xyz, l1_points, s[1], sampled=pl[1], wt_table=wt)
diff --git a/papc_amd/stack.py b/papc_amd/stack.py
--- a/papc_amd/stack.py
+++ b/papc_amd/stack.py
@@ -9,6 +9,7 @@
 
 MAXL = 8
 c_p, c_i, c_l, c_f = ctypes.c_void_p, ctypes.c_int32, ctypes.c_int64, ctypes.c_float
+L1_DONE = 4096
 NO_LINGATHER, NO_XYZ1, NO_NOSTORE, NO_GMAX, NO_FUSED_RED, NO_COMPACT, NO_PLANES, NO_PLANES_POINTWISE, NO_XYZ_FUSE, NO_WSTATS, NO_PSEL, NO_GSIGN = 1, 2, 4, 8, 16, 32, 64, 128, 256, 512, 1024, 2048
 
 
@@ -153,6 +154,9 @@
         saved = torch.empty(plan.saved_bytes, device=dev, dtype=torch.uint8)
         scratch = torch.empty(plan.fwd_scratch_bytes, device=dev, dtype=torch.uint8)
         io.out, io.saved, io.scratch = out.data_ptr(), saved.data_ptr(), scratch.data_ptr()
+        wt = spec.wt_table
+        if plan.xyz1 and spec.xyz_pre is not None and getattr(wt, "pending", ()) and wt.flush(l1=(plan, io)):
+            plan.d.disable |= L1_DONE
         check(lib.papc_sa_mlp_fwd(ctypes.byref(plan), ctypes.byref(io), stream_ptr()), "papc_sa_mlp_fwd")
         ctx.spec, ctx.L, ctx.plan, ctx.saved = spec, L, plan, saved
         LAST_PLANS[(int(M), tuple(int(d.cout[l]) for l in range(L)))] = dict(
```
